# qdrant/qdrant

Measured on AMD Instinct MI355X. Metric: QPS @ recall@10, brute-force, d=768 10M vecs, f32 cosine top-10, higher is better.
Workload: dtype f32 (int8 prefilter + exact f32 re-score)

## Files before the change

include/qdrant_amd.h:

```cpp
#ifndef QDRANT_AMD_H
#define QDRANT_AMD_H

#include <stddef.h>
#include <stdint.h>

#ifdef __cplusplus
extern "C" {
#endif

#define QMX_API __attribute__((visibility("default")))

typedef enum qmx_status {
    QMX_OK = 0,
    QMX_ERR_OUT_OF_MEMORY = 1,
    QMX_ERR_OUT_OF_BOUNDS = 2,
    QMX_ERR_NOT_SUPPORTED = 3,
    QMX_ERR_NOT_READY = 4,
    QMX_ERR_TIMEOUT = 5,
    QMX_ERR_OTHER = 6,
    QMX_ERR_CANCELLED = 7,
    QMX_ERR_BAD_ARG = 8,
    QMX_ERR_NO_DEVICE = 9
} qmx_status;

// ... 135 lines not shown

QMX_API int32_t qmx_segment_create(const qmx_segment_desc *desc, qmx_segment **out);
QMX_API int32_t qmx_segment_create_from_files(const qmx_segment_desc *desc, const char *vectors_path, const char *deleted_path,
                                              qmx_segment **out);

QMX_API int32_t qmx_segment_create_chunked(const qmx_segment_desc *desc, const void *const *chunks, uint64_t rows_per_chunk,
                                           uint32_t n_chunks, qmx_segment **out);
QMX_API int32_t qmx_segment_destroy(qmx_segment *seg);
QMX_API int32_t qmx_segment_set_deleted(qmx_segment *seg, const uint64_t *point_deleted,
                                        uint64_t n_point_bits, const uint64_t *vec_deleted,
                                        uint64_t n_vec_bits);
QMX_API int32_t qmx_segment_read_rows(const qmx_segment *seg, const uint32_t *ids, uint32_t n,
                                      void *out_rows );
QMX_API int32_t qmx_segment_row_bytes(const qmx_segment *seg, uint64_t *out);

typedef struct qmx_sparse_segment_desc {
    uint64_t n;
    const uint64_t *offsets;
    const uint32_t *indices;
    const float *values;
    const uint32_t *map_keys;
    const uint32_t *map_values;
    uint64_t n_map;
    int32_t device_id;
    uint32_t flags;
} qmx_sparse_segment_desc;
QMX_API int32_t qmx_sparse_segment_create(const qmx_sparse_segment_desc *desc, qmx_segment **out);
QMX_API int32_t qmx_sparse_query_create(const qmx_segment *seg, const uint64_t *offsets, const uint32_t *indices, const float *values, uint32_t nq,
                                        qmx_query **out);
typedef struct qmx_segment_info {
    uint32_t derived_copy;
    uint32_t chosen_by_trial;
    uint64_t derived_copy_bytes;
    float i8_scale_balance;
    float trial_i8_ms;
    float trial_half_ms;
    float trial_i8_verified_rows;
    uint32_t trial_i8_fallback_queries;
    uint32_t reserved;
} qmx_segment_info;
QMX_API int32_t qmx_segment_get_info(const qmx_segment *seg, qmx_segment_info *out);


QMX_API int32_t qmx_preprocess_f32(int32_t device_id, uint32_t distance, const float *in,
                                   uint64_t n, uint32_t dim, float *out);
QMX_API int32_t qmx_cast_f32(int32_t device_id, uint32_t dst_dtype, const float *in, uint64_t count,
                             void *out);


QMX_API int32_t qmx_query_create(const qmx_segment *seg, const float *queries, uint32_t nq,
                                 qmx_query **out);
QMX_API int32_t qmx_query_create_internal(const qmx_segment *seg, const uint32_t *point_ids,
                                          uint32_t nq, qmx_query **out);
QMX_API int32_t qmx_query_update(qmx_query *q, const float *queries);
QMX_API int32_t qmx_query_set_filter(qmx_query *q, const uint64_t *allowed, uint64_t n_bits);
QMX_API int32_t qmx_query_destroy(qmx_query *q);
QMX_API int32_t qmx_query_set_stream(qmx_query *q, void *hip_stream);
QMX_API int32_t qmx_query_synchronize(qmx_query *q);
QMX_API int32_t qmx_query_set_timing(qmx_query *q, int32_t enabled);
QMX_API int32_t qmx_query_timing(qmx_query *q, float *total_ms, uint32_t *n_launches);
QMX_API int32_t qmx_query_last_kernel(const qmx_query *q, char *buf, size_t buf_len);
QMX_API int32_t qmx_query_read_encoded(const qmx_query *q, uint32_t query_index, void *out,
                                       uint64_t out_bytes, uint64_t *written);


QMX_API int32_t qmx_score_points(qmx_query *q, const uint32_t *ids, uint32_t n, float *scores,
                                 qmx_counters *counters);
QMX_API int32_t qmx_score_points_ragged(qmx_query *q, const uint32_t *ids, const uint32_t *offsets,
                                        float *scores, qmx_counters *counters);
QMX_API int32_t qmx_score_point(qmx_query *q, uint32_t query_index, uint32_t id, float *out);
QMX_API int32_t qmx_score_internal(const qmx_segment *seg, const uint32_t *a, const uint32_t *b,
                                   uint32_t n, float *out);
QMX_API int32_t qmx_score_bytes(qmx_query *q, const void *rows, uint32_t n, uint64_t stride_bytes,
                                float *scores );


QMX_API int32_t qmx_search_topk(qmx_query *q, uint32_t top, const uint32_t *ids, uint64_t n_ids,
                                qmx_scored_point *out, uint32_t *out_counts,
                                const volatile uint8_t *is_stopped, qmx_counters *counters);
QMX_API int32_t qmx_search_topk_async(qmx_query *q, uint32_t top, const uint32_t *ids,
                                      uint64_t n_ids, qmx_scored_point *out_dev,
                                      uint32_t *out_counts_dev);
QMX_API int32_t qmx_query_last_counters(qmx_query *q, qmx_counters *out);

QMX_API int32_t qmx_rescore(qmx_query *q, const uint32_t *ids, const uint32_t *counts,
                            uint32_t n_per_query, uint32_t top, qmx_scored_point *out,
                            uint32_t *out_counts);

typedef struct qmx_search_params {
    uint32_t top;
    float oversampling;
    uint8_t rescore;
    uint8_t acorn;
    uint8_t pad_[2];
    uint32_t hnsw_ef;
} qmx_search_params;

QMX_API int32_t qmx_search_quantized(const qmx_hnsw *g, qmx_query *searched, qmx_query *original, const qmx_search_params *params,
                                     const uint32_t *ids, uint64_t n_ids, qmx_scored_point *out, uint32_t *out_counts,
                                     const volatile uint8_t *is_stopped, qmx_counters *counters);


typedef enum qmx_custom_kind {
    QMX_CUSTOM_RECO_BEST_SCORE = 0,
    QMX_CUSTOM_RECO_SUM_SCORES = 1,
    QMX_CUSTOM_DISCOVER = 2,
    QMX_CUSTOM_CONTEXT = 3,
    QMX_CUSTOM_FEEDBACK = 4
} qmx_custom_kind;
typedef struct qmx_custom_query {
    uint32_t kind;
    uint32_t first;
    uint32_t n_a;
    uint32_t n_b;
    uint32_t coef_first;
} qmx_custom_query;

QMX_API int32_t qmx_custom_set_coefficients(qmx_query *examples, const float *coefs, uint32_t n);

QMX_API int32_t qmx_multi_score_points(qmx_query *inner, const uint32_t *query_first, uint32_t n_queries, const uint64_t *point_offsets,
                                       uint32_t n_points, const uint32_t *ids, uint32_t n, float *scores);
QMX_API int32_t qmx_multi_search_topk(qmx_query *inner, const uint32_t *query_first, uint32_t n_queries, const uint64_t *point_offsets,
                                      uint32_t n_points, const uint64_t *point_deleted, uint64_t n_deleted_bits, uint32_t top,
                                      const uint32_t *ids, uint64_t n_ids, qmx_scored_point *out, uint32_t *out_counts);

QMX_API int32_t qmx_hnsw_search_with_vectors(const qmx_hnsw *g, qmx_query *links, qmx_query *base, uint32_t top, uint32_t ef,
                                             qmx_scored_point *out, uint32_t *out_counts, const volatile uint8_t *is_stopped,
                                             qmx_counters *counters);

QMX_API int32_t qmx_multi_hnsw_search(const qmx_hnsw *g, qmx_query *inner, const uint32_t *query_first, uint32_t n_queries,
                                      const uint64_t *point_offsets, uint32_t n_points, const uint64_t *point_deleted, uint64_t n_deleted_bits,
                                      uint32_t top, uint32_t ef, qmx_scored_point *out, uint32_t *out_counts, qmx_counters *counters);

QMX_API int32_t qmx_custom_score_points(qmx_query *examples, const qmx_custom_query *queries, uint32_t n_queries,
                                        const uint32_t *ids, uint32_t n, float *scores);
QMX_API int32_t qmx_custom_search_topk(qmx_query *examples, const qmx_custom_query *queries, uint32_t n_queries, uint32_t top,
                                       const uint32_t *ids, uint64_t n_ids, qmx_scored_point *out, uint32_t *out_counts);

QMX_API int32_t qmx_sparse_custom_score_points(qmx_query *examples, const qmx_custom_query *queries, uint32_t n_queries,
                                               const uint32_t *ids, uint32_t n, float *scores);
QMX_API int32_t qmx_sparse_custom_search_topk(qmx_query *examples, const qmx_custom_query *queries, uint32_t n_queries, uint32_t top,
                                              const uint32_t *ids, uint64_t n_ids, qmx_scored_point *out, uint32_t *out_counts,
                                              const volatile uint8_t *is_stopped, qmx_counters *counters);

QMX_API int32_t qmx_custom_hnsw_search(const qmx_hnsw *g, qmx_query *ex, const qmx_custom_query *queries, uint32_t n_queries, uint32_t top,
                                       uint32_t ef, qmx_scored_point *out, uint32_t *out_counts, const volatile uint8_t *is_stopped,
                                       qmx_counters *counters);

QMX_API int32_t qmx_multi_custom_score_points(qmx_query *inner, const uint32_t *example_first, uint32_t n_examples,
                                              const qmx_custom_query *queries, uint32_t n_queries, const uint64_t *point_offsets,
                                              uint32_t n_points, const uint32_t *ids, uint32_t n, float *scores );
QMX_API int32_t qmx_multi_custom_search_topk(qmx_query *inner, const uint32_t *example_first, uint32_t n_examples,
                                             const qmx_custom_query *queries, uint32_t n_queries, const uint64_t *point_offsets,
                                             uint32_t n_points, const uint64_t *point_deleted, uint64_t n_deleted_bits, uint32_t top,
                                             const uint32_t *ids, uint64_t n_ids, qmx_scored_point *out, uint32_t *out_counts);
QMX_API int32_t qmx_multi_custom_hnsw_search(const qmx_hnsw *g, qmx_query *inner, const uint32_t *example_first, uint32_t n_examples,
                                             const qmx_custom_query *queries, uint32_t n_queries, const uint64_t *point_offsets, uint32_t n_points,
                                             const uint64_t *point_deleted, uint64_t n_deleted_bits, uint32_t top, uint32_t ef, qmx_scored_point *out,
                                             uint32_t *out_counts, qmx_counters *counters);

QMX_API int32_t qmx_merge_topk(int32_t device_id, const qmx_scored_point *lists,
                               const uint32_t *list_counts, uint32_t n_lists, uint32_t nq,
                               uint32_t k, qmx_scored_point *out, uint32_t *out_counts);

QMX_API int32_t qmx_merge_topk_async(int32_t device_id, void *hip_stream, const qmx_scored_point *lists_dev,
                                     const uint32_t *list_counts_dev, const uint32_t *list_idx_base_dev,
// ... 155 lines not shown
```

qdrant_amd/_ffi.py:

```python
import ctypes as C
import os

_HERE = os.path.dirname(os.path.abspath(__file__))
LIB_PATH = os.path.join(_HERE, "libqdrant_amd.so")
TESTDATA_LIB_PATH = os.path.join(_HERE, "libqmx_testdata.so")

OK, ERR_OUT_OF_MEMORY, ERR_OUT_OF_BOUNDS, ERR_NOT_SUPPORTED, ERR_NOT_READY, ERR_TIMEOUT, ERR_OTHER, \
    ERR_CANCELLED, ERR_BAD_ARG, ERR_NO_DEVICE = range(10)
STATUS_NAMES = ["OK", "OUT_OF_MEMORY", "OUT_OF_BOUNDS", "NOT_SUPPORTED", "NOT_READY", "TIMEOUT", "OTHER",
                "CANCELLED", "BAD_ARG", "NO_DEVICE"]

DTYPE_F32, DTYPE_F16, DTYPE_U8, DTYPE_SQ_U8, DTYPE_PQ, DTYPE_BQ, DTYPE_TQ, DTYPE_SPARSE = range(8)
COSINE, EUCLID, DOT, MANHATTAN = range(4)

SEG_DATA_ON_DEVICE = 0x1
SEG_U8_SCALAR_ORDER = 0x2
SEG_TIME_KERNELS = 0x4
SEG_BQ_TOGGLE_INVERT = 0x8
SEG_SPLIT_COPY = 0x10
SEG_HALF_COPY = 0x20
SEG_I8_COPY = 0x40
SEG_AUTO_COPY = 0x80
SEG_PQ_PREFILTER_COPY = 0x100


class ScoredPoint(C.Structure):
    _fields_ = [("idx", C.c_uint32), ("score", C.c_float)]


class Counters(C.Structure):
    _fields_ = [("vectors_scored", C.c_uint64), ("bytes_read", C.c_uint64), ("kernel_launches", C.c_uint64),
                ("kernel_ms", C.c_float), ("reserved", C.c_float),
                ("prefilter_candidates", C.c_uint64), ("verified_rows", C.c_uint64), ("fallback_queries", C.c_uint32), ("prefilter_queries", C.c_uint32)]


class SqParams(C.Structure):
    _fields_ = [("actual_dim", C.c_uint32), ("alpha", C.c_float), ("offset", C.c_float), ("multiplier", C.c_float),
                ("invert", C.c_uint8), ("pad_", C.c_uint8 * 3)]


class PqParams(C.Structure):
    _fields_ = [("chunk_size", C.c_uint32), ("n_centroids", C.c_uint32), ("centroids", C.c_void_p),
                ("invert", C.c_uint8), ("lut_mfma", C.c_uint8), ("pad_", C.c_uint8 * 2)]


class BqParams(C.Structure):
    _fields_ = [("encoding", C.c_uint32), ("query_encoding", C.c_uint32), ("mean", C.c_void_p), ("stddev", C.c_void_p)]


BQ_ONE_BIT, BQ_TWO_BITS, BQ_ONE_AND_HALF_BITS = range(3)
BQ_QUERY_SAME_AS_STORAGE, BQ_QUERY_SCALAR_4BITS, BQ_QUERY_SCALAR_8BITS = range(3)


class TqParams(C.Structure):
    _fields_ = [("bits", C.c_uint32), ("rotation_unpadded", C.c_uint32), ("invert", C.c_uint8), ("plus_mode", C.c_uint8), ("pad_", C.c_uint8 * 2),
                ("reserved", C.c_uint32), ("ec_shift", C.c_void_p), ("ec_scale", C.c_void_p)]


TQ_BITS4, TQ_BITS2, TQ_BITS1_5, TQ_BITS1 = range(4)


class SegmentInfo(C.Structure):
    _fields_ = [("derived_copy", C.c_uint32), ("chosen_by_trial", C.c_uint32), ("derived_copy_bytes", C.c_uint64), ("i8_scale_balance", C.c_float),
                ("trial_i8_ms", C.c_float), ("trial_half_ms", C.c_float), ("trial_i8_verified_rows", C.c_float), ("trial_i8_fallback_queries", C.c_uint32),
                ("reserved", C.c_uint32)]


class SegmentDesc(C.Structure):
    _fields_ = [("dtype", C.c_uint32), ("distance", C.c_uint32), ("dim", C.c_uint32), ("flags", C.c_uint32),
                ("n", C.c_uint64), ("row_stride_bytes", C.c_uint64), ("data", C.c_void_p),
                ("device_id", C.c_int32), ("reserved", C.c_int32), ("sq", C.POINTER(SqParams)),
                ("pq", C.POINTER(PqParams)), ("bq", C.POINTER(BqParams)), ("tq", C.POINTER(TqParams))]


class SparseSegmentDesc(C.Structure):
    _fields_ = [("n", C.c_uint64), ("offsets", C.c_void_p), ("indices", C.c_void_p), ("values", C.c_void_p),
                ("map_keys", C.c_void_p), ("map_values", C.c_void_p), ("n_map", C.c_uint64), ("device_id", C.c_int32), ("flags", C.c_uint32)]


class HnswDesc(C.Structure):
    _fields_ = [("m", C.c_uint32), ("m0", C.c_uint32), ("n_points", C.c_uint32), ("n_levels", C.c_uint32),
                ("reindex", C.c_void_p), ("level_offsets", C.c_void_p), ("offsets", C.c_void_p), ("n_offsets", C.c_uint64),
                ("neighbors", C.c_void_p), ("n_neighbors", C.c_uint64),
                ("entry_point_ids", C.c_void_p), ("entry_point_levels", C.c_void_p), ("n_entry_points", C.c_uint32),
                ("n_extra_entry_points", C.c_uint32), ("extra_entry_point_ids", C.c_void_p),
                ("extra_entry_point_levels", C.c_void_p), ("device_id", C.c_int32), ("reserved", C.c_int32)]


class QuantMeta(C.Structure):
    _fields_ = [("dtype", C.c_uint32), ("dim", C.c_uint32), ("distance", C.c_uint32), ("invert", C.c_uint8),
                ("has_deprecated_count", C.c_uint8), ("bq_query_encoding", C.c_uint8), ("pad_", C.c_uint8),
                ("deprecated_count", C.c_uint64), ("sq", SqParams), ("pq", PqParams), ("bq", BqParams), ("tq", TqParams), ("owner", C.c_void_p)]


class GraphLinks(C.Structure):
    _fields_ = [("format", C.c_uint32), ("m", C.c_uint32), ("m0", C.c_uint32), ("n_points", C.c_uint32), ("n_levels", C.c_uint32),
                ("reserved", C.c_uint32), ("n_offsets", C.c_uint64), ("n_neighbors", C.c_uint64),
                ("reindex", C.POINTER(C.c_uint32)), ("level_offsets", C.POINTER(C.c_uint64)), ("offsets", C.POINTER(C.c_uint64)),
                ("neighbors", C.POINTER(C.c_uint32)), ("owner", C.c_void_p)]


class HnswBuildParams(C.Structure):
    _fields_ = [("m", C.c_uint32), ("m0", C.c_uint32), ("ef_construct", C.c_uint32), ("entry_points_num", C.c_uint32),
                ("seed", C.c_uint64), ("max_batch", C.c_uint32), ("reserved", C.c_uint32)]


class HnswInfo(C.Structure):
    _fields_ = [("m", C.c_uint32), ("m0", C.c_uint32), ("n_points", C.c_uint32), ("n_levels", C.c_uint32),
                ("n_offsets", C.c_uint64), ("n_neighbors", C.c_uint64), ("n_entry_points", C.c_uint32),
                ("n_extra_entry_points", C.c_uint32)]


class SearchParams(C.Structure):
    _fields_ = [("top", C.c_uint32), ("oversampling", C.c_float), ("rescore", C.c_uint8), ("acorn", C.c_uint8), ("pad_", C.c_uint8 * 2), ("hnsw_ef", C.c_uint32)]


class CustomQuery(C.Structure):
    _fields_ = [("kind", C.c_uint32), ("first", C.c_uint32), ("n_a", C.c_uint32), ("n_b", C.c_uint32), ("coef_first", C.c_uint32)]


CUSTOM_RECO_BEST_SCORE, CUSTOM_RECO_SUM_SCORES, CUSTOM_DISCOVER, CUSTOM_CONTEXT, CUSTOM_FEEDBACK = range(5)


class FusionParams(C.Structure):
    _fields_ = [("kind", C.c_uint32), ("rrf_k", C.c_uint32), ("weights", C.c_void_p), ("n_weights", C.c_uint32), ("top", C.c_uint32)]


FUSION_RRF, FUSION_DBSF = range(2)
FUSE_MAX_SOURCES, FUSE_MAX_ENTRIES, MMR_MAX_CANDIDATES = 64, 8192, 4096


class QmxError(RuntimeError):
    def __init__(self, status, message):
        self.status = status
        name = STATUS_NAMES[status] if 0 <= status < len(STATUS_NAMES) else str(status)
        super().__init__(f"qmx status {status} ({name}): {message}")


_P = C.c_void_p
TESTDATA_SIGNATURES = {
    "qmx_synth_fill_f32": (C.c_int32, [C.c_int32, C.c_uint64, C.c_uint64, C.c_uint64, C.c_uint32, C.c_void_p]),
    "qmx_synth_fill_latent_f32": (C.c_int32, [C.c_int32, C.c_uint64, C.c_uint64, C.c_uint64, C.c_uint32, C.c_uint32, C.c_float, C.c_void_p]),
}

SIGNATURES = {
    "qmx_abi_version": (C.c_uint32, []),
    "qmx_set_option": (C.c_int32, [C.c_char_p, C.c_int64]),
    "qmx_get_option": (C.c_int32, [C.c_char_p, C.POINTER(C.c_int64)]),
    "qmx_device_count": (C.c_int32, [C.POINTER(C.c_int32)]),
    "qmx_last_error": (C.c_int32, [C.c_char_p, C.c_size_t]),
    "qmx_segment_create": (C.c_int32, [C.POINTER(SegmentDesc), C.POINTER(_P)]),
    "qmx_segment_create_chunked": (C.c_int32, [C.POINTER(SegmentDesc), _P, C.c_uint64, C.c_uint32, C.POINTER(_P)]),
    "qmx_segment_destroy": (C.c_int32, [_P]),
    "qmx_segment_set_deleted": (C.c_int32, [_P, _P, C.c_uint64, _P, C.c_uint64]),
    "qmx_segment_read_rows": (C.c_int32, [_P, _P, C.c_uint32, _P]),
    "qmx_segment_row_bytes": (C.c_int32, [_P, C.POINTER(C.c_uint64)]),
    "qmx_segment_get_info": (C.c_int32, [_P, C.POINTER(SegmentInfo)]),
    "qmx_sparse_segment_create": (C.c_int32, [C.POINTER(SparseSegmentDesc), C.POINTER(_P)]),
    "qmx_sparse_query_create": (C.c_int32, [_P, _P, _P, _P, C.c_uint32, C.POINTER(_P)]),
    "qmx_preprocess_f32": (C.c_int32, [C.c_int32, C.c_uint32, _P, C.c_uint64, C.c_uint32, _P]),
    "qmx_cast_f32": (C.c_int32, [C.c_int32, C.c_uint32, _P, C.c_uint64, _P]),
    "qmx_query_create": (C.c_int32, [_P, _P, C.c_uint32, C.POINTER(_P)]),
    "qmx_query_create_internal": (C.c_int32, [_P, _P, C.c_uint32, C.POINTER(_P)]),
    "qmx_query_update": (C.c_int32, [_P, _P]),
    "qmx_query_set_filter": (C.c_int32, [_P, _P, C.c_uint64]),
    "qmx_query_destroy": (C.c_int32, [_P]),
    "qmx_query_set_stream": (C.c_int32, [_P, _P]),
    "qmx_query_synchronize": (C.c_int32, [_P]),
    "qmx_query_set_timing": (C.c_int32, [_P, C.c_int32]),
    "qmx_query_timing": (C.c_int32, [_P, C.POINTER(C.c_float), C.POINTER(C.c_uint32)]),
    "qmx_query_last_kernel": (C.c_int32, [_P, C.c_char_p, C.c_size_t]),
    "qmx_query_read_encoded": (C.c_int32, [_P, C.c_uint32, _P, C.c_uint64, C.POINTER(C.c_uint64)]),
    "qmx_score_points": (C.c_int32, [_P, _P, C.c_uint32, _P, C.POINTER(Counters)]),
    "qmx_score_points_ragged": (C.c_int32, [_P, _P, _P, _P, C.POINTER(Counters)]),
    "qmx_score_point": (C.c_int32, [_P, C.c_uint32, C.c_uint32, C.POINTER(C.c_float)]),
    "qmx_score_internal": (C.c_int32, [_P, _P, _P, C.c_uint32, _P]),
    "qmx_score_bytes": (C.c_int32, [_P, _P, C.c_uint32, C.c_uint64, _P]),
    "qmx_search_topk": (C.c_int32, [_P, C.c_uint32, _P, C.c_uint64, _P, _P, _P, C.POINTER(Counters)]),
    "qmx_search_topk_async": (C.c_int32, [_P, C.c_uint32, _P, C.c_uint64, _P, _P]),
    "qmx_query_last_counters": (C.c_int32, [_P, C.POINTER(Counters)]),
    "qmx_rescore": (C.c_int32, [_P, _P, _P, C.c_uint32, C.c_uint32, _P, _P]),
    "qmx_search_quantized": (C.c_int32, [_P, _P, _P, C.POINTER(SearchParams), _P, C.c_uint64, _P, _P, _P, C.POINTER(Counters)]),
    "qmx_custom_score_points": (C.c_int32, [_P, _P, C.c_uint32, _P, C.c_uint32, _P]),
    "qmx_custom_search_topk": (C.c_int32, [_P, _P, C.c_uint32, C.c_uint32, _P, C.c_uint64, _P, _P]),
    "qmx_sparse_custom_score_points": (C.c_int32, [_P, _P, C.c_uint32, _P, C.c_uint32, _P]),
    "qmx_sparse_custom_search_topk": (C.c_int32, [_P, _P, C.c_uint32, C.c_uint32, _P, C.c_uint64, _P, _P, _P, C.POINTER(Counters)]),
    "qmx_custom_hnsw_search": (C.c_int32, [_P, _P, _P, C.c_uint32, C.c_uint32, C.c_uint32, _P, _P, _P, C.POINTER(Counters)]),
    "qmx_multi_custom_score_points": (C.c_int32, [_P, _P, C.c_uint32, _P, C.c_uint32, _P, C.c_uint32, _P, C.c_uint32, _P]),
    "qmx_multi_custom_search_topk": (C.c_int32, [_P, _P, C.c_uint32, _P, C.c_uint32, _P, C.c_uint32, _P, C.c_uint64, C.c_uint32, _P, C.c_uint64, _P, _P]),
    "qmx_multi_custom_hnsw_search": (C.c_int32, [_P, _P, _P, C.c_uint32, _P, C.c_uint32, _P, C.c_uint32, _P, C.c_uint64, C.c_uint32, C.c_uint32, _P, _P,
                                                 C.POINTER(Counters)]),
    "qmx_merge_topk": (C.c_int32, [C.c_int32, _P, _P, C.c_uint32, C.c_uint32, C.c_uint32, _P, _P]),
    "qmx_merge_topk_async": (C.c_int32, [C.c_int32, _P, _P, _P, _P, C.c_uint32, C.c_uint32, C.c_uint32, _P, _P]),
    "qmx_topk_record_bytes": (C.c_uint64, [C.c_uint32, C.c_uint32]),
    "qmx_merge_topk_packed_async": (C.c_int32, [C.c_int32, _P, _P, _P, C.c_uint32, C.c_uint32, C.c_uint32, _P, _P]),
    "qmx_fuse_topk": (C.c_int32, [C.c_int32, _P, _P, C.c_uint32, C.c_uint32, C.c_uint32, C.POINTER(FusionParams), _P, _P]),
    "qmx_fuse_topk_async": (C.c_int32, [C.c_int32, _P, _P, _P, C.c_uint32, C.c_uint32, C.c_uint32, C.POINTER(FusionParams), _P, _P]),
    "qmx_mmr_select": (C.c_int32, [_P, _P, _P, C.c_uint32, C.c_float, C.c_uint32, _P, _P]),
    "qmx_mmr_select_async": (C.c_int32, [_P, _P, _P, C.c_uint32, C.c_float, C.c_uint32, _P, _P]),
    "qmx_sharded_search_topk": (C.c_int32, [_P, C.c_uint32, C.c_uint32, _P, _P, _P, _P, C.POINTER(Counters)]),
    "qmx_sharded_search_topk_async": (C.c_int32, [_P, C.c_uint32, C.c_uint32, _P, _P, _P]),
    "qmx_sharded_hnsw_search": (C.c_int32, [_P, _P, C.c_uint32, C.c_uint32, C.c_uint32, _P, _P, _P, _P, C.POINTER(Counters)]),
    "qmx_sharded_query_update": (C.c_int32, [_P, C.c_uint32, _P]),
    "qmx_hnsw_create": (C.c_int32, [C.POINTER(HnswDesc), C.POINTER(_P)]),
    "qmx_hnsw_create_from_plain_file": (C.c_int32, [_P, C.c_uint64, C.POINTER(HnswDesc), C.POINTER(_P)]),
    "qmx_hnsw_create_from_file": (C.c_int32, [_P, C.c_uint64, C.POINTER(HnswDesc), C.POINTER(_P)]),
    "qmx_quant_meta_parse": (C.c_int32, [C.c_uint32, C.c_char_p, C.c_uint64, C.POINTER(QuantMeta)]),
    "qmx_quant_meta_free": (None, [C.POINTER(QuantMeta)]),
    "qmx_graph_links_decode": (C.c_int32, [_P, C.c_uint64, C.POINTER(GraphLinks)]),
    "qmx_graph_links_free": (None, [C.POINTER(GraphLinks)]),
    "qmx_hnsw_destroy": (C.c_int32, [_P]),
    "qmx_hnsw_build": (C.c_int32, [_P, C.POINTER(HnswBuildParams), C.POINTER(_P)]),
    "qmx_hnsw_build_quantized": (C.c_int32, [_P, _P, C.POINTER(HnswBuildParams), C.POINTER(_P)]),
    "qmx_sharded_hnsw_build": (C.c_int32, [C.POINTER(_P), C.POINTER(_P), C.c_uint32, C.POINTER(HnswBuildParams), C.POINTER(_P), C.POINTER(C.c_int32)]),
    "qmx_hnsw_get_info": (C.c_int32, [_P, C.POINTER(HnswInfo)]),
    "qmx_hnsw_export_plain": (C.c_int32, [_P, _P, _P, _P, _P, _P, _P, _P, _P]),
    "qmx_hnsw_search": (C.c_int32, [_P, _P, C.c_uint32, C.c_uint32, _P, _P, _P, C.POINTER(Counters)]),
    "qmx_hnsw_search_acorn": (C.c_int32, [_P, _P, C.c_uint32, C.c_uint32, _P, _P, _P, C.POINTER(Counters)]),
    "qmx_hnsw_search_async": (C.c_int32, [_P, _P, C.c_uint32, C.c_uint32, _P, _P, _P]),
    "qmx_hnsw_search_traced": (C.c_int32, [_P, _P, C.c_uint32, C.c_uint32, _P, _P, _P, C.c_uint32, _P]),
    "qmx_sq_encode": (C.c_int32, [C.c_int32, C.c_uint32, C.POINTER(SqParams), _P, C.c_uint64, C.c_uint32, _P]),
    "qmx_pq_train": (C.c_int32, [C.c_int32, _P, C.c_uint64, C.c_uint32, C.c_uint32, C.c_uint32, C.c_uint32, C.c_float, C.c_uint32, _P, _P]),
    "qmx_sq_fit_min_max": (C.c_int32, [C.c_int32, C.c_uint32, _P, C.c_uint64, C.c_uint32, C.POINTER(SqParams)]),
    "qmx_segment_create_from_files": (C.c_int32, [C.POINTER(SegmentDesc), C.c_char_p, C.c_char_p, C.POINTER(_P)]),
    "qmx_sq_fit_quantile": (C.c_int32, [C.c_int32, C.c_uint32, _P, C.c_uint64, C.c_uint32, C.c_uint64, C.c_float, C.POINTER(SqParams), C.POINTER(C.c_int32)]),
    "qmx_multi_score_points": (C.c_int32, [_P, _P, C.c_uint32, _P, C.c_uint32, _P, C.c_uint32, _P]),
    "qmx_multi_search_topk": (C.c_int32, [_P, _P, C.c_uint32, _P, C.c_uint32, _P, C.c_uint64, C.c_uint32, _P, C.c_uint64, _P, _P]),
    "qmx_tq_encode": (C.c_int32, [C.c_int32, C.c_uint32, C.c_uint32, _P, _P, C.c_uint64, _P]),
    "qmx_vector_stats": (C.c_int32, [C.c_int32, _P, C.c_uint64, C.c_uint32, _P, _P, _P, _P]),
    "qmx_tq_fit_plus": (C.c_int32, [C.c_int32, C.c_uint32, C.c_uint32, _P, _P, C.c_uint64, _P, _P]),
    "qmx_hnsw_search_with_vectors": (C.c_int32, [_P, _P, _P, C.c_uint32, C.c_uint32, _P, _P, _P, _P]),
    "qmx_multi_hnsw_build": (C.c_int32, [_P, _P, C.c_uint32, _P, C.c_uint64, _P, _P]),
    "qmx_multi_hnsw_build_quantized": (C.c_int32, [_P, _P, _P, C.c_uint32, _P, C.c_uint64, _P, _P]),
    "qmx_multi_hnsw_search": (C.c_int32, [_P, _P, _P, C.c_uint32, _P, C.c_uint32, _P, C.c_uint64, C.c_uint32, C.c_uint32, _P, _P, _P]),
    "qmx_custom_set_coefficients": (C.c_int32, [_P, _P, C.c_uint32]),
    "qmx_bq_encode_ex": (C.c_int32, [C.c_int32, C.POINTER(BqParams), _P, C.c_uint64, C.c_uint32, _P]),
    "qmx_bq_row_bytes": (C.c_uint64, [C.c_uint32, C.c_uint32]),
    "qmx_bq_encode": (C.c_int32, [C.c_int32, _P, C.c_uint64, C.c_uint32, _P]),
    "qmx_pq_encode": (C.c_int32, [C.c_int32, C.POINTER(PqParams), _P, C.c_uint64, C.c_uint32, _P]),
}

_lib = None


def lib():
    global _lib
    if _lib is None:
        if not os.path.exists(LIB_PATH):
            raise ImportError(
                f"{LIB_PATH} is missing: build it with `make` (hipcc --offload-arch=gfx950). "
                "qdrant_amd has no CPU fallback.")
        handle = C.CDLL(LIB_PATH)
        for name, (res, args) in SIGNATURES.items():
            fn = getattr(handle, name)
            fn.restype = res
            fn.argtypes = args
        if os.path.exists(TESTDATA_LIB_PATH):
            td = C.CDLL(TESTDATA_LIB_PATH)
            for name, (res, args) in TESTDATA_SIGNATURES.items():
                fn = getattr(td, name)
                fn.restype = res
                fn.argtypes = args
                setattr(handle, name, fn)
# ... 44 lines not shown
```

qdrant_amd/csrc/api_core.hip:

```cpp
#include "api_internal.hpp"

namespace qmx {

static thread_local std::string g_last_error;
const std::string &last_error_text() { return g_last_error; }

void set_error(const char *fmt, ...) {
    char buf[1024];
    va_list ap;
    va_start(ap, fmt);
    vsnprintf(buf, sizeof(buf), fmt, ap);
    va_end(ap);
    g_last_error = buf;
}

int32_t hip_status(hipError_t e, const char *what, const char *file, int line) {
    set_error("HIP error %d (%s) at %s:%d: %s", (int)e, hipGetErrorString(e), file, line, what);
    (void)hipGetLastError();
    switch (e) {
        case hipErrorOutOfMemory: return QMX_ERR_OUT_OF_MEMORY;
        case hipErrorNoDevice:
        case hipErrorInvalidDevice:
        case hipErrorNoBinaryForGpu:
        case hipErrorInsufficientDriver: return QMX_ERR_NO_DEVICE;
        case hipErrorNotReady: return QMX_ERR_NOT_READY;
        case hipErrorInvalidValue: return QMX_ERR_BAD_ARG;
        default: return QMX_ERR_OTHER;
    }
}

static const char *const g_option_names[OPT_COUNT] = {"no_mfma_scan", "no_mfma16", "no_prescan", "prescan_shift", "hnsw_log_cap", "no_split_scan", "split_min_queries", "no_split256", "no_pq_pair", "no_pq_prefilter", "pq_prefilter_min_queries", "hnsw_pq_per_cu", "tq_rotate_block", "no_topk_small", "verify_max_per_query", "hnsw_pq_direct_walk", "hnsw_pq_table_build", "hnsw_no_pq_prefilter", "hnsw_no_lds_visited", "pq_lut_no_lds", "hnsw_per_cu", "hnsw_reference_heap_order", "tq_wide_min_queries", "tq_wide_high_digit", "sq_wide_min_queries", "i8_resident", "debug"};
struct OptionTable {
    std::atomic<int64_t> v[OPT_COUNT];
    int64_t initial[OPT_COUNT];
    OptionTable() {
        for (int i = 0; i < OPT_COUNT; ++i) {
            char env[64] = "QMX_";
            size_t k = 4;
            for (const char *c = g_option_names[i]; *c && k + 1 < sizeof(env); ++c) env[k++] = (char)toupper((unsigned char)*c);
            env[k] = 0;
            const char *e = getenv(env);
            int64_t val = 0;
            if (e) { val = (*e >= '0' && *e <= '9') ? atoll(e) : 1; }
            if (i == OPT_PRESCAN_SHIFT && !e) val = 10;
            if (i == OPT_SPLIT_MIN_QUERIES && !e) val = 1;
            if (i == OPT_PQ_PREFILTER_MIN_QUERIES && !e) val = 4;
            if (i == OPT_TQ_WIDE_MIN_QUERIES && !e) val = 33;
            if (i == OPT_SQ_WIDE_MIN_QUERIES && !e) val = 33;
            if (i == OPT_I8_RESIDENT && !e) val = 1;
            initial[i] = val;
            v[i].store(val, std::memory_order_relaxed);
        }
    }
};
static OptionTable g_options;
int64_t option(Option o) { return g_options.v[o].load(std::memory_order_relaxed); }

static thread_local const void *g_last_kernel = nullptr;
const void *last_noted_kernel() { return g_last_kernel; }
void note_kernel(const void *host_function) { g_last_kernel = host_function; }

void clear_stale_error() {
    hipError_t e = hipGetLastError();
    if (e != hipSuccess) {
        const bool debug = option(OPT_DEBUG) != 0;
        if (debug) fprintf(stderr, "[qmx] dropped stale HIP error %d (%s) before a kernel launch\n", (int)e, hipGetErrorString(e));
    }
}

bool is_device_ptr(const void *p) {
    if (!p) return false;
    hipPointerAttribute_t attr;
    hipError_t e = hipPointerGetAttributes(&attr, p);
    if (e != hipSuccess) {
        (void)hipGetLastError();
        return false;
    }
    return attr.type == hipMemoryTypeDevice || attr.type == hipMemoryTypeManaged;
}

uint32_t elem_bytes(uint32_t dtype) {
    switch (dtype) {
        case QMX_DTYPE_F32: return 4;
        case QMX_DTYPE_F16: return 2;
        default: return 1;
    }
}



int32_t check_device(int32_t device_id, hipDeviceProp_t *prop_out) {
    int count = 0;
    hipError_t e = hipGetDeviceCount(&count);
    if (e != hipSuccess || count == 0) {
        (void)hipGetLastError();
        set_error("no HIP device visible (%s); libqdrant_amd has no CPU fallback", e == hipSuccess ? "count=0" : hipGetErrorString(e));
        return QMX_ERR_NO_DEVICE;
    }
    QMX_REQUIRE(device_id >= 0 && device_id < count, QMX_ERR_NO_DEVICE, "device %d out of range (have %d)", device_id, count);
    hipDeviceProp_t prop;
    QMX_HIP(hipGetDeviceProperties(&prop, device_id));
    QMX_REQUIRE(strncmp(prop.gcnArchName, "gfx950", 6) == 0, QMX_ERR_NO_DEVICE,
                "device %d is %s; this library ships gfx950 (MI355X) code objects only", device_id, prop.gcnArchName);
    QMX_HIP(hipSetDevice(device_id));
    if (prop_out) *prop_out = prop;
    return QMX_OK;
}

}


extern "C" {


// ... 48 lines not shown
```

qdrant_amd/csrc/api_internal.hpp:

```cpp
#pragma once
#include <stdarg.h>
#include <stdio.h>
#include <stdlib.h>
#include <string.h>

#include <ctype.h>
#include <cxxabi.h>

#include <algorithm>
#include <atomic>
#include <mutex>
#include <string>
#include <thread>
#include <new>
#include <vector>

#include "kernels.hpp"
#include "tq_rotate.hpp"

namespace qmx {
const std::string &last_error_text();
const void *last_noted_kernel();
bool is_device_ptr(const void *p);
uint32_t elem_bytes(uint32_t dtype);
// ... 58 lines not shown
    uint32_t tq_bits = 0, tq_value_bits = 0, tq_padded_dim = 0, tq_rot_dim = 0, tq_code_bytes = 0, tq_n_chunks = 0;
    bool tq_invert = false;
    float *d_tq_sf = nullptr, *d_tq_l2 = nullptr, *d_tq_xm = nullptr;
    bool tq_wide = false;
    float tq_sf_min = 0.f, tq_sf_max = 0.f, tq_l2_min = 0.f, tq_l2_max = 0.f;
    uint32_t tq_c1 = 0;
    float *d_tq_shift = nullptr, *d_tq_scale = nullptr;
    int16_t *d_tq_weights = nullptr;
    float tq_weight_scale = 1.0f, tq_mm_const = 0.0f;
    uint32_t *d_tq_tables = nullptr;
    void *d_tq_l1 = nullptr;
    double *d_tq_norms = nullptr;
    bool split_stats = false;
    float row_maxabs = 0.f, row_norm_max = 0.f;
    void *d_rows_split = nullptr;
    bool split_half = false;
    bool split_i8 = false;
    float *d_i8_scale = nullptr;
    uint32_t *d_i8_stats = nullptr;
    float i8_balance = 0.0f;
    uint64_t copy_bytes = 0;
    bool auto_choice = false;
    float auto_i8_ms = 0.0f, auto_half_ms = 0.0f, auto_i8_verified = 0.0f;
    uint32_t auto_i8_fallback = 0;
    SparseSeg *sparse = nullptr;

    bool fast_layout() const {
        if (dtype == QMX_DTYPE_BQ || dtype == QMX_DTYPE_TQ) return row_stride % 16 == 0 && ((uintptr_t)d_rows % 16) == 0;
        if (dtype <= QMX_DTYPE_U8) {
            const uint64_t eb = dtype == QMX_DTYPE_F32 ? 4 : dtype == QMX_DTYPE_F16 ? 2 : 1;
            return dim < 32 ? (row_stride % eb == 0 && ((uintptr_t)d_rows % eb) == 0)
                            : (row_stride % 16 == 0 && ((uintptr_t)d_rows % 16) == 0);
        }
        return true;
    }
    DeletedView deleted_view() const {
        DeletedView v;
        v.point_deleted = d_point_deleted;
        v.n_point_bits = n_point_bits;
        v.vec_deleted = d_vec_deleted;
        v.n_vec_bits = n_vec_bits;
        v.n_rows = n;
        v.allowed = nullptr;
        v.n_allowed_bits = 0;
        return v;
    }
    uint64_t scan_rows() const { return d_point_deleted ? std::min<uint64_t>(n, n_point_bits) : n; }
};

struct qmx_query {
    const qmx_segment *seg = nullptr;
    int device = 0;
    uint32_t nq = 0;
    uint32_t nq_padded = 0;
    uint32_t q_stride = 0;
    uint32_t bq_bits = 1;
    uint32_t tq_qbytes_off = 0;
    uint32_t aux_off = 0;
    void *d_queries = nullptr;
    hipStream_t stream = nullptr;
    hipStream_t own_stream = nullptr;
    struct EvPair { hipEvent_t a = nullptr, b = nullptr; };
    std::vector<EvPair> evs;
    size_t ev_used = 0;
    float timing_ms = 0.f;
    uint32_t timing_launches = 0;
    DevBuf partial, out, counts, ids, scores, misc, enc, bounds, gthr;
    DevBuf mv_qfirst, mv_offsets, mv_deleted;
    DevBuf cq_multi;
    DevBuf cq_sims, cq_scores, cq_desc, cq_coefs;
    uint32_t n_cq_coefs = 0;
    DevBuf cand, cand_cnt, cand_ids;
    DevBuf mmr_ids, mmr_rel;
    DevBuf sp_bq, sp_f32, sp_cand, sp_cnt, sp_ver, sp_vscores, sp_sample, sp_wl, xcnt, tq_rot;
    DevBuf sh_lists, sh_out;
    std::vector<uint32_t> sh_bases_host;
    hipEvent_t sh_done = nullptr;
    hipEvent_t sh_merged = nullptr;
    DevBuf pq_table;
    DevBuf sp_probe, sp_pscores;
    DevBuf sp_plan, sp_fq;
    qmx_counters last_counters{};
    bool last_split = false, last_pq = false;
    uint32_t last_fqt = 64;
    uint64_t last_row_bytes = 0, last_n_cand = 0;
    uint64_t sp_sample_n = 0, sp_sample_of = 0;
    DevBuf filter;
    uint64_t n_filter_bits = 0;
    bool has_filter = false;
    DevBuf hnsw_lutx;
    DevBuf hnsw_pq8;
    DevBuf hnsw_next;
    DevBuf hnsw_refc;
    DevBuf hnsw_vis, hnsw_log, hnsw_scored;
    uint32_t hnsw_slots = 0;
    uint64_t hnsw_vis_words = 0;
    int *d_err = nullptr;
    uint32_t partial_grid_cap = 0;
    bool timing = false;
    const void *last_kernel = nullptr;
    SparseQuery *sparse = nullptr;
};

static inline bool is_sparse(const qmx_segment *s) { return s && s->dtype == QMX_DTYPE_SPARSE; }
static inline bool is_sparse(const qmx_query *q) { return q && is_sparse(q->seg); }
static inline int32_t refuse_sparse(const char *fn) {
    set_error("%s: not supported on a sparse segment (QMX_DTYPE_SPARSE)", fn);
    return QMX_ERR_NOT_SUPPORTED;
}
#define QMX_REFUSE_SPARSE(x)                                 \
    do {                                                     \
        if (is_sparse(x)) return refuse_sparse(__func__);    \
    } while (0)


static bool mfma_scan_ok(const qmx_segment *s) {
    if (s->dtype == QMX_DTYPE_SQ_U8) return sq_mfma_ok(s->distance, s->scan_dim) && !option(OPT_NO_MFMA_SCAN);
    if (s->dtype == QMX_DTYPE_TQ) return !option(OPT_NO_MFMA_SCAN);
    return (s->dtype == QMX_DTYPE_F32 || s->dtype == QMX_DTYPE_F16) && (s->distance == QMX_DISTANCE_DOT || s->distance == QMX_DISTANCE_COSINE) && s->dim >= 32 &&
           s->fast_layout() && !option(OPT_NO_MFMA_SCAN);
}
constexpr uint32_t MAX_QT_MFMA = 32;
constexpr uint32_t MAX_QT_TOPK = 64;
static bool bq_mfma_ok(const qmx_query *q);
static uint32_t tile_qt(const qmx_segment *s, const qmx_query *q) {
    if (s->dtype == QMX_DTYPE_BQ) return bq_mfma_ok(q) && (size_t)MAX_QT_MFMA * q->q_stride <= 150 * 1024 ? MAX_QT_MFMA : MAX_QT;
    if (s->dtype == QMX_DTYPE_SQ_U8) return mfma_scan_ok(s) ? MAX_QT_MFMA : MAX_QT;
    if (s->dtype == QMX_DTYPE_TQ) return mfma_scan_ok(s) && (size_t)MAX_QT_MFMA * q->q_stride <= 150 * 1024 ? MAX_QT_MFMA : 4;
    return mfma_scan_ok(s) && (size_t)MAX_QT_MFMA * (((size_t)s->dim * 4 + 127) / 128 * 128 + QUERY_AUX_BYTES) <= 150 * 1024 ? MAX_QT_MFMA : MAX_QT;
}

static bool bq_mfma_ok(const qmx_query *q) {
    return q->seg->dtype == QMX_DTYPE_BQ && q->tq_qbytes_off != 0 && !option(OPT_NO_MFMA_SCAN) && (size_t)MAX_QT * q->q_stride <= 150 * 1024;
}

static uint32_t lds_tile_stride(uint32_t bytes) { return bytes + (16u + 256u - bytes % 256u) % 256u; }

static void tq_entry_layout(const qmx_segment *seg, uint32_t *pieces, uint32_t *qbytes_off, uint32_t *aux_off) {
    *pieces = seg->tq_value_bits == 4 ? 4 : (seg->tq_value_bits == 1 && seg->d_tq_shift) ? 16 : 8;
    const uint32_t body = (seg->scan_dim + 63) & ~63u;
    *aux_off = body * *pieces;
    *qbytes_off = 0;
    if (seg->tq_value_bits == 1) {
        *qbytes_off = *aux_off;
        *aux_off += body * (*pieces == 16 ? 16 : 8);
    }
}

static int32_t stage_in(qmx_query *q, DevBuf &buf, const void *src, size_t bytes, const void **dev_out) {
    if (bytes == 0 || !src) {
        *dev_out = nullptr;
        return QMX_OK;
    }
    if (is_device_ptr(src)) {
        *dev_out = src;
        return QMX_OK;
    }
    QMX_TRY(buf.reserve(bytes));
    QMX_HIP(hipMemcpyAsync(buf.p, src, bytes, hipMemcpyHostToDevice, q->stream));
    *dev_out = buf.p;
    return QMX_OK;
}

static int32_t copy_out(hipStream_t st, void *dst, const void *src_dev, size_t bytes) {
    if (bytes == 0) return QMX_OK;
    QMX_HIP(hipMemcpyAsync(dst, src_dev, bytes, is_device_ptr(dst) ? hipMemcpyDeviceToDevice : hipMemcpyDeviceToHost, st));
// ... 165 lines not shown
```

qdrant_amd/csrc/api_search.hip:

```cpp
#include "api_internal.hpp"

extern "C" {



static int32_t split_stage(qmx_query *q, const char *what) {
    if (option(OPT_DEBUG) < 2) return QMX_OK;
    hipError_t e = hipStreamSynchronize(q->stream);
    fprintf(stderr, "[qmx] split stage %-28s %s\n", what, e == hipSuccess ? "ok" : hipGetErrorString(e));
    fflush(stderr);
    return e == hipSuccess ? QMX_OK : QMX_ERR_OTHER;
}

static int32_t verify_pool(qmx_query *q, unsigned char *plan, VerifyPool *vp) {
    const uint32_t cap = (uint32_t)std::min<uint64_t>(std::max<uint64_t>((uint64_t)q->nq * SPLIT_VCAP, 262144), 1u << 26);
    QMX_TRY(q->sp_ver.reserve(((size_t)cap * 2 + (size_t)q->nq * 2) * 4));
    QMX_TRY(q->sp_vscores.reserve((size_t)cap * 4));
    uint32_t *b = (uint32_t *)q->sp_ver.p;
    vp->ids = b;
    vp->qsel = b + cap;
    vp->off = b + (size_t)2 * cap;
    vp->cnt = vp->off + q->nq;
    vp->used = (uint32_t *)(plan + 24);
    vp->cap = cap;
    const int64_t mx = option(OPT_VERIFY_MAX_PER_QUERY);
    vp->max_per_query = mx > 0 ? (uint32_t)std::min<int64_t>(mx, cap) : cap;
    return QMX_OK;
}
static inline float split_rel_band(bool half, uint32_t dim) {
    const float acc = (float)dim * 1.1920929e-7f;
    return (half ? 9.765625e-4f + 9.5367432e-7f : 1.9073486e-6f) + acc;
}

__global__ void sample_ids_kernel(uint32_t *ids, uint32_t n, uint64_t step) {
    const uint32_t i = blockIdx.x * blockDim.x + threadIdx.x;
    if (i < n) ids[i] = (uint32_t)((uint64_t)i * step);
}

constexpr uint32_t PQF_TILE = 256;
constexpr uint32_t PQF_WCAP = 512;
static int32_t pq_prefilter_enqueue(qmx_query *q, uint32_t top, uint64_t n_cand, qmx_scored_point *d_out, uint32_t *d_counts,
                                    const volatile uint8_t *is_stopped, qmx_counters *counters, bool timed) {
    const qmx_segment *s = q->seg;
    const SplitPlanLayout pl(q->nq);
    const uint32_t m = s->pq_m, m_pad = (m + 31) / 32 * 32;
    const uint32_t tile_max = std::min<uint32_t>(PQF_TILE, q->nq);
    const uint32_t grid_max = pq_prefilter_grid(s->num_cus, tile_max, nullptr);
    QMX_TRY(q->gthr.reserve((size_t)std::max<uint32_t>(q->nq_padded, PQF_TILE) * sizeof(uint64_t)));
    QMX_TRY(q->pq_table.reserve(pq_prefilter_table_bytes(m, tile_max) + (size_t)(PQF_TILE + 4) * 4));
    QMX_TRY(q->sp_f32.reserve(1024 * sizeof(float)));
    QMX_TRY(q->sp_cand.reserve((size_t)tile_max * SPLIT_CAND_CAP * sizeof(uint64_t)));
    QMX_TRY(q->sp_cnt.reserve((size_t)SPLIT_QT_MAX * 4));
    {
        uint32_t g = grid_max;
        for (uint32_t t = 4; t <= tile_max; t += 4) g = std::max(g, pq_prefilter_grid(s->num_cus, t, nullptr));
        QMX_TRY(q->sp_wl.reserve(pq_prefilter_wlists_bytes(g, PQF_WCAP)));
    }
    QMX_TRY(q->sp_plan.reserve(pl.bytes));
    unsigned char *plan = (unsigned char *)q->sp_plan.p;
    VerifyPool vp;
    QMX_TRY(verify_pool(q, plan, &vp));
    float *band = (float *)q->sp_f32.p;
    q->last_counters = qmx_counters{};
    q->last_split = false;
    const int sshift = (int)std::min<int64_t>(std::max<int64_t>(option(OPT_PRESCAN_SHIFT) - 2, 1), 20);
    const uint64_t S = std::min<uint64_t>(n_cand, std::max<uint64_t>(n_cand >> sshift, 8192));
    if (q->sp_sample_n != S || q->sp_sample_of != n_cand) {
        QMX_TRY(q->sp_sample.reserve((size_t)S * 4));
        ::qmx::clear_stale_error();
        hipLaunchKernelGGL(sample_ids_kernel, dim3((uint32_t)((S + 255) / 256)), dim3(256), 0, q->stream, (uint32_t *)q->sp_sample.p, (uint32_t)S, n_cand / S);
        QMX_HIP(hipGetLastError());
        q->sp_sample_n = S;
        q->sp_sample_of = n_cand;
    }
    const uint32_t *d_sample = (const uint32_t *)q->sp_sample.p;
    QMX_HIP(hipMemsetAsync(plan, 0, pl.zero_bytes, q->stream));
    uint32_t n_tiles = 0, launches = 0;
    for (uint32_t tile0 = 0; tile0 < q->nq; tile0 += PQF_TILE, ++n_tiles) {
        const uint32_t nq_tile = std::min<uint32_t>(PQF_TILE, q->nq - tile0);
        if (is_stopped && *is_stopped) {
            set_error("search cancelled");
            return QMX_ERR_CANCELLED;
        }
        uint64_t *gthr = (uint64_t *)q->gthr.p + tile0;
        ScanArgs a;
        fill_args(q, tile0, nq_tile, a);
        a.n_cand = n_cand;
        a.top = top;
        QMX_TRY(q->scores.reserve((size_t)nq_tile * S * sizeof(float)));
        const uint32_t SQT = tile_qt(s, q);
        for (uint32_t st0 = 0; st0 < nq_tile; st0 += SQT) {
            const uint32_t nq_sub = std::min<uint32_t>(SQT, nq_tile - st0);
            ScanArgs pre;
            fill_args(q, tile0 + st0, nq_sub, pre);
            pre.ids = d_sample;
            pre.n_cand = S;
            pre.top = 1;
            pre.scores = (float *)q->scores.p + (size_t)st0 * S;
            pre.scores_stride = S;
            uint32_t pgrid = 0;
            QMX_TRY(launch_scan(q, (int)pow2_ceil(nq_sub), SCAN_SCORES, pre, &pgrid));
            ++launches;
        }
        QMX_TRY(launch_custom_topk(q->stream, (const float *)q->scores.p, S, d_sample, a.del, nq_tile, top, d_out + (size_t)tile0 * top, d_counts + tile0, gthr));
        int32_t *thr = (int32_t *)((unsigned char *)q->pq_table.p + pq_prefilter_table_bytes(m, tile_max));
        QMX_TRY(launch_pq_lut8(q->stream, a.queries, q->q_stride, nq_tile, m, s->pq.n_centroids, gthr, q->pq_table.p, thr, band));
        QMX_HIP(hipMemsetAsync(q->sp_cnt.p, 0, (size_t)SPLIT_QT_MAX * 4, q->stream));
        uint32_t grid = 0;
        size_t slot = 0;
        if (timed) QMX_TRY(timing_begin(q, &slot));
        QMX_TRY(launch_pq_prefilter(q->stream, a, s->d_pq_rot, q->pq_table.p, thr, nq_tile, s->num_cus, q->sp_wl.p, PQF_WCAP, &grid));
        q->last_kernel = last_noted_kernel();
        if (timed) QMX_TRY(timing_end(q, slot));
        int *tile_ovf = (int *)(plan + pl.tile_ovf) + n_tiles;
        QMX_TRY(launch_regroup_lists(q->stream, a.del, (const unsigned char *)q->sp_wl.p + pq_prefilter_wlists_counts_bytes(grid), (const uint32_t *)q->sp_wl.p, PQF_WCAP,
                                     grid * 16, (uint64_t *)q->sp_cand.p, (uint32_t *)q->sp_cnt.p, SPLIT_CAND_CAP, tile_ovf));
        QMX_TRY(launch_split_select(q->stream, (const uint64_t *)q->sp_cand.p, (const uint32_t *)q->sp_cnt.p, SPLIT_CAND_CAP, band, nq_tile, top, vp, tile0,
                                    tile_ovf, (uint32_t *)(plan + pl.ovf_q) + tile0, (SplitStats *)plan));
        launches += 6;
    }
    const void *pf_kernel = q->last_kernel;
    PairSel sel{vp.qsel, 0, nullptr, vp.used};
    QMX_TRY(score_pairs_device(q, sel, vp.ids, vp.cap, (float *)q->sp_vscores.p, false));
    QMX_TRY(launch_sort_scored(q->stream, (const float *)q->sp_vscores.p, vp.ids, vp.cnt, 0, q->nq, top, d_out, d_counts, vp.off));
    uint32_t *ovf_list = (uint32_t *)(plan + pl.list);
    QMX_TRY(launch_split_plan(q->stream, (const uint32_t *)(plan + pl.ovf_q), q->nq, (const uint64_t *)q->gthr.p, ovf_list, (uint64_t *)(plan + pl.gthr_packed),
                              pl.list_cap, (uint32_t *)(plan + pl.count), (int *)(plan + pl.run16), (int *)(plan + pl.run64), pl.n_run64, (SplitStats *)plan, nullptr, 0,
                              nullptr));
    {
        ScanArgs a;
        fill_args(q, 0, q->nq, a);
        a.n_cand = n_cand;
        a.top = top;
        a.q_map = ovf_list;
        a.run_if = (const int *)(plan + pl.count);
        const uint64_t want = (n_cand + 1023) / 1024, cap = std::max<uint64_t>(1, ((uint64_t)s->num_cus * 2 + q->nq - 1) / q->nq);
        uint32_t slabs = (uint32_t)std::max<uint64_t>(1, std::min(want, cap));
        QMX_TRY(q->partial.reserve((size_t)slabs * q->nq * top * sizeof(uint64_t)));
        a.partial = (uint64_t *)q->partial.p;
        a.partial_qt = q->nq;
        QMX_TRY(launch_scan_pq(q->stream, SCAN_TOPK, a, s->num_cus, &slabs));
        QMX_TRY(launch_merge_keys(q->stream, (const uint64_t *)q->partial.p, slabs, q->nq, q->nq, top, d_out, d_counts, top, 0, nullptr, a.run_if, ovf_list,
                                  slabs * q->nq));
        launches += 5;
    }
    q->last_kernel = pf_kernel;
    q->last_split = true;
    q->last_pq = true;
    {
        qmx_counters &c = q->last_counters;
        c.vectors_scored = (uint64_t)q->nq * n_cand;
        c.bytes_read = (uint64_t)((q->nq + 3) / 4) * n_cand * m_pad + (uint64_t)q->nq * S * s->row_bytes;
        c.kernel_launches = launches;
        c.prefilter_queries = q->nq;
        q->last_row_bytes = s->row_bytes;
        q->last_n_cand = n_cand;
        if (counters) *counters = c;
    }
    return QMX_OK;
}

constexpr uint32_t TQW_FQT = 32;
static int32_t wide_exact_enqueue(qmx_query *q, uint32_t top, uint64_t n_cand, qmx_scored_point *d_out, uint32_t *d_counts, const volatile uint8_t *is_stopped,
                                  qmx_counters *counters, bool timed) {
    const qmx_segment *s = q->seg;
    const bool sq = s->dtype == QMX_DTYPE_SQ_U8;
    const bool tq_high = !sq && option(OPT_TQ_WIDE_HIGH_DIGIT) != 0;
    const SplitPlanLayout pl(q->nq, TQW_FQT);
    const uint32_t grid_cap = (uint32_t)s->num_cus * 8;
    QMX_TRY(q->gthr.reserve((size_t)std::max<uint32_t>(q->nq_padded, SPLIT_QT) * sizeof(uint64_t)));
    QMX_TRY(q->sp_bq.reserve(sq ? sqw_query_bytes(s->scan_dim) : tq4w_query_bytes(s->scan_dim)));
    QMX_TRY(q->sp_f32.reserve(1024 * sizeof(float)));
    QMX_TRY(q->sp_cand.reserve((size_t)SPLIT_QT * SPLIT_CAND_CAP * sizeof(uint64_t)));
    QMX_TRY(q->sp_cnt.reserve((size_t)SPLIT_QT_MAX * 4));
    QMX_TRY(q->sp_wl.reserve(sq ? sqw_wlists_bytes(s->num_cus) : tq4w_wlists_bytes(s->num_cus)));
    QMX_TRY(q->sp_plan.reserve(pl.bytes));
    QMX_TRY(q->sp_fq.reserve((size_t)pl.list_cap * q->q_stride));
    QMX_TRY(q->partial.reserve((size_t)grid_cap * TQW_FQT * std::min<uint32_t>(top, MAX_TOP_FAST) * sizeof(uint64_t)));
    unsigned char *plan = (unsigned char *)q->sp_plan.p;
    VerifyPool vp;
    QMX_TRY(verify_pool(q, plan, &vp));
    float *qinfo = (float *)q->sp_f32.p, *band = qinfo + 512;
    int32_t *thr_i = (int32_t *)(qinfo + 768);
    q->last_counters = qmx_counters{};
    q->last_split = false;
    const int sshift = (int)std::min<int64_t>(std::max<int64_t>(option(OPT_PRESCAN_SHIFT) - (sq ? 2 : 3), 1), 20);
    const uint64_t S = std::min<uint64_t>(n_cand, std::max<uint64_t>(n_cand >> sshift, 8192));
    if (q->sp_sample_n != S || q->sp_sample_of != n_cand) {
        QMX_TRY(q->sp_sample.reserve((size_t)S * 4));
        ::qmx::clear_stale_error();
        hipLaunchKernelGGL(sample_ids_kernel, dim3((uint32_t)((S + 255) / 256)), dim3(256), 0, q->stream, (uint32_t *)q->sp_sample.p, (uint32_t)S, n_cand / S);
        QMX_HIP(hipGetLastError());
        q->sp_sample_n = S;
        q->sp_sample_of = n_cand;
    }
    const uint32_t *d_sample = (const uint32_t *)q->sp_sample.p;
    QMX_HIP(hipMemsetAsync(plan, 0, pl.zero_bytes, q->stream));
    uint32_t n_tiles = 0, launches = 2;
    const void *wide_kernel = nullptr;
    for (uint32_t tile0 = 0; tile0 < q->nq; tile0 += SPLIT_QT, ++n_tiles) {
        const uint32_t nq_tile = std::min<uint32_t>(SPLIT_QT, q->nq - tile0);
        if (is_stopped && *is_stopped) {
            set_error("search cancelled");
            return QMX_ERR_CANCELLED;
        }
        uint64_t *gthr = (uint64_t *)q->gthr.p + tile0;
        ScanArgs a;
        fill_args(q, tile0, nq_tile, a);
        a.n_cand = n_cand;
        a.top = top;
        QMX_TRY(q->scores.reserve((size_t)nq_tile * S * sizeof(float)));
        QMX_TRY(score_matrix_enqueue(q, tile0, nq_tile, d_sample, S, (float *)q->scores.p, S, &launches));
        QMX_TRY(launch_custom_topk(q->stream, (const float *)q->scores.p, S, d_sample, a.del, nq_tile, top, d_out + (size_t)tile0 * top, d_counts + tile0, gthr));
        if (sq) QMX_TRY(launch_sqw_pack(q->stream, a, gthr, s->sq_off_absmax, q->sp_bq.p, thr_i, qinfo, band, (uint32_t *)q->sp_cnt.p, SPLIT_QT_MAX));
        else QMX_TRY(launch_tq4w_pack(q->stream, a, gthr, s->tq_sf_min, s->tq_sf_max, s->tq_l2_min, s->tq_l2_max, s->tq_c1, tq_high ? 1 : 0, q->sp_bq.p, thr_i, qinfo, band,
                                      (uint32_t *)q->sp_cnt.p, SPLIT_QT_MAX));
        uint32_t grid = 0;
        size_t slot = 0;
        if (timed) QMX_TRY(timing_begin(q, &slot));
        if (sq) QMX_TRY(launch_scan_sqw(q->stream, a, q->sp_bq.p, thr_i, s->d_sq_bi, qinfo, s->num_cus, q->sp_wl.p, &grid));
        else QMX_TRY(launch_scan_tq4w(q->stream, a, q->sp_bq.p, thr_i, qinfo, tq_high ? band : nullptr, s->num_cus, q->sp_wl.p, &grid));
        wide_kernel = last_noted_kernel();
        if (timed) QMX_TRY(timing_end(q, slot));
        int *tile_ovf = (int *)(plan + pl.tile_ovf) + n_tiles;
        QMX_TRY(launch_regroup_lists(q->stream, a.del, (const unsigned char *)q->sp_wl.p + (sq ? sqw_wlists_counts_bytes(s->num_cus) : tq4w_wlists_counts_bytes(s->num_cus)), (const uint32_t *)q->sp_wl.p,
                                     sq ? sqw_wcap() : tq4w_wcap(),
                                     grid * 8, (uint64_t *)q->sp_cand.p, (uint32_t *)q->sp_cnt.p, SPLIT_CAND_CAP, tile_ovf));
        QMX_TRY(launch_split_select(q->stream, (const uint64_t *)q->sp_cand.p, (const uint32_t *)q->sp_cnt.p, SPLIT_CAND_CAP, band, nq_tile, top, vp, tile0, tile_ovf,
                                    (uint32_t *)(plan + pl.ovf_q) + tile0, (SplitStats *)plan, tq_high ? qinfo + 3 * SPLIT_QT : nullptr, tq_high));
        launches += 6;
    }
    PairSel sel{vp.qsel, 0, nullptr, vp.used};
    QMX_TRY(score_pairs_device(q, sel, vp.ids, vp.cap, (float *)q->sp_vscores.p, false));
    QMX_TRY(launch_sort_scored(q->stream, (const float *)q->sp_vscores.p, vp.ids, vp.cnt, 0, q->nq, top, d_out, d_counts, vp.off));
    uint32_t *ovf_list = (uint32_t *)(plan + pl.list);
    uint64_t *gthr_packed = (uint64_t *)(plan + pl.gthr_packed);
    QMX_TRY(launch_split_plan(q->stream, (const uint32_t *)(plan + pl.ovf_q), q->nq, (const uint64_t *)q->gthr.p, ovf_list, gthr_packed, pl.list_cap,
                              (uint32_t *)(plan + pl.count), (int *)(plan + pl.run16), (int *)(plan + pl.run64), pl.n_run64, (SplitStats *)plan, q->d_queries,
                              q->q_stride, q->sp_fq.p));
    for (uint32_t pass = 0; pass <= pl.n_run64; ++pass) {
        if (pass && q->nq <= 16) break;
        const uint32_t p0 = pass ? (pass - 1) * TQW_FQT : 0;
        const uint32_t nq_sub = pass ? std::min<uint32_t>(TQW_FQT, q->nq - p0) : std::min<uint32_t>(16, q->nq);
        const int *run_if = pass ? (const int *)(plan + pl.run64) + (pass - 1) : (const int *)(plan + pl.run16);
        ScanArgs a;
        fill_args(q, 0, nq_sub, a);
        a.queries = (const char *)q->sp_fq.p + (size_t)p0 * q->q_stride;
        a.n_cand = n_cand;
        a.top = top;
        a.partial = (uint64_t *)q->partial.p;
        a.gthr = gthr_packed + p0;
        a.run_if = run_if;
        const int fqt = (int)std::max<uint32_t>(16, pow2_ceil(nq_sub));
        a.partial_qt = (uint32_t)fqt;
        uint32_t grid = grid_cap;
        if (sq) QMX_TRY(launch_scan_sq_mfma(q->stream, fqt, SCAN_TOPK, a, s->num_cus, &grid));
        else QMX_TRY(launch_scan_tq_mfma(q->stream, fqt, SCAN_TOPK, a, s->num_cus, &grid));
        QMX_TRY(launch_merge_keys(q->stream, (const uint64_t *)q->partial.p, grid, (uint32_t)fqt, nq_sub, top, d_out, d_counts, top, 0, nullptr, run_if, ovf_list + p0));
        launches += 2;
    }
    q->last_kernel = wide_kernel;
    q->last_split = true;
    q->last_pq = false;
    q->last_fqt = TQW_FQT;
    {
        qmx_counters &c = q->last_counters;
        c.vectors_scored = (uint64_t)q->nq * n_cand;
        c.bytes_read = (uint64_t)n_tiles * n_cand * s->row_bytes + (uint64_t)((q->nq + MAX_QT_MFMA - 1) / MAX_QT_MFMA) * S * s->row_bytes;
        c.kernel_launches = launches;
        c.prefilter_queries = q->nq;
        q->last_row_bytes = s->row_bytes;
        q->last_n_cand = n_cand;
        if (counters) *counters = c;
    }
    return QMX_OK;
}

int32_t search_enqueue(qmx_query *q, uint32_t top, const uint32_t *d_ids, uint64_t n_ids,
                              qmx_scored_point *d_out, uint32_t *d_counts, const volatile uint8_t *is_stopped,
                              qmx_counters *counters, bool timed) {
    const qmx_segment *s = q->seg;
    if (is_sparse(s)) return sparse_search_enqueue(q, top, d_ids, n_ids, d_out, d_counts, is_stopped, counters, timed);
    const uint64_t n_cand = d_ids ? n_ids : s->scan_rows();
    if (tq_l1(s)) {
        q->last_counters = qmx_counters{};
        q->last_split = false;
        ScanArgs a;
        fill_args(q, 0, q->nq, a);
        const uint32_t qtile = (uint32_t)std::max<uint64_t>(1, std::min<uint64_t>(q->nq, (1ull << 26) / std::max<uint64_t>(n_cand, 1)));
        QMX_TRY(q->scores.reserve((size_t)qtile * std::max<uint64_t>(n_cand, 1) * sizeof(float)));
        for (uint32_t q0 = 0; q0 < q->nq; q0 += qtile) {
            if (is_stopped && *is_stopped) {
                set_error("search cancelled");
                return QMX_ERR_CANCELLED;
            }
            const uint32_t nq_tile = std::min<uint32_t>(qtile, q->nq - q0);
            QMX_TRY(tq_l1_scores_device(q, q0, nq_tile, d_ids, n_cand, (float *)q->scores.p, n_cand, nullptr));
            QMX_TRY(launch_custom_topk(q->stream, (const float *)q->scores.p, n_cand, d_ids, a.del, nq_tile, top, d_out + (size_t)q0 * top, d_counts + q0));
            if (counters) counters->kernel_launches += 1 + 3 * (uint32_t)((n_cand + 65535) / 65536);
        }
        if (counters) {
            counters->vectors_scored += (uint64_t)q->nq * n_cand;
            counters->bytes_read += (uint64_t)((q->nq + qtile - 1) / qtile) * n_cand * s->row_bytes;
        }
        return QMX_OK;
    }
    if (s->dtype == QMX_DTYPE_PQ && s->d_pq_rot && !d_ids && top <= MAX_TOP_FAST && n_cand >= (1u << 18) && !option(OPT_NO_PQ_PREFILTER) &&
        q->nq >= (uint32_t)std::max<int64_t>(1, option(OPT_PQ_PREFILTER_MIN_QUERIES)))
        return pq_prefilter_enqueue(q, top, n_cand, d_out, d_counts, is_stopped, counters, timed);
    if (s->dtype == QMX_DTYPE_TQ && s->tq_wide && !d_ids && top <= MAX_TOP_FAST && n_cand >= (1u << 18) && mfma_scan_ok(s) && option(OPT_TQ_WIDE_MIN_QUERIES) > 0 &&
        q->nq >= (uint32_t)option(OPT_TQ_WIDE_MIN_QUERIES) && (size_t)MAX_QT_MFMA * q->q_stride <= 150 * 1024) {
        ScanArgs probe;
        fill_args(q, 0, std::min<uint32_t>(q->nq, SPLIT_QT), probe);
        probe.n_cand = n_cand;
        probe.top = top;
        if (tq4w_shape_ok(probe)) return wide_exact_enqueue(q, top, n_cand, d_out, d_counts, is_stopped, counters, timed);
    }
    if (s->dtype == QMX_DTYPE_SQ_U8 && s->sq_wide && !d_ids && top <= MAX_TOP_FAST && n_cand >= (1u << 18) && mfma_scan_ok(s) && option(OPT_SQ_WIDE_MIN_QUERIES) > 0 &&
        q->nq >= (uint32_t)option(OPT_SQ_WIDE_MIN_QUERIES)) {
        ScanArgs probe;
        fill_args(q, 0, std::min<uint32_t>(q->nq, SPLIT_QT), probe);
        probe.n_cand = n_cand;
        probe.top = top;
        if (sqw_shape_ok(probe)) return wide_exact_enqueue(q, top, n_cand, d_out, d_counts, is_stopped, counters, timed);
    }
    const uint32_t grid_cap = (uint32_t)s->num_cus * 8;
    const bool q64 = s->dtype == QMX_DTYPE_F32 && mfma_scan_ok(s) && q->nq > MAX_QT_MFMA && mfma16_dim_ok(64, s->dim) &&
                     !option(OPT_NO_MFMA16);
    const bool q32 = s->dtype == QMX_DTYPE_F32 && mfma_scan_ok(s) && q->nq > MAX_QT && s->dim > 768 && mfma16_dim_ok(32, s->dim) &&
                     !option(OPT_NO_MFMA16);
    const uint32_t split_fqt = split_fallback_qt(s->dim);
    const bool split_dims = s->dtype == QMX_DTYPE_F32 && mfma_scan_ok(s) && (mfma16_dim_ok(64, s->dim) || (s->d_rows_split && split_fqt != 0)) && !option(OPT_NO_MFMA16);
    const bool split = split_dims && (q64 || (s->d_rows_split && q->nq >= (uint32_t)std::max<int64_t>(1, option(OPT_SPLIT_MIN_QUERIES)))) && s->split_stats &&
                       !d_ids && top <= MAX_TOP_FAST && n_cand >= (1u << 18) && s->dim % 128 == 0 && s->row_stride % 16 == 0 && !option(OPT_NO_SPLIT_SCAN);
    const uint32_t split_qt = (split && s->d_rows_split && s->split_half && q->nq > SPLIT_QT && !option(OPT_NO_SPLIT256)) ? SPLIT_QT_MAX : SPLIT_QT;
    const uint32_t TQ = split ? split_qt : q64 ? MAX_QT_TOPK : q32 ? MAX_QT_MFMA : tile_qt(s, q);
    const uint32_t ptop_max = std::min<uint32_t>(top, MAX_TOP_FAST);
    const uint32_t n_pass = (top + MAX_TOP_FAST - 1) / MAX_TOP_FAST;
    QMX_TRY(q->partial.reserve((size_t)grid_cap * std::min<uint32_t>(TQ, MAX_QT_TOPK) * ptop_max * sizeof(uint64_t)));
    if (n_pass > 1) QMX_TRY(q->bounds.reserve((size_t)TQ * sizeof(uint64_t)));
    QMX_TRY(q->gthr.reserve((size_t)std::max<uint32_t>(q->nq_padded, SPLIT_QT_MAX) * sizeof(uint64_t)));
    std::vector<std::pair<uint32_t, uint32_t>> split_tiles;
    float *sp_qnorm = nullptr, *sp_thr = nullptr, *sp_band = nullptr, *sp_scales = nullptr, *sp_qmax = nullptr;
    const SplitPlanLayout pl(q->nq, split_fqt ? split_fqt : SPLIT_FQT);
    unsigned char *plan = nullptr;
    VerifyPool vp{};
    q->last_counters = qmx_counters{};
    q->last_split = false;
    if (split) {
        QMX_TRY(q->sp_bq.reserve(split_query_bytes(s->dim)));
        QMX_TRY(q->sp_f32.reserve(1280 * sizeof(float)));
        QMX_TRY(q->sp_cand.reserve((size_t)split_qt * SPLIT_CAND_CAP * sizeof(uint64_t)));
        QMX_TRY(q->sp_cnt.reserve((size_t)SPLIT_QT_MAX * 4));
        if (s->d_rows_split) QMX_TRY(q->sp_wl.reserve(split_wlists_bytes(s->num_cus)));
        QMX_TRY(q->sp_plan.reserve(pl.bytes));
        QMX_TRY(verify_pool(q, (unsigned char *)q->sp_plan.p, &vp));
        QMX_TRY(q->sp_fq.reserve((size_t)pl.list_cap * q->q_stride));
        if (s->split_i8) {
            QMX_TRY(q->sp_probe.reserve((size_t)q->nq * (split_i8_probe() + 1) * 4));
            QMX_TRY(q->sp_pscores.reserve((size_t)q->nq * split_i8_probe() * 4));
        }
        plan = (unsigned char *)q->sp_plan.p;
        float *f = (float *)q->sp_f32.p;
        sp_qnorm = f; sp_thr = f + 256; sp_band = f + 512; sp_scales = f + 768; sp_qmax = f + 1024;
        const int sshift = (int)std::min<int64_t>(std::max<int64_t>(option(OPT_PRESCAN_SHIFT) + (s->d_rows_split ? 1 : -2), 1), 20);
        const uint64_t S = std::min<uint64_t>(n_cand, std::max<uint64_t>(n_cand >> sshift, 8192));
        if (q->sp_sample_n != S || q->sp_sample_of != n_cand) {
            QMX_TRY(q->sp_sample.reserve((size_t)S * 4));
            ::qmx::clear_stale_error();
            hipLaunchKernelGGL(sample_ids_kernel, dim3((uint32_t)((S + 255) / 256)), dim3(256), 0, q->stream, (uint32_t *)q->sp_sample.p, (uint32_t)S, n_cand / S);
            QMX_HIP(hipGetLastError());
            q->sp_sample_n = S;
            q->sp_sample_of = n_cand;
        }
        QMX_HIP(hipMemsetAsync(plan, 0, pl.zero_bytes, q->stream));
    }
    for (uint32_t tile0 = 0; tile0 < q->nq; tile0 += TQ) {
        const uint32_t nq_tile = std::min<uint32_t>(TQ, q->nq - tile0);
        if (split && (nq_tile > MAX_QT_TOPK || s->d_rows_split)) {
            if (is_stopped && *is_stopped) {
                set_error("search cancelled");
                return QMX_ERR_CANCELLED;
            }
            const uint32_t S = (uint32_t)q->sp_sample_n;
            const uint32_t *d_sample = (const uint32_t *)q->sp_sample.p;
            uint64_t *gthr = (uint64_t *)q->gthr.p + tile0;
            ScanArgs a;
            fill_args(q, tile0, nq_tile, a);
            a.n_cand = n_cand;
            a.top = top;
            QMX_TRY(q->scores.reserve((size_t)nq_tile * S * sizeof(float)));
            QMX_TRY(score_matrix_enqueue(q, tile0, nq_tile, d_sample, S, (float *)q->scores.p, S, nullptr));
            QMX_TRY(launch_custom_topk(q->stream, (const float *)q->scores.p, S, d_sample, a.del, nq_tile, top, d_out + (size_t)tile0 * top, d_counts + tile0, gthr));
            QMX_TRY(split_stage(q, "prescan"));
            if (s->split_i8) {
                float *sp_texact = sp_qnorm, *sp_qscale = sp_qmax;
                QMX_TRY(launch_split_i8_pack(q->stream, (const float *)q->enc.p + (size_t)tile0 * s->dim, nq_tile, s->dim, s->d_i8_scale, gthr, s->d_i8_stats,
                                             s->row_norm_max, q->sp_bq.p, sp_qscale, sp_band, sp_thr, sp_texact, (uint32_t *)q->sp_cnt.p, SPLIT_QT_MAX));
                QMX_TRY(split_stage(q, "int8 pack"));
                const uint32_t np = split_i8_probe();
                uint32_t *probe_ids = (uint32_t *)q->sp_probe.p, *probe_cnt = probe_ids + (size_t)q->nq * np;
                int *tile_ovf = (int *)(plan + pl.tile_ovf) + split_tiles.size();
                const uint32_t sstride = 16;
                for (uint32_t ph = 1; ph <= 2; ++ph) {
                    const uint32_t phase = ph | (sstride << 8);
                    size_t slot = 0;
                    if (timed) QMX_TRY(timing_begin(q, &slot));
                    QMX_TRY(launch_scan_i8copy(q->stream, a, q->sp_bq.p, sp_qscale, sp_thr, s->num_cus, s->d_rows_split, q->sp_wl.p, phase));
                    q->last_kernel = last_noted_kernel();
                    if (timed) QMX_TRY(timing_end(q, slot));
                    QMX_TRY(launch_split_regroup(q->stream, a, q->sp_wl.p, s->num_cus, (uint64_t *)q->sp_cand.p, (uint32_t *)q->sp_cnt.p, SPLIT_CAND_CAP, tile_ovf,
                                                 phase, SPLIT_QT));
                    QMX_TRY(launch_split_i8_probe(q->stream, (const uint64_t *)q->sp_cand.p, (const uint32_t *)q->sp_cnt.p, SPLIT_CAND_CAP, sp_band, nq_tile, top, tile_ovf,
                                                  probe_ids + (size_t)tile0 * np, probe_cnt + tile0));
                    const void *scan_kernel = q->last_kernel;
                    PairSel psel{nullptr, np, probe_cnt};
                    QMX_TRY(score_pairs_device(q, psel, probe_ids, (uint64_t)(tile0 + nq_tile) * np, (float *)q->sp_pscores.p, false));
                    q->last_kernel = scan_kernel;
                    QMX_TRY(launch_split_i8_bound(q->stream, (const float *)q->sp_pscores.p + (size_t)tile0 * np, probe_cnt + tile0, nq_tile, top, sp_band, sp_qscale,
                                                  sp_thr, sp_texact));
                }
                QMX_TRY(split_stage(q, "int8 scan"));
                QMX_TRY(launch_split_select(q->stream, (const uint64_t *)q->sp_cand.p, (const uint32_t *)q->sp_cnt.p, SPLIT_CAND_CAP, sp_band, nq_tile, top, vp, tile0,
                                            tile_ovf, (uint32_t *)(plan + pl.ovf_q) + tile0, (SplitStats *)plan, sp_texact));
                QMX_TRY(split_stage(q, "select"));
                split_tiles.push_back({tile0, nq_tile});
                if (counters) counters->kernel_launches += 13;
                continue;
            }
            const float row_scale = split_row_scale(s->row_maxabs);
            const int half = s->split_half ? 1 : 0;
            const uint32_t tqt = nq_tile > SPLIT_QT ? SPLIT_QT_MAX : SPLIT_QT;
            QMX_TRY(launch_split_pack_queries(q->stream, (const float *)q->enc.p + (size_t)tile0 * s->dim, nq_tile, s->dim, sp_qmax, sp_qnorm, q->sp_bq.p, half, tqt));
            QMX_TRY(launch_split_thresholds(q->stream, gthr, sp_qnorm, sp_qmax, nq_tile, split_rel_band(half, s->dim), s->row_norm_max, row_scale, sp_scales, sp_thr,
                                            sp_band, tqt, (uint32_t *)q->sp_cnt.p, SPLIT_QT_MAX));
            QMX_TRY(split_stage(q, "pack + thresholds"));
            for (uint32_t phase = s->d_rows_split ? 1 : 0; phase <= (s->d_rows_split ? 2u : 0u); ++phase) {
                size_t slot = 0;
                if (timed) QMX_TRY(timing_begin(q, &slot));
                QMX_TRY(launch_scan_f32_split(q->stream, a, q->sp_bq.p, row_scale, sp_scales, sp_thr, (uint64_t *)q->sp_cand.p, (uint32_t *)q->sp_cnt.p,
                                              SPLIT_CAND_CAP, s->num_cus, s->d_rows_split, half, q->sp_wl.p, phase, tqt));
                q->last_kernel = last_noted_kernel();
                if (timed) QMX_TRY(timing_end(q, slot));
                if (s->d_rows_split)
                    QMX_TRY(launch_split_regroup(q->stream, a, q->sp_wl.p, s->num_cus, (uint64_t *)q->sp_cand.p, (uint32_t *)q->sp_cnt.p, SPLIT_CAND_CAP,
                                                 (int *)(plan + pl.tile_ovf) + split_tiles.size(), phase, tqt));
                if (phase == 1)
                    QMX_TRY(launch_split_refine(q->stream, (const uint64_t *)q->sp_cand.p, (const uint32_t *)q->sp_cnt.p, SPLIT_CAND_CAP, sp_band, nq_tile, top,
                                                sp_scales, sp_thr));
            }
            QMX_TRY(split_stage(q, "split kernel"));
            QMX_TRY(launch_split_select(q->stream, (const uint64_t *)q->sp_cand.p, (const uint32_t *)q->sp_cnt.p, SPLIT_CAND_CAP, sp_band, nq_tile, top, vp, tile0,
                                        (const int *)(plan + pl.tile_ovf) + split_tiles.size(), (uint32_t *)(plan + pl.ovf_q) + tile0, (SplitStats *)plan));
            QMX_TRY(split_stage(q, "select"));
            split_tiles.push_back({tile0, nq_tile});
            if (counters) counters->kernel_launches += 8;
            continue;
        }
        const int qt = (int)pow2_ceil(nq_tile);
        for (uint32_t pass = 0; pass < n_pass; ++pass) {
            if (is_stopped && *is_stopped) {
                set_error("search cancelled");
                return QMX_ERR_CANCELLED;
            }
            const uint32_t off = pass * MAX_TOP_FAST;
            const uint32_t ptop = std::min<uint32_t>(MAX_TOP_FAST, top - off);
            ScanArgs a;
            fill_args(q, tile0, nq_tile, a);
            a.ids = d_ids;
            a.n_cand = n_cand;
            a.top = ptop;
            a.partial = (uint64_t *)q->partial.p;
            a.partial_qt = (uint32_t)qt;
            a.key_bound = pass ? (const uint64_t *)q->bounds.p : nullptr;
            const bool m16 = s->dtype == QMX_DTYPE_F32 && mfma_scan_ok(s) && mfma16_scan_ok(qt, SCAN_TOPK, a);
            const bool sqm = (s->dtype == QMX_DTYPE_SQ_U8 || s->dtype == QMX_DTYPE_TQ ? qt >= 4 : s->dtype == QMX_DTYPE_F16 && qt >= 8) && mfma_scan_ok(s);
            const bool m4 = s->dtype == QMX_DTYPE_F32 && qt >= 8 && mfma_scan_ok(s);
            const bool bqk = s->dtype == QMX_DTYPE_BQ && qt >= 4;
            if (pass == 0 && n_cand >= (1u << 18) && (m16 || sqm || m4 || bqk) && !option(OPT_NO_PRESCAN)) {
                const int pre_shift = (int)std::min<int64_t>(std::max<int64_t>(option(OPT_PRESCAN_SHIFT), 1), 20);
                const uint64_t pre_n = std::max<uint64_t>(n_cand >> pre_shift, 1u << 13) & ~(uint64_t)15;
                {
                    QMX_TRY(q->scores.reserve((size_t)nq_tile * pre_n * sizeof(float)));
                    QMX_TRY(score_matrix_enqueue(q, tile0, nq_tile, d_ids, pre_n, (float *)q->scores.p, pre_n, nullptr));
                    QMX_TRY(launch_custom_topk(q->stream, (const float *)q->scores.p, pre_n, d_ids, a.del, nq_tile, ptop, d_out + (size_t)tile0 * top,
                                               d_counts + tile0, (uint64_t *)q->gthr.p + tile0));
                }
                a.gthr = (const uint64_t *)q->gthr.p + tile0;
                if (counters) counters->kernel_launches += 2;
            }
            uint32_t grid = grid_cap;
            size_t slot = 0;
            if (timed) QMX_TRY(timing_begin(q, &slot));
            QMX_TRY(launch_scan(q, qt, SCAN_TOPK, a, &grid));
            q->last_kernel = last_noted_kernel();
            if (timed) QMX_TRY(timing_end(q, slot));
            QMX_TRY(launch_merge_keys(q->stream, (const uint64_t *)q->partial.p, grid, (uint32_t)qt, nq_tile, ptop,
                                      d_out + (size_t)tile0 * top, d_counts + tile0, top, off,
                                      n_pass > 1 ? (uint64_t *)q->bounds.p : nullptr));
            if (counters) counters->kernel_launches += 2;
        }
    }
    if (!split_tiles.empty()) {
        const void *split_kernel = q->last_kernel;
        const uint32_t first = split_tiles.front().first, last = split_tiles.back().first + split_tiles.back().second;
        QMX_REQUIRE(first == 0, QMX_ERR_OTHER, "split tiles must start at query 0");
        PairSel sel{vp.qsel, 0, nullptr, vp.used};
        QMX_TRY(score_pairs_device(q, sel, vp.ids, vp.cap, (float *)q->sp_vscores.p, false));
        QMX_TRY(split_stage(q, "verify gather"));
        QMX_TRY(launch_sort_scored(q->stream, (const float *)q->sp_vscores.p, vp.ids, vp.cnt, 0, last, top, d_out, d_counts, vp.off));
// ... 60 lines not shown

int32_t fold_split_counters(qmx_query *q, qmx_counters *c) {
    if (!q->last_split || !q->sp_plan.p) return QMX_OK;
    SplitStats st;
    QMX_HIP(hipMemcpy(&st, q->sp_plan.p, sizeof(st), hipMemcpyDeviceToHost));
    c->prefilter_candidates = st.candidates;
    c->verified_rows = st.verified;
    c->fallback_queries = st.fallback_queries;
    c->bytes_read += st.verified * q->last_row_bytes;
    if (st.fallback_queries) {
        const uint32_t f = st.fallback_queries;
        const uint64_t passes = q->last_pq ? f : f <= 16 ? 1 : (f + q->last_fqt - 1) / q->last_fqt;
        c->bytes_read += passes * q->last_n_cand * q->last_row_bytes;
    }
    return QMX_OK;
}

int32_t qmx_search_topk(qmx_query *q, uint32_t top, const uint32_t *ids, uint64_t n_ids, qmx_scored_point *out,
                        uint32_t *out_counts, const volatile uint8_t *is_stopped, qmx_counters *counters) {
    QMX_REQUIRE(q && out && out_counts, QMX_ERR_BAD_ARG, "NULL argument");
    if (top == 0 && is_sparse(q)) {
        if (counters) memset(counters, 0, sizeof(*counters));
        QMX_HIP(hipSetDevice(q->device));
        if (is_device_ptr(out_counts)) {
            QMX_HIP(hipMemsetAsync(out_counts, 0, (size_t)q->nq * 4, q->stream));
            QMX_HIP(hipStreamSynchronize(q->stream));
        } else {
            for (uint32_t i = 0; i < q->nq; ++i) out_counts[i] = 0;
        }
        return QMX_OK;
    }
    QMX_REQUIRE(top >= 1, QMX_ERR_BAD_ARG, "top must be > 0 (FixedLengthPriorityQueue::new panics on 0)");
    QMX_REQUIRE(top <= MAX_TOP, QMX_ERR_NOT_SUPPORTED, "top %u > %u not supported yet", top, MAX_TOP);
    QMX_HIP(hipSetDevice(q->seg->device));
    if (counters) memset(counters, 0, sizeof(*counters));
    if (q->nq == 0) return QMX_OK;
    const void *d_ids = nullptr;
    if (ids) {
        if (n_ids == 0) {
            if (is_device_ptr(out_counts)) {
                QMX_HIP(hipMemsetAsync(out_counts, 0, (size_t)q->nq * 4, q->stream));
                QMX_HIP(hipStreamSynchronize(q->stream));
            } else {
                for (uint32_t i = 0; i < q->nq; ++i) out_counts[i] = 0;
            }
            return QMX_OK;
        }
        QMX_TRY(stage_in(q, q->ids, ids, (size_t)n_ids * 4, &d_ids));
    }
    const bool out_dev = is_device_ptr(out);
    const bool cnt_dev = is_device_ptr(out_counts);
    qmx_scored_point *d_out = out;
    uint32_t *d_counts = out_counts;
    if (!out_dev) {
        QMX_TRY(q->out.reserve((size_t)q->nq * top * sizeof(qmx_scored_point)));
        d_out = (qmx_scored_point *)q->out.p;
    }
    if (!cnt_dev) {
        QMX_TRY(q->counts.reserve((size_t)q->nq * sizeof(uint32_t)));
        d_counts = (uint32_t *)q->counts.p;
    }
    const bool timed = q->timing || (q->seg->flags & QMX_SEG_TIME_KERNELS) != 0;
    QMX_TRY(search_enqueue(q, top, (const uint32_t *)d_ids, n_ids, d_out, d_counts, is_stopped, counters, timed));
    if (!out_dev) QMX_TRY(copy_out(q->stream, out, d_out, (size_t)q->nq * top * sizeof(qmx_scored_point)));
    if (!cnt_dev) QMX_TRY(copy_out(q->stream, out_counts, d_counts, (size_t)q->nq * sizeof(uint32_t)));
    QMX_TRY(check_err_flag(q));
    if (counters) QMX_TRY(fold_split_counters(q, counters));
    if (timed) {
        const float before = q->timing_ms;
        QMX_TRY(timing_fold(q));
        if (counters) counters->kernel_ms = q->timing_ms - before;
    }
    return QMX_OK;
}

int32_t qmx_query_last_counters(qmx_query *q, qmx_counters *out) {
    QMX_REQUIRE(q && out, QMX_ERR_BAD_ARG, "NULL argument");
    QMX_HIP(hipSetDevice(q->device));
    QMX_HIP(hipStreamSynchronize(q->stream));
    *out = q->last_counters;
    return fold_split_counters(q, out);
}

int32_t qmx_search_topk_async(qmx_query *q, uint32_t top, const uint32_t *ids, uint64_t n_ids,
                              qmx_scored_point *out_dev, uint32_t *out_counts_dev) {
    QMX_REQUIRE(q && out_dev && out_counts_dev, QMX_ERR_BAD_ARG, "NULL argument");
    QMX_REQUIRE(top >= 1 && top <= MAX_TOP, QMX_ERR_NOT_SUPPORTED, "top %u not in 1..%u", top, MAX_TOP);
    QMX_REQUIRE(!ids || is_device_ptr(ids), QMX_ERR_BAD_ARG, "async search needs device ids");
    QMX_HIP(hipSetDevice(q->seg->device));
    if (q->nq == 0) return QMX_OK;
    const bool timed = q->timing || (q->seg->flags & QMX_SEG_TIME_KERNELS) != 0;
    return search_enqueue(q, top, ids, n_ids, out_dev, out_counts_dev, nullptr, nullptr, timed);
}

int32_t qmx_merge_topk(int32_t device_id, const qmx_scored_point *lists, const uint32_t *list_counts, uint32_t n_lists,
                       uint32_t nq, uint32_t k, qmx_scored_point *out, uint32_t *out_counts) {
    QMX_REQUIRE(lists && out && out_counts, QMX_ERR_BAD_ARG, "NULL argument");
    QMX_REQUIRE(k >= 1 && k <= MAX_TOP, QMX_ERR_NOT_SUPPORTED, "k %u not in 1..%u", k, MAX_TOP);
    QMX_TRY(check_device(device_id, nullptr));
    if (nq == 0) return QMX_OK;
    const size_t lbytes = (size_t)n_lists * nq * k * sizeof(qmx_scored_point);
    const size_t cbytes = (size_t)n_lists * nq * sizeof(uint32_t);
    const size_t obytes = (size_t)nq * k * sizeof(qmx_scored_point);
    DevBuf bl, bc, bo, boc;
    const qmx_scored_point *d_lists = lists;
    const uint32_t *d_lc = list_counts;
    qmx_scored_point *d_out = out;
    uint32_t *d_oc = out_counts;
    int32_t rc = QMX_OK;
    do {
        if (!is_device_ptr(lists)) {
            if ((rc = bl.reserve(lbytes)) != QMX_OK) break;
            if (hipMemcpy(bl.p, lists, lbytes, hipMemcpyHostToDevice) != hipSuccess) { rc = QMX_ERR_OTHER; break; }
            d_lists = (const qmx_scored_point *)bl.p;
        }
        if (list_counts && !is_device_ptr(list_counts)) {
            if ((rc = bc.reserve(cbytes)) != QMX_OK) break;
            if (hipMemcpy(bc.p, list_counts, cbytes, hipMemcpyHostToDevice) != hipSuccess) { rc = QMX_ERR_OTHER; break; }
            d_lc = (const uint32_t *)bc.p;
        }
        const bool od = is_device_ptr(out), ocd = is_device_ptr(out_counts);
        if (!od) { if ((rc = bo.reserve(obytes)) != QMX_OK) break; d_out = (qmx_scored_point *)bo.p; }
        if (!ocd) { if ((rc = boc.reserve((size_t)nq * 4)) != QMX_OK) break; d_oc = (uint32_t *)boc.p; }
        if ((rc = launch_merge_points(nullptr, d_lists, d_lc, nullptr, n_lists, nq, k, d_out, d_oc)) != QMX_OK) break;
        if (!od && hipMemcpy(out, d_out, obytes, hipMemcpyDeviceToHost) != hipSuccess) { rc = QMX_ERR_OTHER; break; }
        if (!ocd && hipMemcpy(out_counts, d_oc, (size_t)nq * 4, hipMemcpyDeviceToHost) != hipSuccess) { rc = QMX_ERR_OTHER; break; }
        if (hipDeviceSynchronize() != hipSuccess) rc = QMX_ERR_OTHER;
    } while (0);
    bl.release(); bc.release(); bo.release(); boc.release();
    return rc;
}

int32_t qmx_merge_topk_async(int32_t device_id, void *hip_stream, const qmx_scored_point *lists_dev,
                             const uint32_t *list_counts_dev, const uint32_t *list_idx_base_dev, uint32_t n_lists,
                             uint32_t nq, uint32_t k, qmx_scored_point *out_dev, uint32_t *out_counts_dev) {
    QMX_REQUIRE(lists_dev && out_dev && out_counts_dev, QMX_ERR_BAD_ARG, "NULL argument");
    QMX_REQUIRE(k >= 1 && k <= MAX_TOP, QMX_ERR_NOT_SUPPORTED, "k %u not in 1..%u", k, MAX_TOP);
    QMX_HIP(hipSetDevice(device_id));
    if (nq == 0) return QMX_OK;
    return launch_merge_points((hipStream_t)hip_stream, lists_dev, list_counts_dev, list_idx_base_dev, n_lists, nq, k,
                               out_dev, out_counts_dev);
}


uint64_t qmx_topk_record_bytes(uint32_t nq, uint32_t k) {
    return ((uint64_t)nq * k * sizeof(qmx_scored_point) + (uint64_t)nq * sizeof(uint32_t) + 7) & ~7ull;
}

int32_t qmx_merge_topk_packed_async(int32_t device_id, void *hip_stream, const void *records_dev, const uint32_t *list_idx_base_dev, uint32_t n_lists,
                                    uint32_t nq, uint32_t k, qmx_scored_point *out_dev, uint32_t *out_counts_dev) {
    QMX_REQUIRE(records_dev && out_dev && out_counts_dev, QMX_ERR_BAD_ARG, "NULL argument");
    QMX_REQUIRE(k >= 1 && k <= MAX_TOP, QMX_ERR_NOT_SUPPORTED, "k %u not in 1..%u", k, MAX_TOP);
    QMX_REQUIRE(((uintptr_t)records_dev & 7) == 0, QMX_ERR_BAD_ARG, "records must be 8-byte aligned");
    QMX_HIP(hipSetDevice(device_id));
    if (nq == 0) return QMX_OK;
    const uint64_t rec = qmx_topk_record_bytes(nq, k);
    const qmx_scored_point *lists = (const qmx_scored_point *)records_dev;
    const uint32_t *counts = (const uint32_t *)((const char *)records_dev + (uint64_t)nq * k * sizeof(qmx_scored_point));
    return launch_merge_points((hipStream_t)hip_stream, lists, counts, list_idx_base_dev, n_lists, nq, k, out_dev, out_counts_dev,
                               rec / sizeof(qmx_scored_point), rec / sizeof(uint32_t));
}

int32_t qmx_search_quantized(const qmx_hnsw *g, qmx_query *quantized, qmx_query *raw, const qmx_search_params *p, const uint32_t *ids,
                             uint64_t n_ids, qmx_scored_point *out, uint32_t *out_counts, const volatile uint8_t *is_stopped,
                             qmx_counters *counters) {
    QMX_REFUSE_SPARSE(quantized);
// ... 53 lines not shown
```

qdrant_amd/csrc/common.hpp:

```cpp
#pragma once
#include <hip/hip_runtime.h>
#include <hip/hip_fp16.h>
#include <stdint.h>
#include <atomic>
#include <string>

#include "../../include/qdrant_amd.h"

namespace qmx {

void set_error(const char *fmt, ...);
int32_t hip_status(hipError_t e, const char *what, const char *file, int line);
void clear_stale_error();

enum Option {
    OPT_NO_MFMA_SCAN = 0,
    OPT_NO_MFMA16,
    OPT_NO_PRESCAN,
    OPT_PRESCAN_SHIFT,
    OPT_HNSW_LOG_CAP,
    OPT_NO_SPLIT_SCAN,
    OPT_SPLIT_MIN_QUERIES,
    OPT_NO_SPLIT256,
    OPT_NO_PQ_PAIR,
    OPT_NO_PQ_PREFILTER,
    OPT_PQ_PREFILTER_MIN_QUERIES,
    OPT_HNSW_PQ_PER_CU,
    OPT_TQ_ROTATE_BLOCK,
    OPT_NO_TOPK_SMALL,
    OPT_VERIFY_MAX_PER_QUERY,
    OPT_HNSW_PQ_DIRECT_WALK,
    OPT_HNSW_PQ_TABLE_BUILD,
    OPT_HNSW_NO_PQ_PREFILTER,
    OPT_HNSW_NO_LDS_VISITED,
    OPT_PQ_LUT_NO_LDS,
    OPT_HNSW_PER_CU,
    OPT_HNSW_REFERENCE_HEAP_ORDER,
    OPT_TQ_WIDE_MIN_QUERIES,
    OPT_TQ_WIDE_HIGH_DIGIT,
    OPT_SQ_WIDE_MIN_QUERIES,
    OPT_I8_RESIDENT,
    OPT_DEBUG,
    OPT_COUNT
};
int64_t option(Option o);
struct DeviceOnce {
    std::atomic<uint64_t> done{0};
    int dev = 0;
    bool need() {
        if (hipGetDevice(&dev) != hipSuccess) { dev = 0; return true; }
        return dev >= 64 || !(done.load(std::memory_order_acquire) & (1ull << dev));
    }
    void mark() { if (dev < 64) done.fetch_or(1ull << dev, std::memory_order_release); }
};
void note_kernel(const void *host_function);
#define QMX_NOTE_KERNEL(fn) ::qmx::note_kernel(reinterpret_cast<const void *>(fn))

#define QMX_HIP(expr)                                                        \
    do {                                                                     \
        hipError_t e__ = (expr);                                             \
        if (e__ != hipSuccess) return ::qmx::hip_status(e__, #expr, __FILE__, __LINE__); \
    } while (0)

#define QMX_TRY(expr)                           \
    do {                                        \
        int32_t s__ = (expr);                   \
        if (s__ != QMX_OK) return s__;          \
    } while (0)

#define QMX_REQUIRE(cond, code, ...)            \
    do {                                        \
        if (!(cond)) {                          \
            ::qmx::set_error(__VA_ARGS__);      \
            return (code);                      \
        }                                       \
    } while (0)

#if defined(__HIPCC__)

constexpr int WAVE = 64;

constexpr int DPP_QUAD_XOR1 = 0xB1;
constexpr int DPP_QUAD_XOR2 = 0x4E;
constexpr int DPP_ROW_HALF_MIRROR = 0x141;
constexpr int DPP_QUAD_BCAST0 = 0x00;
constexpr int DPP_QUAD_BCAST1 = 0x55;
constexpr int DPP_QUAD_BCAST2 = 0xAA;
constexpr int DPP_QUAD_BCAST3 = 0xFF;

template <int CTRL>
__device__ __forceinline__ float dpp_f32(float v) {
    return __int_as_float(__builtin_amdgcn_update_dpp(0, __float_as_int(v), CTRL, 0xF, 0xF, true));
}
template <int CTRL>
__device__ __forceinline__ int dpp_i32(int v) {
    return __builtin_amdgcn_update_dpp(0, v, CTRL, 0xF, 0xF, true);
}

__device__ __forceinline__ uint64_t readlane_u64(uint64_t v, int lane_uniform) {
    uint32_t lo = __builtin_amdgcn_readlane((int)(uint32_t)v, lane_uniform);
    uint32_t hi = __builtin_amdgcn_readlane((int)(uint32_t)(v >> 32), lane_uniform);
    return ((uint64_t)hi << 32) | lo;
}
__device__ __forceinline__ uint64_t shfl_up1_u64(uint64_t v) {
    uint32_t lo = __shfl_up((int)(uint32_t)v, 1, 64);
    uint32_t hi = __shfl_up((int)(uint32_t)(v >> 32), 1, 64);
    return ((uint64_t)hi << 32) | lo;
}

__device__ __forceinline__ uint32_t score_to_ord(float s) {
    uint32_t b = __float_as_uint(s);
    if (s != s) return 0xFFFFFFFFu;
    return (b & 0x80000000u) ? ~b : (b | 0x80000000u);
}
__device__ __forceinline__ float ord_to_score(uint32_t o) {
    uint32_t b = (o & 0x80000000u) ? (o & 0x7FFFFFFFu) : ~o;
    return __uint_as_float(b);
}
__device__ __forceinline__ uint64_t make_key(float s, uint32_t idx) {
    return ((uint64_t)score_to_ord(s) << 32) | (uint32_t)(~idx);
}
__device__ __forceinline__ uint32_t key_idx(uint64_t k) { return ~(uint32_t)k; }
__device__ __forceinline__ float key_score(uint64_t k) { return ord_to_score((uint32_t)(k >> 32)); }

// ... 39 lines not shown
```

qdrant_amd/csrc/kernels.hpp:

```cpp
#pragma once
#include "common.hpp"

namespace qmx {

constexpr int MAX_QT = 16;
constexpr int SCAN_BLOCK = 512;
constexpr int MAX_TOP_FAST = 64;

struct TqEc {
    const int16_t *weights;
    const float *xm;
    float weight_scale, mm_const;
};
struct ScanArgs {
    const void *rows;
    uint64_t n_rows;
    uint64_t row_stride;
    uint32_t dim;
    uint32_t nseg;
    uint32_t rem_pieces;
    uint32_t tail_start;
    uint32_t aux_off;
    uint32_t nq;
    const void *queries;
// ... 208 lines not shown
                                uint32_t padded_dim);
int32_t launch_hnsw_build_pq(hipStream_t st, const ScanArgs &a, const HnswBuildArgs &h, int phase, uint32_t grid, int *per_cu);
int32_t launch_hnsw_build_maxsim_pq(hipStream_t st, const ScanArgs &a, const HnswBuildArgs &h, int phase, uint32_t grid, int *per_cu);
int32_t launch_hnsw_build_maxsim_tq(hipStream_t st, const ScanArgs &a, const HnswBuildArgs &h, int phase, uint32_t grid, int *per_cu);
int32_t launch_pq_pair_table(hipStream_t st, uint32_t distance, uint32_t dim, const qmx_pq_params &pq, const float *d_centroids, float *d_pair);
int32_t launch_u8_row_norms(hipStream_t st, const void *rows, uint64_t row_stride, uint64_t n, uint32_t dim, uint32_t flags, float *norms_f, int32_t *norms_i);
constexpr uint32_t HNSW_LDS_QUERY_MAX = 150 * 1024;

int32_t launch_scan_dense(hipStream_t st, int dtype, int distance, int qt, ScanMode mode,
                          const ScanArgs &a, int num_cus, uint32_t *grid_out);
int32_t launch_scan_f32_mfma(hipStream_t st, int qt, ScanMode mode, const ScanArgs &a, int num_cus, uint32_t *grid_out);
bool sq_mfma_ok(uint32_t distance, uint32_t actual_dim);
int32_t launch_scan_sq_mfma(hipStream_t st, int qt, ScanMode mode, const ScanArgs &a, int num_cus, uint32_t *grid_out);
int32_t launch_scan_f16_mfma(hipStream_t st, int qt, ScanMode mode, const ScanArgs &a, int num_cus, uint32_t *grid_out);
struct PairSel {
    const uint32_t *qsel;
    uint32_t per_query;
    const uint32_t *counts;
    const uint32_t *limit;
    __device__ __forceinline__ uint32_t query_of(uint64_t item) const {
        if (qsel) return qsel[item];
        if (per_query) return (uint32_t)(item / per_query);
        return (uint32_t)item;
    }
    __device__ __forceinline__ bool live(uint64_t item, uint32_t qi) const {
        if (limit && item >= (uint64_t)*limit) return false;
        if (per_query && counts) return (uint32_t)(item % per_query) < counts[qi];
        return true;
    }
};

int32_t launch_pairs_dense(hipStream_t st, int dtype, int distance, const ScanArgs &a, const PairSel &sel,
                           uint64_t n_items, int num_cus);
int32_t launch_pairs_sq(hipStream_t st, int distance, const ScanArgs &a, const PairSel &sel, uint64_t n_items, int num_cus);
int32_t launch_scan_sq(hipStream_t st, int distance, int qt, ScanMode mode, const ScanArgs &a, int num_cus,
                       uint32_t *grid_out);
int32_t launch_sq_encode(hipStream_t st, int distance, const qmx_sq_params &sp, uint32_t dim, const float *in, uint64_t n,
                         uint8_t *codes_out, uint64_t codes_stride, float *offsets_out, uint8_t *rows_out, int is_query,
                         uint32_t aux_off);
int32_t launch_sq_split(hipStream_t st, const void *rows, uint64_t row_stride, uint64_t n, uint32_t actual_dim, void *codes,
                        float *offsets);
int32_t launch_sq_gather_rows(hipStream_t st, const void *codes, const float *offsets, uint32_t actual_dim, const uint32_t *ids,
                              uint32_t n, uint64_t n_rows, void *rows_out, int *err_flag);
int32_t launch_sq_internal_query(hipStream_t st, const void *codes, const float *offsets, uint32_t actual_dim, const uint32_t *ids,
                                 uint32_t nq, uint64_t n_rows, float shift, void *tile, uint32_t q_stride, uint32_t aux_off,
                                 int *err_flag);
bool mfma16_dim_ok(int qt, uint32_t dim);
bool mfma16_scan_ok(int qt, ScanMode mode, const ScanArgs &a);
int32_t launch_scan_f32_mfma16(hipStream_t st, int qt, const ScanArgs &a, int num_cus, uint32_t *grid_out);
bool split_scan_ok(const ScanArgs &a);
size_t split_query_bytes(uint32_t dim);
float split_row_scale(float row_maxabs);
int32_t launch_split_row_stats(hipStream_t st, const void *rows, uint64_t row_stride, uint64_t n, uint32_t dim, uint32_t *d_stats);
int32_t launch_split_pack_queries(hipStream_t st, const float *d_q, uint32_t nq, uint32_t dim, float *d_qmax, float *d_qnorm, void *d_bq, int half, uint32_t qt);
int32_t launch_split_thresholds(hipStream_t st, const uint64_t *d_gthr, const float *d_qnorm, const float *d_qmax, uint32_t nq, float rel_band, float row_norm_max,
                                float row_scale, float *d_scales, float *d_thr, float *d_band, uint32_t qt, uint32_t *d_cand_cnt, uint32_t n_cnt);
int32_t launch_scan_f32_split(hipStream_t st, const ScanArgs &a, const void *d_bq, float row_scale, const float *d_scales, const float *d_thr,
                              uint64_t *d_cand, uint32_t *d_cand_cnt, uint32_t cap, int num_cus, const void *d_rows_split, int half, void *d_wlists, uint32_t phase, uint32_t qt);
int32_t launch_regroup_lists(hipStream_t st, const DeletedView &del, const void *d_wlist, const uint32_t *d_wcnt, uint32_t wcap, uint32_t n_lists, uint64_t *d_cand,
                             uint32_t *d_cand_cnt, uint32_t cap, int *d_overflow);
size_t pq_rot_bytes(uint64_t n, uint32_t m);
bool pq_prefilter_shape_ok(uint32_t m, uint32_t ncent);
int32_t launch_pq_rotate(hipStream_t st, const void *codes, uint64_t row_stride, uint64_t n, uint32_t m, void *d_out);
size_t pq_prefilter_table_bytes(uint32_t m, uint32_t nq);
uint32_t pq_prefilter_grid(int num_cus, uint32_t nq, uint32_t *n_slabs_out);
size_t pq_prefilter_wlists_counts_bytes(uint32_t grid);
size_t pq_prefilter_wlists_bytes(uint32_t grid, uint32_t wcap);
int32_t launch_pq_lut8(hipStream_t st, const void *d_luts, uint32_t q_stride, uint32_t nq, uint32_t m, uint32_t ncent, const uint64_t *d_gthr, void *d_table8,
                       int32_t *d_thr, float *d_band);
int32_t launch_pq_prefilter(hipStream_t st, const ScanArgs &a, const void *d_rot, const void *d_table8, const int32_t *d_thr, uint32_t nq, int num_cus,
                            void *d_wlists, uint32_t wcap, uint32_t *grid_out);
int32_t launch_split_refine(hipStream_t st, const uint64_t *d_cand, const uint32_t *d_cand_cnt, uint32_t cap, const float *d_band, uint32_t nq, uint32_t top,
                            const float *d_scales, float *d_thr);
size_t split_wlists_bytes(int num_cus);
int32_t launch_split_regroup(hipStream_t st, const ScanArgs &a, const void *d_wlists, int num_cus, uint64_t *d_cand, uint32_t *d_cand_cnt, uint32_t cap,
                             int *d_overflow, uint32_t phase, uint32_t qt);
size_t split_copy_bytes(uint64_t n, uint32_t dim, int half);
int32_t launch_split_copy(hipStream_t st, const void *rows, uint64_t row_stride, uint64_t n, uint32_t dim, float row_scale, void *d_out, int half);
struct SplitStats {
    unsigned long long candidates;
    unsigned long long verified;
    uint32_t fallback_queries;
    uint32_t pad;
};
struct VerifyPool {
    uint32_t *ids, *qsel, *off, *cnt, *used;
    uint32_t cap;
    uint32_t max_per_query;
};
int32_t launch_split_select(hipStream_t st, const uint64_t *d_cand, const uint32_t *d_cand_cnt, uint32_t cap, const float *d_band, uint32_t nq, uint32_t top,
                            const VerifyPool &pool, uint32_t q_base, const int *d_tile_overflow, uint32_t *d_ovf_q, SplitStats *d_stats,
                            const float *d_t_exact = nullptr, bool tighten = false);
bool split_i8_dim_ok(uint32_t dim);
size_t split_i8_copy_bytes(uint64_t n, uint32_t dim);
size_t split_i8_query_bytes(uint32_t dim);
uint32_t split_i8_probe();
int32_t launch_split_i8_colstats(hipStream_t st, const void *rows, uint64_t row_stride, uint64_t n, uint32_t dim, uint32_t *d_colmax, float *d_colsq);
float split_i8_choose_scales(const float *colmax, const float *colsq, uint64_t n, uint32_t dim, float *scale);
int32_t launch_split_i8_rowstats(hipStream_t st, const void *rows, uint64_t row_stride, uint64_t n, uint32_t dim, const float *d_scale, uint32_t *d_stats);
int32_t launch_split_i8_copy(hipStream_t st, const void *rows, uint64_t row_stride, uint64_t n, uint32_t dim, const float *d_scale, void *d_out);
int32_t launch_split_i8_pack(hipStream_t st, const float *d_q, uint32_t nq, uint32_t dim, const float *d_scale, const uint64_t *d_gthr, const uint32_t *d_row_stats,
                             float row_norm_max, void *d_bq, float *d_qscale, float *d_band, float *d_thr, float *d_t_exact, uint32_t *d_cand_cnt, uint32_t n_cnt);
int32_t launch_scan_i8copy(hipStream_t st, const ScanArgs &a, const void *d_bq, const float *d_qscale, const float *d_thr, int num_cus, const void *d_rows_i8,
                           void *d_wlists, uint32_t phase);
int32_t launch_split_i8_probe(hipStream_t st, const uint64_t *d_cand, const uint32_t *d_cand_cnt, uint32_t cap, const float *d_band, uint32_t nq, uint32_t top,
                              const int *d_tile_overflow, uint32_t *d_probe_ids, uint32_t *d_probe_cnt);
int32_t launch_split_i8_bound(hipStream_t st, const float *d_scores, uint32_t *d_probe_cnt, uint32_t nq, uint32_t top, const float *d_band, const float *d_qscale,
                              float *d_thr, float *d_t_exact);
bool tq4w_shape_ok(const ScanArgs &a);
size_t tq4w_query_bytes(uint32_t code_bytes);
size_t tq4w_wlists_counts_bytes(int num_cus);
size_t tq4w_wlists_bytes(int num_cus);
uint32_t tq4w_wcap();
int32_t launch_tq4w_stats(hipStream_t st, const float *d_sf, const float *d_l2, const void *d_rows, uint64_t row_stride, uint32_t code_bytes, uint64_t n, uint32_t *d_stats);
int32_t launch_tq4w_pack(hipStream_t st, const ScanArgs &a, const uint64_t *d_gthr, float sf_min, float sf_max, float l2_min, float l2_max, uint32_t c1, int high_only,
                         void *d_bq, int32_t *d_thr_i,
                         float *d_qinfo, float *d_band, uint32_t *d_cand_cnt, uint32_t n_cnt);
int32_t launch_scan_tq4w(hipStream_t st, const ScanArgs &a, const void *d_bq, const int32_t *d_thr_i, const float *d_qinfo, const float *d_band_high_only, int num_cus,
                         void *d_wlists, uint32_t *grid_out);
bool sqw_shape_ok(const ScanArgs &a);
size_t sqw_query_bytes(uint32_t dim);
size_t sqw_wlists_counts_bytes(int num_cus);
size_t sqw_wlists_bytes(int num_cus);
uint32_t sqw_wcap();
int32_t launch_sqw_stats(hipStream_t st, const float *d_off, uint64_t n, float multiplier, int32_t *d_bi, uint32_t *d_stats);
int32_t launch_sqw_pack(hipStream_t st, const ScanArgs &a, const uint64_t *d_gthr, float off_absmax, void *d_bq, int32_t *d_thr_i, float *d_qinfo, float *d_band,
                        uint32_t *d_cand_cnt, uint32_t n_cnt);
int32_t launch_scan_sqw(hipStream_t st, const ScanArgs &a, const void *d_bq, const int32_t *d_thr_i, const int32_t *d_bi, const float *d_qinfo, int num_cus,
                        void *d_wlists, uint32_t *grid_out);
int32_t launch_split_plan(hipStream_t st, const uint32_t *d_ovf_q, uint32_t nq, const uint64_t *d_gthr, uint32_t *d_list, uint64_t *d_gthr_packed, uint32_t list_cap,
                          uint32_t *d_count, int *d_run16, int *d_run64, uint32_t n_run64, SplitStats *d_stats, const void *d_queries, uint32_t q_stride,
                          void *d_packed_queries);
int32_t launch_order_statistics_f32(hipStream_t st, const float *d_in, float *d_tmp, uint64_t n, uint64_t lo_pos, uint64_t hi_pos, float *h_out);
int32_t launch_scan_bq(hipStream_t st, int qt, ScanMode mode, const ScanArgs &a, int num_cus, uint32_t *grid_out);
int32_t launch_pairs_bq(hipStream_t st, const ScanArgs &a, const PairSel &sel, uint64_t n_items, int num_cus);
int32_t launch_pairs_tq(hipStream_t st, const ScanArgs &a, const PairSel &sel, uint64_t n_items, int num_cus);
uint64_t bq_row_bytes(uint32_t dim, uint32_t encoding);
int32_t launch_bq_encode_scalar_query(hipStream_t st, const float *d_in, uint32_t nq, uint32_t dim, uint32_t encoding, uint32_t bits, uint8_t *d_out,
                                      uint32_t out_stride, uint32_t qbytes_off, uint32_t aux_off, uint32_t body);
int32_t launch_vector_stats(hipStream_t st, const float *d_rows, uint64_t row_stride_bytes, uint64_t n, uint32_t dim, float *d_min, float *d_max, float *d_mean,
                            float *d_stddev);
int32_t launch_bq_encode(hipStream_t st, const float *d_in, uint64_t n, uint32_t dim, uint32_t encoding, const float *d_mean, const float *d_stddev,
                         uint8_t *d_out, uint64_t out_stride);
int32_t launch_scan_pq(hipStream_t st, ScanMode mode, const ScanArgs &a, int num_cus, uint32_t *grid_out);
int32_t launch_pairs_pq(hipStream_t st, const ScanArgs &a, const PairSel &sel, uint64_t n_items, int num_cus);
int32_t launch_pq_lut(hipStream_t st, uint32_t distance, uint32_t dim, const qmx_pq_params &pq, const float *d_centroids,
                      const float *d_queries, uint32_t nq, float *d_lut);
int32_t launch_pq_internal(hipStream_t st, uint32_t distance, uint32_t dim, const qmx_pq_params &pq, const float *d_centroids,
                           const float *d_pair, const void *rows, uint64_t row_stride, uint64_t n_rows, const uint32_t *a_ids, const uint32_t *b_ids,
                           uint32_t n, float *out, int *err_flag);
int32_t launch_pq_train(hipStream_t st, uint32_t dim, uint32_t chunk_size, uint32_t n_centroids, const float *d_data, uint64_t n,
                        uint32_t max_iters, float accuracy, uint32_t threads, float *d_centroids, uint32_t *iters_host);
int32_t launch_pq_encode(hipStream_t st, uint32_t dim, const qmx_pq_params &pq, const float *d_centroids, const float *d_in,
                         uint64_t n, uint8_t *d_codes);
int32_t launch_pack_queries(hipStream_t st, int dtype, int distance, const void *src, int src_is_encoded,
                            uint32_t src_stride, uint32_t nq, uint32_t dim, void *tile, uint32_t q_stride, uint32_t aux_off);
int32_t launch_merge_keys(hipStream_t st, const uint64_t *partial, uint32_t n_lists,
                          uint32_t qt_stride, uint32_t nq, uint32_t top, qmx_scored_point *out,
                          uint32_t *out_counts, uint32_t out_stride = 0, uint32_t out_offset = 0,
                          uint64_t *next_bound = nullptr, const int *run_if = nullptr, const uint32_t *out_map = nullptr, uint32_t shared_grid = 0);
int32_t launch_merge_points(hipStream_t st, const qmx_scored_point *lists, const uint32_t *list_counts,
                            const uint32_t *list_idx_base, uint32_t n_lists, uint32_t nq, uint32_t k, qmx_scored_point *out,
                            uint32_t *out_counts, uint64_t list_stride = 0, uint64_t count_stride = 0);
int32_t launch_split_candidates(hipStream_t st, const qmx_scored_point *cand, const uint32_t *cand_cnt, uint32_t n_per, uint32_t nq,
                                uint32_t *ids, uint32_t top, qmx_scored_point *out, uint32_t *out_counts);
int32_t launch_sort_scored(hipStream_t st, const float *scores, const uint32_t *ids, const uint32_t *counts, uint32_t n_per_query, uint32_t nq, uint32_t top,
                           qmx_scored_point *out, uint32_t *out_counts, const uint32_t *offsets = nullptr);

int32_t launch_custom_combine(hipStream_t st, const qmx_custom_query *d_queries, uint32_t n_queries, const float *d_sims, uint64_t n,
                              const float *d_coefs, float *d_out);
int32_t launch_maxsim(hipStream_t st, const float *d_sims, uint64_t n_rows, const uint32_t *d_qfirst, uint32_t n_queries, const uint64_t *d_offsets,
                      uint32_t n_points, const uint32_t *d_ids, uint64_t n, float *d_out, int *err_flag);
int32_t launch_custom_topk(hipStream_t st, const float *d_scores, uint64_t n, const uint32_t *d_ids, const DeletedView &del, uint32_t n_queries,
                           uint32_t top, qmx_scored_point *d_out, uint32_t *d_counts, uint64_t *d_bound = nullptr);

int32_t launch_cosine_preprocess_f32(hipStream_t st, const float *in, float *out, uint64_t n, uint32_t dim);
int32_t launch_cast_f32(hipStream_t st, int dst_dtype, const float *in, void *out, uint64_t count);
int32_t launch_minmax_f32(hipStream_t st, const float *in, uint64_t count, float *min_out, float *max_out);
int32_t launch_gather_rows(hipStream_t st, const void *rows, uint64_t row_stride, uint64_t row_bytes,
                           const uint32_t *ids, uint32_t n, uint64_t n_rows, void *out, int *err_flag);

struct SparseRows {
    const uint64_t *off;
    const uint32_t *idx;
    const float *val;
    uint64_t n;
};
// ... 69 lines not shown
```

qdrant_amd/csrc/scan_split.hip:

```cpp
#include <type_traits>

#include "scan_common.hpp"

namespace qmx {

typedef _Float16 half8 __attribute__((ext_vector_type(8)));
typedef _Float16 half4 __attribute__((ext_vector_type(4)));
typedef float f32x4s __attribute__((ext_vector_type(4)));

constexpr int SP_BM = 256;
constexpr int SP_QT = 128;
constexpr int SP_QT_MAX = 256;
constexpr int SP_THREADS = 768;
constexpr int SP_CONSUMERS = 8;
constexpr int SP_A_UNITS = SP_BM * 2 * 4;
constexpr int SP_B_UNITS = SP_QT * 2 * 4;
constexpr int SP_BRING = 4;
constexpr int SP_LDS = (2 * SP_A_UNITS + SP_BRING * SP_B_UNITS) * 16;

__device__ __forceinline__ uint32_t sp_unit(uint32_t t, uint32_t hl, uint32_t kq, uint32_t m) { return ((t * 2 + hl) * 4 + kq) * 16 + (m ^ (2 * kq)); }

__device__ __forceinline__ void sp_split4(const f32x4s v, float scale, half4 &h, half4 &l) {
#pragma unroll
    for (int i = 0; i < 4; ++i) {
// ... 43 lines not shown
    mx = sh[0];
    for (uint32_t w = 1; w < blockDim.x / 64; ++w) mx = __builtin_fmaxf(mx, sh[w]);
    return sp_pow2_scale(mx);
}
__global__ __launch_bounds__(256) void sp_pack_queries_kernel(const float *q, uint32_t nq, uint32_t dim, const float *qmax, uint4 *bq, int half, uint32_t qt) {
    __shared__ float sh_mx[4];
    const float scale = sp_batch_scale(qmax, nq, sh_mx);
    const uint32_t gid = blockIdx.x * blockDim.x + threadIdx.x;
    if (gid >= (dim / 32) * qt * 4) return;
    const uint32_t b_units = qt * 8;
    const uint32_t k32 = gid / (qt * 4), r = gid % (qt * 4);
    const uint32_t nt = r / 64, kq = (r / 16) % 4, n = r % 16;
    const uint32_t qi = nt * 16 + n;
    half8 h, l;
#pragma unroll
    for (int e = 0; e < 8; ++e) {
        const float x = qi < nq ? q[(uint64_t)qi * dim + k32 * 32 + kq * 8 + e] * scale : 0.0f;
        h[e] = (_Float16)x;
        l[e] = (_Float16)(x - (float)h[e]);
    }
    if (half) {
        bq[(uint64_t)(k32 / 2) * b_units + sp_unit(nt, k32 & 1u, kq, n)] = *reinterpret_cast<const uint4 *>(&h);
        return;
    }
    uint4 *chunk = bq + (uint64_t)k32 * b_units;
    chunk[sp_unit(nt, 0, kq, n)] = *reinterpret_cast<const uint4 *>(&h);
    chunk[sp_unit(nt, 1, kq, n)] = *reinterpret_cast<const uint4 *>(&l);
}
__global__ __launch_bounds__(256) void sp_thresholds_kernel(const uint64_t *gthr, const float *qnorm, const float *qmax, uint32_t nq, float rel_band,
                                                            float row_norm_max, float row_scale, float *scales, float *thr, float *band, uint32_t *cand_cnt,
                                                            uint32_t n_cnt) {
    __shared__ float sh_mx[4];
    const float qs = sp_batch_scale(qmax, nq, sh_mx);
    const uint32_t q = threadIdx.x;
    if (q == 0) {
        scales[0] = qs;
        scales[1] = row_scale * qs;
        scales[2] = 1.0f / (row_scale * qs);
    }
    for (uint32_t i = q; i < n_cnt; i += blockDim.x) cand_cnt[i] = 0;
    if (q >= nq) { thr[q] = __builtin_inff(); band[q] = 0.0f; return; }
    const float b = rel_band * row_norm_max * qnorm[q];
    const uint64_t k = gthr[q];
    band[q] = k ? b : __builtin_inff();
    thr[q] = k ? (key_score(k) - b) * (row_scale * qs) : __builtin_inff();
}

typedef __attribute__((address_space(3))) unsigned char sp_lds_byte;
__device__ __forceinline__ void sp_glds16(const unsigned char *src, uint32_t lane_off, uint32_t lds_dst) {
    unsigned keep;
    asm volatile("s_mov_b32 %0, m0\n\ts_mov_b32 m0, %3\n\ts_nop 0\n\tglobal_load_lds_dwordx4 %1, %2\n\ts_mov_b32 m0, %0"
                 : "=&s"(keep) : "v"(lane_off), "s"(src), "s"(lds_dst) : "memory");
}

__device__ __forceinline__ void sp_glds16_nt(const unsigned char *src, uint32_t lane_off, uint32_t lds_dst) {
    unsigned keep;
    asm volatile("s_mov_b32 %0, m0\n\ts_mov_b32 m0, %3\n\ts_nop 0\n\tglobal_load_lds_dwordx4 %1, %2 nt\n\ts_mov_b32 m0, %0"
                 : "=&s"(keep) : "v"(lane_off), "s"(src), "s"(lds_dst) : "memory");
}

__device__ __forceinline__ void sp_glds16_m0(const unsigned char *src, uint32_t lane_off, uint32_t lds_dst) {
    asm volatile("s_mov_b32 m0, %2\n\ts_nop 0\n\tglobal_load_lds_dwordx4 %0, %1" : : "v"(lane_off), "s"(src), "s"(lds_dst) : "memory");
}

__device__ __forceinline__ void sp_glds16_m0_nt(const unsigned char *src, uint32_t lane_off, uint32_t lds_dst) {
    asm volatile("s_mov_b32 m0, %2\n\ts_nop 0\n\tglobal_load_lds_dwordx4 %0, %1 nt" : : "v"(lane_off), "s"(src), "s"(lds_dst) : "memory");
}

struct SplitArgs {
    const uint4 *bq;
    uint32_t nchunks;
    uint32_t nq;
    float row_scale;
    const float *scales;
    const float *thr;
    const uint4 *rows_split;
    uint32_t phase;
    uint4 *wlist;
    uint32_t *wcnt;
    uint32_t wcap;
    uint64_t *cand;
    uint32_t *cand_cnt;
    uint32_t cap;
};

__device__ __forceinline__ void sp_stage_barrier() {
    asm volatile("s_waitcnt lgkmcnt(0)" ::: "memory");
    __builtin_amdgcn_s_barrier();
    asm volatile("" ::: "memory");
}

__global__ __launch_bounds__(SP_THREADS, 1) void scan_f32_split_kernel(const ScanArgs a, const SplitArgs s) {
    extern __shared__ __attribute__((aligned(16))) unsigned char smem_raw[];
    uint4 *lds = reinterpret_cast<uint4 *>(smem_raw);
    const int tid = threadIdx.x, lane = tid & 63;
    const int w = __builtin_amdgcn_readfirstlane(tid >> 6);
    const unsigned char *rows = reinterpret_cast<const unsigned char *>(a.rows);
    const uint64_t n_tiles = (a.n_cand + SP_BM - 1) / SP_BM;
    const uint32_t nch = s.nchunks;
    const uint64_t my_tiles = blockIdx.x < n_tiles ? (n_tiles - blockIdx.x + gridDim.x - 1) / gridDim.x : 0;
    const uint64_t G = my_tiles * nch;
    if (G == 0) return;

    if (w >= SP_CONSUMERS) {
        const uint32_t pw = (uint32_t)w - SP_CONSUMERS;
        const uint32_t p = (uint32_t)lane & 7u, lrow0 = pw * 64u + ((uint32_t)lane >> 3);
        const float rscale = s.row_scale;
        const uint32_t kq_w = p >> 1;
        uint32_t a_wr[2];
#pragma unroll
        for (int e = 0; e < 2; ++e) a_wr[e] = sp_unit(pw * 4u, 0, kq_w, ((uint32_t)lane >> 3) + 8u * (uint32_t)e) * 16u + (p & 1u) * 8u;
        f32x4s areg[3][8];
        typedef const __attribute__((address_space(1))) unsigned char *sp_gptr;
        sp_gptr tile_base = (sp_gptr)(uintptr_t)rows;
        uint32_t voff[8];
        uint64_t ld_g = 0, ld_it = 0;
        uint32_t ld_kc = 0;
        auto set_tile = [&](uint64_t it) {
            const uint64_t tile = blockIdx.x + it * gridDim.x;
            const uint64_t first = tile * SP_BM;
            const uint64_t left = a.n_cand - first;
            const uint64_t tb = (uint64_t)(uintptr_t)(rows + first * a.row_stride);
            tile_base = (sp_gptr)(uintptr_t)(((uint64_t)(uint32_t)__builtin_amdgcn_readfirstlane((int)(uint32_t)(tb >> 32)) << 32) |
                                             (uint32_t)__builtin_amdgcn_readfirstlane((int)(uint32_t)tb));
#pragma unroll
            for (int rr = 0; rr < 8; ++rr) {
                const uint64_t rl = lrow0 + 8u * (uint32_t)rr;
                voff[rr] = (uint32_t)((rl < left ? rl : left - 1) * a.row_stride) + p * 16u;
            }
        };
        auto issue = [&](int slot) {
            if (ld_g >= G) return;
            sp_gptr cb = tile_base + ld_kc * 128u;
#pragma unroll
            for (int rr = 0; rr < 8; ++rr)
                areg[slot][rr] = __builtin_nontemporal_load(reinterpret_cast<const __attribute__((address_space(1))) f32x4s *>(cb + voff[rr]));
            ++ld_g;
            if (++ld_kc == nch) {
                ld_kc = 0;
                ++ld_it;
                if (ld_g < G) set_tile(ld_it);
            }
        };
        auto convert = [&](int slot, uint32_t buf) {
            unsigned char *ab = reinterpret_cast<unsigned char *>(lds + buf * SP_A_UNITS);
#pragma unroll
            for (int rr = 0; rr < 8; ++rr) {
                half4 h, l;
                sp_split4(areg[slot][rr], rscale, h, l);
                const uint32_t off = a_wr[rr & 1] + (uint32_t)(rr >> 1) * (128u * 16u);
                *reinterpret_cast<half4 *>(ab + off) = h;
                *reinterpret_cast<half4 *>(ab + off + 64 * 16) = l;
            }
        };
        set_tile(0);
#pragma unroll
        for (int sl = 0; sl < 3; ++sl) issue(sl);
        convert(0, 0);
        issue(0);
        sp_stage_barrier();
        for (uint64_t g = 0; g < G; g += 6) {
#pragma unroll
            for (int u = 0; u < 6; ++u) {
                if (g + u >= G) break;
                if (g + u + 1 < G) {
                    convert((u + 1) % 3, (uint32_t)(u + 1) & 1u);
// ... 778 lines not shown
constexpr uint32_t SP_I8_PROBE = 64;
constexpr uint32_t SP_I8_MAX_DIM = 4096;

__global__ __launch_bounds__(256) void sp_i8_colmax_kernel(const unsigned char *rows, uint64_t row_stride, uint64_t n, uint32_t dim, uint32_t *colmax, float *colsq) {
    float mx[SP_I8_MAX_DIM / 256], sq[SP_I8_MAX_DIM / 256];
#pragma unroll
    for (int j = 0; j < (int)(SP_I8_MAX_DIM / 256); ++j) { mx[j] = 0.0f; sq[j] = 0.0f; }
    for (uint64_t r = blockIdx.x; r < n; r += gridDim.x) {
        const float *v = reinterpret_cast<const float *>(rows + r * row_stride);
#pragma unroll
        for (int j = 0; j < (int)(SP_I8_MAX_DIM / 256); ++j) {
            const uint32_t c = threadIdx.x + 256u * (uint32_t)j;
            if (c < dim) {
                const float x = v[c];
                mx[j] = __builtin_fmaxf(mx[j], __builtin_fabsf(x));
                sq[j] = __builtin_fmaf(x, x, sq[j]);
            }
        }
    }
#pragma unroll
    for (int j = 0; j < (int)(SP_I8_MAX_DIM / 256); ++j) {
        const uint32_t c = threadIdx.x + 256u * (uint32_t)j;
        if (c < dim) {
            atomicMax(&colmax[c], __float_as_uint(mx[j]));
            atomicAdd(&colsq[c], sq[j]);
        }
    }
}
__device__ __forceinline__ int sp_i8_code(float x, float s) {
    int c = (int)__builtin_rintf(x / s);
    return c > 127 ? 127 : (c < -127 ? -127 : c);
}
__global__ __launch_bounds__(256) void sp_i8_row_stats_kernel(const unsigned char *rows, uint64_t row_stride, uint64_t n, uint32_t dim, const float *scale,
                                                              uint32_t *stats) {
    const int lane = threadIdx.x & 63;
    const uint64_t wave = (uint64_t)blockIdx.x * 4 + (threadIdx.x >> 6), nwaves = (uint64_t)gridDim.x * 4;
    uint32_t m1 = 0, m2 = 0;
    bool bad = false;
    for (uint64_t r = wave; r < n; r += nwaves) {
        const float *v = reinterpret_cast<const float *>(rows + r * row_stride);
        uint32_t c1 = 0, c2 = 0;
        for (uint32_t i = lane; i < dim; i += 64) {
            const float x = v[i];
            bad = bad || !(__builtin_fabsf(x) < __builtin_inff());
            const int c = sp_i8_code(x, scale[i]);
            c1 += (uint32_t)(c < 0 ? -c : c);
            c2 += (uint32_t)(c * c);
        }
        for (int o = 32; o >= 1; o >>= 1) {
            c1 += __shfl_xor(c1, o, 64);
            c2 += __shfl_xor(c2, o, 64);
        }
        m1 = c1 > m1 ? c1 : m1;
        m2 = c2 > m2 ? c2 : m2;
    }
    if (lane == 0) {
        atomicMax(&stats[0], m1);
        atomicMax(&stats[1], m2);
    }
    if (bad) atomicOr(&stats[2], 1u);
}
__global__ __launch_bounds__(256) void sp_i8_copy_kernel(const unsigned char *rows, uint64_t row_stride, uint64_t n, uint32_t dim, const float *scale, uint4 *out) {
    const uint32_t nch = dim / 128;
    const uint64_t n_tiles = (n + SP3_BM - 1) / SP3_BM;
    const uint64_t total = n_tiles * nch * SP3_A_UNITS;
    for (uint64_t gid = (uint64_t)blockIdx.x * 256 + threadIdx.x; gid < total; gid += (uint64_t)gridDim.x * 256) {
        const uint32_t u = (uint32_t)(gid % SP3_A_UNITS);
        const uint64_t blk = gid / SP3_A_UNITS, tile = blk / nch;
        const uint32_t k128 = (uint32_t)(blk % nch);
        const uint32_t kq = (u >> 4) & 3u, hl = (u >> 6) & 1u, t = u >> 7, m = (u & 15u) ^ (2u * kq);
        const uint64_t r = tile * SP3_BM + t * 16u + m;
        const uint32_t g = k128 * 8u + hl * 4u + kq;
        uint32_t w[4] = {0u, 0u, 0u, 0u};
        if (r < n) {
            const float *v = reinterpret_cast<const float *>(rows + r * row_stride) + g * 16;
            const float *sc = scale + g * 16;
#pragma unroll
            for (int e = 0; e < 16; ++e) w[e / 4] |= ((uint32_t)sp_i8_code(v[e], sc[e]) & 0xFFu) << (8 * (e % 4));
        }
        out[gid] = make_uint4(w[0], w[1], w[2], w[3]);
    }
}

__device__ __forceinline__ float sp_block_max(float v, float *sh) {
    for (int o = 32; o >= 1; o >>= 1) v = __builtin_fmaxf(v, __shfl_xor(v, o, 64));
    __syncthreads();
    if ((threadIdx.x & 63) == 0) sh[threadIdx.x >> 6] = v;
    __syncthreads();
    return __builtin_fmaxf(__builtin_fmaxf(sh[0], sh[1]), __builtin_fmaxf(sh[2], sh[3]));
}
__device__ __forceinline__ float sp_block_sum(float v, float *sh) {
    for (int o = 32; o >= 1; o >>= 1) v += __shfl_xor(v, o, 64);
    __syncthreads();
    if ((threadIdx.x & 63) == 0) sh[threadIdx.x >> 6] = v;
    __syncthreads();
    return (sh[0] + sh[1]) + (sh[2] + sh[3]);
}
__global__ __launch_bounds__(256) void sp_i8_pack_kernel(const float *q, uint32_t nq, uint32_t dim, const float *scale, const uint64_t *gthr,
                                                         const uint32_t *row_stats, float row_norm_max, uint4 *bq, float *qscale, float *band, float *thr,
                                                         float *t_exact, uint32_t *cand_cnt, uint32_t n_cnt) {
    extern __shared__ __attribute__((aligned(16))) float sh_q[];
    __shared__ float sh_red[4];
    const uint32_t qi = blockIdx.x;
    const bool live = qi < nq;
    if (qi == 0)
        for (uint32_t i = threadIdx.x; i < n_cnt; i += 256) cand_cnt[i] = 0;
    float mx = 0.0f, ss = 0.0f, bad = 0.0f;
    for (uint32_t i = threadIdx.x; i < dim; i += 256) {
        const float raw = live ? q[(uint64_t)qi * dim + i] : 0.0f;
        const float v = raw * scale[i];
        sh_q[i] = v;
        mx = __builtin_fmaxf(mx, __builtin_fabsf(v));
        ss = __builtin_fmaf(raw, raw, ss);
        if (!(__builtin_fabsf(v) < __builtin_inff())) bad = 1.0f;
    }
    mx = sp_block_max(mx, sh_red);
    ss = sp_block_sum(ss, sh_red);
    bad = sp_block_max(bad, sh_red);
    const float t = mx > 1.0e-30f ? mx / 127.0f : 1.0f;
    float sabs = 0.0f, sf2 = 0.0f;
    for (uint32_t u = threadIdx.x; u < dim / 16; u += 256) {
        const uint32_t k128 = u / 8, hl = (u / 4) & 1u, kq = u % 4;
        uint32_t w[4] = {0u, 0u, 0u, 0u};
#pragma unroll
        for (int e = 0; e < 16; ++e) {
            const float x = sh_q[u * 16 + e] / t;
            float c = __builtin_rintf(x);
            c = c > 127.0f ? 127.0f : (c < -127.0f ? -127.0f : c);
            if (!(c == c)) c = 0.0f;
            const float f = x - c;
            sabs += __builtin_fabsf(c);
            sf2 = __builtin_fmaf(f, f, sf2);
            w[e / 4] |= ((uint32_t)(int)c & 0xFFu) << (8 * (e % 4));
        }
        bq[(uint64_t)k128 * SP_B_UNITS + sp_unit(qi >> 4, hl, kq, qi & 15u)] = make_uint4(w[0], w[1], w[2], w[3]);
    }
    sabs = sp_block_sum(sabs, sh_red);
    sf2 = sp_block_sum(sf2, sh_red);
    if (threadIdx.x != 0) return;
    if (!live) {
        qscale[qi] = 0.0f;
        band[qi] = 0.0f;
        thr[qi] = __builtin_inff();
        t_exact[qi] = -__builtin_inff();
        return;
    }
    const float c1 = (float)row_stats[0], c2 = __builtin_sqrtf((float)row_stats[1]);
    const float cf = __builtin_fminf(0.5f * c1, c2 * __builtin_sqrtf(sf2));
    const float b = t * (cf + 0.5f * sabs + 0.25f * (float)dim) * 1.001f + 2.0f * (float)dim * 1.1920929e-7f * row_norm_max * __builtin_sqrtf(ss);
    const uint64_t k = gthr[qi];
    const bool ok = bad == 0.0f && k != 0 && b < 3.0e38f;
    qscale[qi] = t;
    band[qi] = ok ? b : __builtin_inff();
    t_exact[qi] = ok ? key_score(k) : -__builtin_inff();
    thr[qi] = ok ? (key_score(k) - b) / t : __builtin_inff();
}

constexpr int SP8_BRING = 3;
constexpr int SP8_LDS = (SP3_ARING * SP3_A_UNITS + SP8_BRING * SP_B_UNITS) * 16;
__global__ __launch_bounds__(SP3_THREADS, 1) void scan_i8copy_kernel(const ScanArgs a, const SplitArgs s) {
    extern __shared__ __attribute__((aligned(16))) unsigned char smem_raw[];
    uint4 *lds = reinterpret_cast<uint4 *>(smem_raw);
    const int tid = threadIdx.x, lane = tid & 63;
    const int w = __builtin_amdgcn_readfirstlane(tid >> 6);
    const uint64_t all_tiles = (a.n_cand + SP3_BM - 1) / SP3_BM;
    const uint64_t n_tiles = split_phase_tiles(all_tiles, s.phase);
    const uint32_t nch = s.nchunks;
    const uint64_t my_tiles = blockIdx.x < n_tiles ? (n_tiles - blockIdx.x + gridDim.x - 1) / gridDim.x : 0;
    const uint32_t phase = s.phase & 0xFFu, pstride = split_phase_stride(s.phase);
    auto tile_of = [&](uint64_t j) -> uint64_t { return phase == 0 ? j : phase == 1 ? j * pstride : j + j / (pstride - 1) + 1; };
    if (my_tiles == 0) {
        if (lane == 0) s.wcnt[blockIdx.x * (SP3_THREADS / 64) + (uint32_t)w] = 0;
        return;
    }
    const uint32_t wm = (uint32_t)w & 3u, wn = (uint32_t)w >> 2;
    const uint32_t kq_r = (uint32_t)lane >> 4, m_r = (uint32_t)lane & 15u;
    const uint32_t a_rd = sp_unit(wm * 4, 0, kq_r, m_r), b_rd = sp_unit(wn * 4, 0, kq_r, m_r);
    float thr[4], qs[4];
#pragma unroll
    for (int nt = 0; nt < 4; ++nt) {
        thr[nt] = s.thr[wn * 64 + nt * 16 + m_r];
        qs[nt] = s.scales[wn * 64 + nt * 16 + m_r];
    }
    asm volatile("s_waitcnt vmcnt(0)" ::: "memory");
    const uint32_t lds0 = (uint32_t)(uintptr_t)(sp_lds_byte *)smem_raw;
    const uint32_t lane_off = (uint32_t)lane * 16u;
    uint4 *b_lds = lds + SP3_ARING * SP3_A_UNITS;
    uint64_t ra_it = 0;
    uint32_t ra_kc = 0, ra_slot = 0, rb_kc = 0, rb_slot = 0;
    auto uniform_ptr = [&](uint64_t v) {
        return reinterpret_cast<const unsigned char *>(((uint64_t)(uint32_t)__builtin_amdgcn_readfirstlane((int)(uint32_t)(v >> 32)) << 32) |
                                                       (uint32_t)__builtin_amdgcn_readfirstlane((int)(uint32_t)v));
    };
    const unsigned char *ra_src = nullptr, *rb_src = nullptr;
    uint32_t ra_dst = 0, rb_dst = 0;
    auto rows_begin = [&]() {
        const uint64_t tile = tile_of(blockIdx.x + ra_it * gridDim.x);
        ra_src = uniform_ptr((uint64_t)(uintptr_t)(s.rows_split + (tile * nch + ra_kc) * SP3_A_UNITS) + (uint32_t)w * 4096u);
        ra_dst = lds0 + (ra_slot * SP3_A_UNITS) * 16u + (uint32_t)w * 4096u;
        ra_slot = ra_slot + 1 == SP3_ARING ? 0 : ra_slot + 1;
        if (ra_kc + 1 < nch) ++ra_kc;
        else if (ra_it + 1 < my_tiles) { ra_kc = 0; ++ra_it; }
    };
    auto rows_piece = [&](int i) { sp_glds16_nt(ra_src + i * 1024, lane_off, ra_dst + i * 1024); };
    auto queries_begin = [&]() {
        rb_src = uniform_ptr((uint64_t)(uintptr_t)(s.bq + (uint64_t)rb_kc * SP_B_UNITS) + (uint32_t)w * 2048u);
        rb_dst = lds0 + (SP3_ARING * SP3_A_UNITS + rb_slot * SP_B_UNITS) * 16u + (uint32_t)w * 2048u;
        rb_slot = rb_slot + 1 == SP8_BRING ? 0 : rb_slot + 1;
        rb_kc = rb_kc + 1 == nch ? 0 : rb_kc + 1;
    };
    auto queries_piece = [&](int i) { sp_glds16(rb_src + i * 1024, lane_off, rb_dst + i * 1024); };
    auto request_rows = [&]() {
        rows_begin();
#pragma unroll
        for (int i = 0; i < 4; ++i) rows_piece(i);
    };
    auto request_queries = [&]() {
        queries_begin();
        queries_piece(0);
        queries_piece(1);
    };
    request_queries();
    request_rows();
    request_queries();
    request_rows();
    asm volatile("s_waitcnt vmcnt(6)" ::: "memory");
    sp_stage_barrier();
    uint32_t slot = 0, bslot = 0;
    i32x4s acc[4][4];
    uint4 *const wl = s.wlist + (uint64_t)(blockIdx.x * (SP3_THREADS / 64) + (uint32_t)w) * s.wcap;
    uint32_t wcount = 0;
    auto epilogue = [&](uint64_t tile) {
        const uint32_t row0 = (uint32_t)(tile * SP3_BM) + wm * 64 + 4 * kq_r;
        const uint32_t n_rows32 = (uint32_t)a.n_cand;
        bool hit[4];
        bool maybe = false;
#pragma unroll
        for (int nt = 0; nt < 4; ++nt) {
            int mx = acc[0][nt][0];
#pragma unroll
            for (int mt = 0; mt < 4; ++mt)
#pragma unroll
                for (int j = 0; j < 4; ++j) mx = acc[mt][nt][j] > mx ? acc[mt][nt][j] : mx;
            hit[nt] = !((float)mx < thr[nt]);
            maybe = maybe || hit[nt];
        }
        if (!__ballot(maybe)) return;
#pragma unroll
        for (int nt = 0; nt < 4; ++nt) {
            if (!__ballot(hit[nt])) continue;
            const uint32_t q = wn * 64 + (uint32_t)nt * 16 + m_r;
#pragma unroll
            for (int mt = 0; mt < 4; ++mt) {
                int m4 = acc[mt][nt][0];
#pragma unroll
                for (int j = 1; j < 4; ++j) m4 = acc[mt][nt][j] > m4 ? acc[mt][nt][j] : m4;
                if (!__ballot(!((float)m4 < thr[nt]))) continue;
#pragma unroll
                for (int j = 0; j < 4; ++j) {
                    const float v = (float)acc[mt][nt][j];
                    const uint32_t row = row0 + (uint32_t)mt * 16 + (uint32_t)j;
                    const bool c = !(v < thr[nt]) && row < n_rows32 && q < s.nq;
                    const uint64_t hits = __ballot(c);
                    if (hits) {
                        const uint32_t at = wcount + __builtin_amdgcn_mbcnt_hi((uint32_t)(hits >> 32), __builtin_amdgcn_mbcnt_lo((uint32_t)hits, 0u));
                        if (c && at < s.wcap) {
                            const uint64_t key = make_key(v * qs[nt], row);
                            wl[at] = make_uint4((uint32_t)key, (uint32_t)(key >> 32), q, 0u);
                        }
                        wcount += (uint32_t)__builtin_popcountll(hits);
                    }
                }
            }
        }
    };
    for (uint64_t it = 0; it < my_tiles; ++it) {
        if (it) epilogue(tile_of(blockIdx.x + (it - 1) * gridDim.x));
#pragma unroll
        for (int mt = 0; mt < 4; ++mt)
#pragma unroll
            for (int nt = 0; nt < 4; ++nt) acc[mt][nt] = (i32x4s){0, 0, 0, 0};
        for (uint32_t kc = 0; kc < nch; ++kc) {
            queries_begin();
            rows_begin();
            const uint4 *ab = lds + slot * SP3_A_UNITS + a_rd;
            const uint4 *bb = b_lds + bslot * SP_B_UNITS + b_rd;
            i32x4s b0[4], b1[4];
#pragma unroll
            for (int nt = 0; nt < 4; ++nt) {
                b0[nt] = *reinterpret_cast<const i32x4s *>(bb + nt * 128);
                b1[nt] = *reinterpret_cast<const i32x4s *>(bb + nt * 128 + 64);
            }
#pragma unroll
            for (int mt = 0; mt < 4; ++mt) {
                const i32x4s a0 = *reinterpret_cast<const i32x4s *>(ab + mt * 128);
                const i32x4s a1 = *reinterpret_cast<const i32x4s *>(ab + mt * 128 + 64);
#pragma unroll
                for (int nt = 0; nt < 4; ++nt) acc[mt][nt] = __builtin_amdgcn_mfma_i32_16x16x64_i8(a1, b1[nt], acc[mt][nt], 0, 0, 0);
                if (mt == 0) queries_piece(0);
                if (mt == 1) queries_piece(1);
                if (mt == 2) { rows_piece(0); rows_piece(1); }
                if (mt == 3) { rows_piece(2); rows_piece(3); }
                __builtin_amdgcn_sched_barrier(0);
#pragma unroll
                for (int nt = 0; nt < 4; ++nt) acc[mt][nt] = __builtin_amdgcn_mfma_i32_16x16x64_i8(a0, b0[nt], acc[mt][nt], 0, 0, 0);
            }
            slot = slot + 1 == SP3_ARING ? 0 : slot + 1;
            bslot = bslot + 1 == SP8_BRING ? 0 : bslot + 1;
            asm volatile("s_waitcnt vmcnt(6)" ::: "memory");
            sp_stage_barrier();
        }
    }
    epilogue(tile_of(blockIdx.x + (my_tiles - 1) * gridDim.x));
    if (lane == 0) s.wcnt[blockIdx.x * (SP3_THREADS / 64) + (uint32_t)w] = wcount;
    asm volatile("s_waitcnt vmcnt(0)" ::: "memory");
}


constexpr uint32_t SP8R_MAX_NCH = 8;
__host__ __device__ constexpr size_t sp8r_lds_bytes(uint32_t nch) { return (size_t)nch * SP_B_UNITS * 16 + 2 * SP_QT * 4; }
template <int OFF>
__device__ __forceinline__ void sp_gload16(i32x4s &dst, const unsigned char *sbase, uint32_t voff) {
    asm volatile("global_load_dwordx4 %0, %1, %2 offset:%3 nt" : "=v"(dst) : "v"(voff), "s"(sbase), "n"(OFF) : "memory");
}
template <int I, int N, class F>
__device__ __forceinline__ void sp_static_for(F &&f) {
    if constexpr (I < N) {
        f(std::integral_constant<int, I>{});
        sp_static_for<I + 1, N>(f);
    }
}
template <int AHEAD>
__global__ __launch_bounds__(SP3_THREADS, 1) void scan_i8copy_kernel_res(const ScanArgs a, const SplitArgs s) {
    constexpr int SLOTS = AHEAD + 1, WAVES = SP3_THREADS / 64, THREADS = SP3_THREADS, MT = 2, NL = 2 * MT;
    static_assert(SP3_BM == WAVES * MT * 16, "a wave owns two row tiles of a 256-row tile");
    static_assert(NL * AHEAD <= 62, "vmcnt is six bits");
    extern __shared__ __attribute__((aligned(16))) unsigned char smem_raw[];
    uint4 *lds = reinterpret_cast<uint4 *>(smem_raw);
    const int tid = threadIdx.x, lane = tid & 63;
    const int w = __builtin_amdgcn_readfirstlane(tid >> 6);
    const uint64_t all_tiles = (a.n_cand + SP3_BM - 1) / SP3_BM;
    const uint64_t n_tiles = split_phase_tiles(all_tiles, s.phase);
    const uint32_t nch = s.nchunks;
    const uint64_t my_tiles = blockIdx.x < n_tiles ? (n_tiles - blockIdx.x + gridDim.x - 1) / gridDim.x : 0;
    const uint32_t phase = s.phase & 0xFFu, pstride = split_phase_stride(s.phase);
    auto tile_of = [&](uint64_t j) -> uint64_t { return phase == 0 ? j : phase == 1 ? j * pstride : j + j / (pstride - 1) + 1; };
    if (my_tiles == 0) {
        if (lane == 0) s.wcnt[blockIdx.x * WAVES + (uint32_t)w] = 0;
        return;
    }
    const uint32_t ws = (uint32_t)w;
    auto my_tile = [&](uint64_t i) -> uint64_t { return tile_of(blockIdx.x + i * gridDim.x); };
    float *thr_lds = reinterpret_cast<float *>(smem_raw + (size_t)nch * SP_B_UNITS * 16), *qs_lds = thr_lds + SP_QT;
#pragma unroll 4
    for (uint32_t u = (uint32_t)tid; u < nch * SP_B_UNITS; u += THREADS) lds[u] = s.bq[u];
    for (int u = tid; u < SP_QT; u += THREADS) {
        thr_lds[u] = s.thr[u];
        qs_lds[u] = s.scales[u];
    }
    __syncthreads();
    asm volatile("s_waitcnt vmcnt(0) lgkmcnt(0)" ::: "memory");
    const uint32_t kq_r = (uint32_t)lane >> 4, m_r = (uint32_t)lane & 15u;
    const uint32_t lane_unit = kq_r * 16u + (m_r ^ (2u * kq_r));
    const uint4 *const b_rd = lds + lane_unit;
    const uint32_t lane_off = lane_unit * 16u;
    auto uniform_ptr = [&](uint64_t v) {
        return reinterpret_cast<const unsigned char *>(((uint64_t)(uint32_t)__builtin_amdgcn_readfirstlane((int)(uint32_t)(v >> 32)) << 32) |
                                                       (uint32_t)__builtin_amdgcn_readfirstlane((int)(uint32_t)v));
    };
    auto load_stage = [&](uint64_t tile, uint32_t kc, i32x4s (&rc)[NL]) __attribute__((always_inline)) {
        const unsigned char *src = uniform_ptr((uint64_t)(uintptr_t)(s.rows_split + (tile * nch + kc) * SP3_A_UNITS) + ws * (NL * 1024u));
        sp_gload16<0>(rc[0], src, lane_off);
        sp_gload16<1024>(rc[1], src, lane_off);
        sp_gload16<2048>(rc[2], src, lane_off);
        sp_gload16<3072>(rc[3], src, lane_off);
    };
    i32x4s acc[MT][8];
    uint4 *const wl = s.wlist + (uint64_t)(blockIdx.x * WAVES + (uint32_t)w) * s.wcap;
    uint32_t wcount = 0;
    const uint32_t n_rows32 = (uint32_t)a.n_cand;
    auto epilogue = [&](uint64_t tile) __attribute__((always_inline)) {
        const uint32_t row0 = (uint32_t)(tile * SP3_BM) + ws * (MT * 16u) + 4 * kq_r;
        uint32_t hits8 = 0;
#pragma unroll
        for (int nt = 0; nt < 8; ++nt) {
            int mx = acc[0][nt][0];
#pragma unroll
            for (int mt = 0; mt < MT; ++mt)
#pragma unroll
                for (int j = 0; j < 4; ++j) mx = acc[mt][nt][j] > mx ? acc[mt][nt][j] : mx;
            if (!((float)mx < thr_lds[nt * 16 + (int)m_r])) hits8 |= 1u << nt;
        }
        if (!__ballot(hits8 != 0)) return;
#pragma unroll
        for (int nt = 0; nt < 8; ++nt) {
            if (!__ballot((hits8 >> nt) & 1u)) continue;
            const uint32_t q = (uint32_t)nt * 16 + m_r;
            const float th = thr_lds[q], qs = qs_lds[q];
#pragma unroll
            for (int mt = 0; mt < MT; ++mt) {
#pragma unroll
                for (int j = 0; j < 4; ++j) {
                    const float v = (float)acc[mt][nt][j];
                    const uint32_t row = row0 + (uint32_t)mt * 16 + (uint32_t)j;
                    const bool c = !(v < th) && row < n_rows32 && q < s.nq;
                    const uint64_t hits = __ballot(c);
                    if (hits) {
                        const uint32_t at = wcount + __builtin_amdgcn_mbcnt_hi((uint32_t)(hits >> 32), __builtin_amdgcn_mbcnt_lo((uint32_t)hits, 0u));
                        if (c && at < s.wcap) {
                            const uint64_t key = make_key(v * qs, row);
                            wl[at] = make_uint4((uint32_t)key, (uint32_t)(key >> 32), q, 0u);
                        }
                        wcount += (uint32_t)__builtin_popcountll(hits);
                    }
                }
            }
        }
    };
    const uint64_t n_stages = my_tiles * nch;
    uint64_t itr = 0, tile_r = my_tile(0);
    uint32_t kr = 0;
    auto advance_r = [&]() {
        if (kr + 1 < nch) ++kr;
        else if (itr + 1 < my_tiles) { kr = 0; ++itr; tile_r = my_tile(itr); }
    };
    i32x4s rc[SLOTS][NL];
    sp_static_for<0, AHEAD>([&](auto DC) __attribute__((always_inline)) {
        load_stage(tile_r, kr, rc[decltype(DC)::value]);
        advance_r();
    });
    uint64_t it = 0, tile_c = my_tile(0), tile_done = 0;
    uint32_t kc = 0;
    auto one_stage = [&](auto IC) __attribute__((always_inline)) {
        constexpr int I = decltype(IC)::value, IL = (I + AHEAD) % SLOTS;
        if (kc == 0) {
            if (it) epilogue(tile_done);
#pragma unroll
            for (int mt = 0; mt < MT; ++mt)
#pragma unroll
                for (int nt = 0; nt < 8; ++nt) acc[mt][nt] = (i32x4s){0, 0, 0, 0};
        }
        load_stage(tile_r, kr, rc[IL]);
        advance_r();
        asm volatile("s_waitcnt vmcnt(%0)" : : "n"(NL * AHEAD) : "memory");
        asm volatile("" : "+v"(rc[I][0]), "+v"(rc[I][1]), "+v"(rc[I][2]), "+v"(rc[I][3]) : : "memory");
#pragma unroll
        for (int hl = 0; hl < 2; ++hl) {
            const uint4 *bb = b_rd + kc * SP_B_UNITS + hl * 64;
            constexpr int RA = 3;
            i32x4s bv[RA + 1];
#pragma unroll
            for (int k = 0; k < RA; ++k) bv[k] = *reinterpret_cast<const i32x4s *>(bb + k * 128);
#pragma unroll
            for (int nt = 0; nt < 8; ++nt) {
                if (nt + RA < 8) bv[(nt + RA) % (RA + 1)] = *reinterpret_cast<const i32x4s *>(bb + (nt + RA) * 128);
#pragma unroll
                for (int mt = 0; mt < MT; ++mt) acc[mt][nt] = __builtin_amdgcn_mfma_i32_16x16x64_i8(rc[I][mt * 2 + hl], bv[nt % (RA + 1)], acc[mt][nt], 0, 0, 0);
                __builtin_amdgcn_sched_barrier(0);
            }
        }
        if (++kc == nch) {
            kc = 0;
            tile_done = tile_c;
            if (++it < my_tiles) tile_c = my_tile(it);
        }
    };
    for (uint64_t g = 0; g < n_stages; g += SLOTS) {
        sp_static_for<0, SLOTS>([&](auto IC) __attribute__((always_inline)) {
            if (g + decltype(IC)::value < n_stages) one_stage(IC);
        });
    }
    asm volatile("s_waitcnt vmcnt(0)" ::: "memory");
    epilogue(tile_done);
    if (lane == 0) s.wcnt[blockIdx.x * WAVES + (uint32_t)w] = wcount;
    asm volatile("s_waitcnt vmcnt(0)" ::: "memory");
}

__global__ __launch_bounds__(SEL_BLOCK) void sp_i8_probe_kernel(const uint64_t *cand, const uint32_t *cand_cnt, uint32_t cap, const float *band,
                                                                const int *tile_overflow, uint32_t top, uint32_t *probe_ids, uint32_t *probe_cnt) {
    __shared__ SelShared sel_sh;
    uint64_t (*const sh)[WAVE] = sel_sh.sh;
    SelScratch &scratch = sel_sh.scratch;
    __shared__ uint64_t sh_kth;
    __shared__ uint32_t sh_n;
    const uint32_t q = blockIdx.x;
    const uint32_t raw = cand_cnt[q];
    if (*tile_overflow || raw > cap || raw == 0 || !(band[q] < 3.0e38f)) {
        if (threadIdx.x == 0) probe_cnt[q] = 0;
        return;
    }
    const uint64_t *c = cand + (uint64_t)q * cap;
    const uint32_t k = top < SP_I8_PROBE ? top : SP_I8_PROBE;
    const uint32_t want = raw < k ? raw : k;
    if (threadIdx.x == 0) sh_n = 0;
    if (raw <= (uint32_t)SEL_SURV) block_kth_key_ranked(c, raw, want, &scratch, &sh_kth);
    else block_kth_key(c, raw, (int)want, sh, &sh_kth);
    const uint64_t kth = sh_kth;
    for (uint32_t base = 0; base < raw; base += SEL_BLOCK) {
        const uint32_t i = base + threadIdx.x;
        if (i < raw) {
            const uint64_t key = c[i];
            if (kth != 0 && key >= kth) {
                const uint32_t slot = atomicAdd(&sh_n, 1u);
                if (slot < SP_I8_PROBE) probe_ids[(uint64_t)q * SP_I8_PROBE + slot] = key_idx(key);
            }
        }
    }
    __syncthreads();
    if (threadIdx.x == 0) probe_cnt[q] = sh_n < SP_I8_PROBE ? sh_n : SP_I8_PROBE;
}
__global__ __launch_bounds__(64) void sp_i8_bound_kernel(const float *scores, uint32_t *probe_cnt, uint32_t top, const float *band, const float *qscale,
                                                         float *thr, float *t_exact) {
    const uint32_t q = blockIdx.x;
    const int lane = threadIdx.x;
    const uint32_t n = probe_cnt[q];
    const float sc = (uint32_t)lane < n ? scores[(uint64_t)q * SP_I8_PROBE + lane] : -__builtin_inff();
    uint32_t rank = 0;
    for (int j = 0; j < 64; ++j) {
        const float o = __shfl(sc, j, 64);
        rank += (o > sc || (o == sc && j < lane)) ? 1u : 0u;
    }
    if (lane == 0) probe_cnt[q] = 0;
    if (n < top || !(band[q] < 3.0e38f)) return;
    if ((uint32_t)lane < n && rank == top - 1 && sc == sc) {
        if (sc > t_exact[q]) t_exact[q] = sc;
        const float t = (sc - band[q]) / qscale[q];
        if (t > thr[q]) thr[q] = t;
    }
// ... 152 lines not shown
    hipLaunchKernelGGL(sp_plan_kernel, dim3(1), dim3(256), 0, st, d_ovf_q, nq, d_gthr, d_list, d_gthr_packed, list_cap, d_count, d_run16, d_run64, n_run64, d_stats,
                       (const uint4 *)d_queries, q_stride / 16, (uint4 *)d_packed_queries);
    QMX_HIP(hipGetLastError());
    return QMX_OK;
}

bool split_i8_dim_ok(uint32_t dim) { return dim % 128 == 0 && dim >= 128 && dim <= SP_I8_MAX_DIM; }
size_t split_i8_copy_bytes(uint64_t n, uint32_t dim) { return (size_t)((n + SP3_BM - 1) / SP3_BM) * (dim / 128) * SP3_A_UNITS * 16; }
size_t split_i8_query_bytes(uint32_t dim) { return (size_t)(dim / 128) * SP_B_UNITS * 16; }
uint32_t split_i8_probe() { return SP_I8_PROBE; }
int32_t launch_split_i8_colstats(hipStream_t st, const void *rows, uint64_t row_stride, uint64_t n, uint32_t dim, uint32_t *d_colmax, float *d_colsq) {
    QMX_REQUIRE(split_i8_dim_ok(dim), QMX_ERR_BAD_ARG, "int8 copy of dim %u", dim);
    ::qmx::clear_stale_error();
    QMX_HIP(hipMemsetAsync(d_colmax, 0, (size_t)dim * 4, st));
    QMX_HIP(hipMemsetAsync(d_colsq, 0, (size_t)dim * 4, st));
    if (n) hipLaunchKernelGGL(sp_i8_colmax_kernel, dim3(2048), dim3(256), 0, st, (const unsigned char *)rows, row_stride, n, dim, d_colmax, d_colsq);
    QMX_HIP(hipGetLastError());
    return QMX_OK;
}
float split_i8_choose_scales(const float *colmax, const float *colsq, uint64_t n, uint32_t dim, float *scale) {
    std::vector<double> s0(dim), sig(dim);
    double wmax = 0.0;
    for (uint32_t i = 0; i < dim; ++i) {
        s0[i] = colmax[i] > 1.0e-30f ? (double)colmax[i] / 127.0 : 1.0;
        sig[i] = n ? sqrt((double)colsq[i] / (double)n) : 0.0;
        if (!(sig[i] < 1.0e30)) sig[i] = 0.0;
        wmax = std::max(wmax, sig[i] * s0[i]);
    }
    auto scales_of = [&](double G, std::vector<double> &s) {
        for (uint32_t i = 0; i < dim; ++i) {
            const double w = sig[i] * s0[i];
            s[i] = (w > 0.0 && wmax / G > w && colmax[i] > 1.0e-30f) ? s0[i] * (wmax / G / w) : s0[i];
        }
    };
    auto predicted = [&](const std::vector<double> &s) {
        double vmax = 0.0, vsum = 0.0, c2 = 0.0;
        for (uint32_t i = 0; i < dim; ++i) {
            const double v = sig[i] * s[i];
            vmax = std::max(vmax, v);
            vsum += v;
            c2 += (sig[i] / s[i]) * (sig[i] / s[i]);
        }
        const double t = 3.0 * vmax / 127.0;
        if (!(t > 0.0)) return 0.0;
        double f2 = 0.0;
        for (uint32_t i = 0; i < dim; ++i) f2 += std::min(1.0 / 12.0, (sig[i] * s[i] / t) * (sig[i] * s[i] / t));
        return 0.4 * vsum + t * sqrt(c2) * sqrt(f2);
    };
    static const double grid[] = {1.0e30, 64.0, 45.0, 32.0, 23.0, 16.0, 11.0, 8.0, 5.6, 4.0, 2.8, 2.0};
    std::vector<double> s(dim), best(dim);
    double best_b = 0.0, best_g = grid[0];
    for (size_t k = 0; k < sizeof(grid) / sizeof(grid[0]); ++k) {
        scales_of(grid[k], s);
        const double b = predicted(s);
        if (k == 0 || b < best_b * 0.98) {
            best_b = b;
            best_g = grid[k];
            best = s;
        }
    }
    for (uint32_t i = 0; i < dim; ++i) {
        float f = (float)best[i];
        const float floor_s = colmax[i] > 1.0e-30f ? colmax[i] / 127.0f : 1.0f;
        scale[i] = f >= floor_s ? f : floor_s;
    }
    return best_g >= 1.0e29 ? 0.0f : (float)best_g;
}
int32_t launch_split_i8_rowstats(hipStream_t st, const void *rows, uint64_t row_stride, uint64_t n, uint32_t dim, const float *d_scale, uint32_t *d_stats) {
    QMX_REQUIRE(split_i8_dim_ok(dim), QMX_ERR_BAD_ARG, "int8 copy of dim %u", dim);
    ::qmx::clear_stale_error();
    QMX_HIP(hipMemsetAsync(d_stats, 0, 16, st));
    if (n) hipLaunchKernelGGL(sp_i8_row_stats_kernel, dim3(2048), dim3(256), 0, st, (const unsigned char *)rows, row_stride, n, dim, d_scale, d_stats);
    QMX_HIP(hipGetLastError());
    return QMX_OK;
}
int32_t launch_split_i8_copy(hipStream_t st, const void *rows, uint64_t row_stride, uint64_t n, uint32_t dim, const float *d_scale, void *d_out) {
    if (n == 0) return QMX_OK;
    ::qmx::clear_stale_error();
    hipLaunchKernelGGL(sp_i8_copy_kernel, dim3(8192), dim3(256), 0, st, (const unsigned char *)rows, row_stride, n, dim, d_scale, (uint4 *)d_out);
    QMX_HIP(hipGetLastError());
    return QMX_OK;
}
int32_t launch_split_i8_pack(hipStream_t st, const float *d_q, uint32_t nq, uint32_t dim, const float *d_scale, const uint64_t *d_gthr, const uint32_t *d_row_stats,
                             float row_norm_max, void *d_bq, float *d_qscale, float *d_band, float *d_thr, float *d_t_exact, uint32_t *d_cand_cnt, uint32_t n_cnt) {
    QMX_REQUIRE(nq <= (uint32_t)SP_QT, QMX_ERR_BAD_ARG, "int8 tile of %u queries", nq);
    ::qmx::clear_stale_error();
    hipLaunchKernelGGL(sp_i8_pack_kernel, dim3(SP_QT), dim3(256), (size_t)dim * 4, st, d_q, nq, dim, d_scale, d_gthr, d_row_stats, row_norm_max, (uint4 *)d_bq,
                       d_qscale, d_band, d_thr, d_t_exact, d_cand_cnt, n_cnt);
    QMX_HIP(hipGetLastError());
    return QMX_OK;
}
int32_t launch_scan_i8copy(hipStream_t st, const ScanArgs &a, const void *d_bq, const float *d_qscale, const float *d_thr, int num_cus, const void *d_rows_i8,
                           void *d_wlists, uint32_t phase) {
    const uint32_t nch_r = a.dim / 128;
    const bool resident = option(OPT_I8_RESIDENT) > 0 && nch_r <= SP8R_MAX_NCH;
    void (*kfn)(const ScanArgs, const SplitArgs) = resident ? scan_i8copy_kernel_res<1> : scan_i8copy_kernel;
    const size_t lds_bytes = resident ? sp8r_lds_bytes(nch_r) : (size_t)SP8_LDS;
    static thread_local DeviceOnce attr_once;
    if (attr_once.need()) {
        QMX_HIP(hipFuncSetAttribute(reinterpret_cast<const void *>(scan_i8copy_kernel), hipFuncAttributeMaxDynamicSharedMemorySize, SP8_LDS));
        QMX_HIP(hipFuncSetAttribute(reinterpret_cast<const void *>(scan_i8copy_kernel_res<1>), hipFuncAttributeMaxDynamicSharedMemorySize, (int)sp8r_lds_bytes(SP8R_MAX_NCH)));
        attr_once.mark();
    }
    QMX_REQUIRE(d_rows_i8 && d_wlists && split_i8_dim_ok(a.dim), QMX_ERR_BAD_ARG, "the int8 scan reads the int8 copy and writes per-wave candidate lists");
    SplitArgs s;
    s.rows_split = (const uint4 *)d_rows_i8;
    s.bq = (const uint4 *)d_bq;
    s.nchunks = a.dim / 128;
    s.nq = a.nq;
    s.row_scale = 1.0f;
    s.scales = d_qscale;
    s.thr = d_thr;
    s.cand = nullptr;
    s.cand_cnt = nullptr;
    s.cap = 0;
    s.wcap = SP_WCAP;
    s.wcnt = (uint32_t *)d_wlists;
    s.wlist = (uint4 *)((unsigned char *)d_wlists + split_wlists_counts_bytes(num_cus));
    s.phase = phase;
    const uint64_t n_tiles = split_phase_tiles((a.n_cand + SP3_BM - 1) / SP3_BM, phase);
    if (n_tiles == 0) return QMX_OK;
    const uint32_t grid = (uint32_t)std::max<uint64_t>(1, std::min<uint64_t>(n_tiles, (uint64_t)num_cus));
    ::qmx::clear_stale_error();
    QMX_NOTE_KERNEL(kfn);
    hipLaunchKernelGGL(kfn, dim3(grid), dim3(SP3_THREADS), lds_bytes, st, a, s);
    QMX_HIP(hipGetLastError());
    return QMX_OK;
}
int32_t launch_split_i8_probe(hipStream_t st, const uint64_t *d_cand, const uint32_t *d_cand_cnt, uint32_t cap, const float *d_band, uint32_t nq, uint32_t top,
                              const int *d_tile_overflow, uint32_t *d_probe_ids, uint32_t *d_probe_cnt) {
    ::qmx::clear_stale_error();
    hipLaunchKernelGGL(sp_i8_probe_kernel, dim3(nq), dim3(SEL_BLOCK), 0, st, d_cand, d_cand_cnt, cap, d_band, d_tile_overflow, top, d_probe_ids, d_probe_cnt);
    QMX_HIP(hipGetLastError());
    return QMX_OK;
}
int32_t launch_split_i8_bound(hipStream_t st, const float *d_scores, uint32_t *d_probe_cnt, uint32_t nq, uint32_t top, const float *d_band, const float *d_qscale,
                              float *d_thr, float *d_t_exact) {
    ::qmx::clear_stale_error();
    hipLaunchKernelGGL(sp_i8_bound_kernel, dim3(nq), dim3(64), 0, st, d_scores, d_probe_cnt, top, d_band, d_qscale, d_thr, d_t_exact);
    QMX_HIP(hipGetLastError());
    return QMX_OK;
}

}
```

qdrant_amd/scorer.py:

```python
import ctypes as C
import enum
import os
from typing import Iterable, List, Optional, Sequence

import numpy as np

from . import _ffi as F


class Distance(enum.IntEnum):
    Cosine = F.COSINE
    Euclid = F.EUCLID
    Dot = F.DOT
    Manhattan = F.MANHATTAN


class VectorStorageDatatype(enum.IntEnum):
    Float32 = F.DTYPE_F32
    Float16 = F.DTYPE_F16
    Uint8 = F.DTYPE_U8


ScoredPointOffset = np.dtype([("idx", np.uint32), ("score", np.float32)])

# ... 575 lines not shown
        self.nq = nq

    def set_filter(self, allowed=None):
        if allowed is None:
            F.check(F.lib().qmx_query_set_filter(self._h, None, 0))
            return
        words = _bits_to_words(np.asarray(allowed, dtype=bool))
        F.check(F.lib().qmx_query_set_filter(self._h, F.ptr(words), len(allowed)))

    def score_points(self, points: Sequence[int]) -> np.ndarray:
        ids = np.ascontiguousarray(points, dtype=np.uint32)
        scores = np.empty((self.nq, len(ids)), dtype=np.float32)
        F.check(F.lib().qmx_score_points(self._h, F.ptr(ids), len(ids), F.ptr(scores), None))
        return scores

    def score_point(self, point: int, query_index: int = 0) -> float:
        out = C.c_float()
        F.check(F.lib().qmx_score_point(self._h, query_index, int(point), C.byref(out)))
        return out.value

    def score_internal(self, point_a, point_b) -> np.ndarray:
        a = np.ascontiguousarray(np.atleast_1d(point_a), dtype=np.uint32)
        b = np.ascontiguousarray(np.atleast_1d(point_b), dtype=np.uint32)
        out = np.empty(len(a), dtype=np.float32)
        F.check(F.lib().qmx_score_internal(self.storage._h, F.ptr(a), F.ptr(b), len(a), F.ptr(out)))
        return out

    def score_points_ragged(self, ids_per_query: Sequence[Sequence[int]]) -> List[np.ndarray]:
        assert len(ids_per_query) == self.nq
        lens = [len(x) for x in ids_per_query]
        offsets = np.zeros(self.nq + 1, dtype=np.uint32)
        offsets[1:] = np.cumsum(lens)
        ids = (np.concatenate([np.asarray(x, dtype=np.uint32) for x in ids_per_query])
               if offsets[-1] else np.zeros(0, dtype=np.uint32))
        scores = np.empty(int(offsets[-1]), dtype=np.float32)
        F.check(F.lib().qmx_score_points_ragged(self._h, F.ptr(ids), F.ptr(offsets), F.ptr(scores), None))
        return [scores[offsets[i]:offsets[i + 1]] for i in range(self.nq)]

    def score_bytes(self, rows) -> np.ndarray:
        rows = np.ascontiguousarray(rows)
        n = rows.shape[0]
        stride = rows.strides[0]
        scores = np.empty((self.nq, n), dtype=np.float32)
        F.check(F.lib().qmx_score_bytes(self._h, F.ptr(rows), n, stride, F.ptr(scores)))
        return scores

    def rescore(self, ids, top: int, counts=None) -> List[np.ndarray]:
        ids = np.ascontiguousarray(ids, dtype=np.uint32)
        assert ids.ndim == 2 and ids.shape[0] == self.nq
        cnt = None if counts is None else np.ascontiguousarray(counts, dtype=np.uint32)
        out = np.zeros((self.nq, top), dtype=ScoredPointOffset)
        oc = np.zeros(self.nq, dtype=np.uint32)
        F.check(F.lib().qmx_rescore(self._h, F.ptr(ids), F.ptr(cnt), ids.shape[1], top, F.ptr(out), F.ptr(oc)))
        return [out[i, :oc[i]].copy() for i in range(self.nq)]

    def encoded_query(self, query_index: int = 0) -> np.ndarray:
        if isinstance(self.storage, EncodedVectorsPQ):
            qz = self.storage.quantizer
            out = np.empty((qz.m, qz.n_centroids), dtype=np.float32)
            F.check(F.lib().qmx_query_read_encoded(self._h, query_index, F.ptr(out), out.nbytes, None))
            return out
        if isinstance(self.storage, EncodedVectorsBin):
            qz = self.storage.quantizer
            planes = {0: 1, 1: 4, 2: 8}[qz.query_encoding] if not getattr(self, "_internal", False) else 1
            out = np.empty(qz.quantized_vector_size() * planes, dtype=np.uint8)
            F.check(F.lib().qmx_query_read_encoded(self._h, query_index, F.ptr(out), out.nbytes, None))
            return out
        if isinstance(self.storage, EncodedVectorsU8):
            nbytes = 4 + self.storage.quantizer.actual_dim
            out = np.empty(nbytes, dtype=np.uint8)
            F.check(F.lib().qmx_query_read_encoded(self._h, query_index, F.ptr(out), nbytes, None))
            return out
        nbytes = self.storage.dim * np.dtype(_NP_ELEM[int(self.storage.datatype)]).itemsize
        out = np.empty(nbytes, dtype=np.uint8)
        written = C.c_uint64()
        F.check(F.lib().qmx_query_read_encoded(self._h, query_index, F.ptr(out), nbytes, C.byref(written)))
        return out[:written.value].view(_NP_ELEM[int(self.storage.datatype)])

    def last_counters(self) -> "F.Counters":
        c = F.Counters()
        F.check(F.lib().qmx_query_last_counters(self._h, C.byref(c)))
        return c

    def close(self):
        if self._h:
            F.lib().qmx_query_destroy(self._h)
            self._h = C.c_void_p()

    def __del__(self):
        try:
            self.close()
        except Exception:
            pass


def new_raw_scorer(query, storage: VectorStorage) -> RawScorer:
    if isinstance(storage, SparseVectorStorage):
        return storage._raw_scorer(query)
    if hasattr(query, "data_ptr") and getattr(query, "is_cuda", False):
        q = query
        assert q.dim() == 2 and q.is_contiguous() and str(q.dtype) == "torch.float32"
    else:
        q = np.ascontiguousarray(np.atleast_2d(query), dtype=np.float32)
    if q.shape[1] != storage.dim:
        raise ValueError(f"query dim {q.shape[1]} != storage dim {storage.dim}")
    h = C.c_void_p()
    F.check(F.lib().qmx_query_create(storage._h, F.ptr(q), q.shape[0], C.byref(h)))
    return RawScorer(h, storage, q.shape[0])


def new_raw_scorer_internal(point_ids, storage: VectorStorage) -> RawScorer:
    ids = np.ascontiguousarray(np.atleast_1d(point_ids), dtype=np.uint32)
    h = C.c_void_p()
    F.check(F.lib().qmx_query_create_internal(storage._h, F.ptr(ids), len(ids), C.byref(h)))
    scorer = RawScorer(h, storage, len(ids))
    scorer._internal = True
    return scorer


def _is_sparse_example(v) -> bool:
    return isinstance(v, (tuple, list)) and len(v) == 2 and np.ndim(v[0]) == 1 and np.ndim(v[1]) == 1


class CustomQuery:

    def __init__(self, kind: int, examples, n_a: int, n_b: int, coefs=None):
        examples = list(examples)
        kinds = {_is_sparse_example(v) for v in examples}
        if len(kinds) > 1:
            raise ValueError("a custom query mixes dense and sparse examples")
        self.sparse = kinds.pop() if kinds else None
        if self.sparse:
            examples = [(np.asarray(ix, dtype=np.uint32), np.asarray(vx, dtype=np.float32)) for ix, vx in examples]
        else:
            examples = [np.asarray(v, dtype=np.float32) for v in examples]
        self.kind, self.examples, self.n_a, self.n_b = kind, examples, n_a, n_b
        self.coefs = None if coefs is None else np.asarray(coefs, dtype=np.float32)

    @classmethod
    def recommend_best_score(cls, positives, negatives):
        return cls(F.CUSTOM_RECO_BEST_SCORE, list(positives) + list(negatives), len(positives), len(negatives))

    @classmethod
    def recommend_sum_scores(cls, positives, negatives):
        return cls(F.CUSTOM_RECO_SUM_SCORES, list(positives) + list(negatives), len(positives), len(negatives))

    @classmethod
    def discover(cls, target, pairs):
        return cls(F.CUSTOM_DISCOVER, [target] + [v for p in pairs for v in p], 1, len(pairs))

    @classmethod
    def context(cls, pairs):
        return cls(F.CUSTOM_CONTEXT, [v for p in pairs for v in p], 0, len(pairs))

    @classmethod
    def feedback_naive(cls, target, feedback, a: float, b: float, c: float, margin: float = 0.0):
        pairs, coefs = [], [np.float32(a)]
        for i, (pv, ps) in enumerate(feedback):
            for j, (nv, ns) in enumerate(feedback):
                if i == j:
                    continue
                confidence = np.float32(ps) - np.float32(ns)
                if confidence <= np.float32(margin):
                    continue
                pairs.append((pv, nv))
                coefs.append(np.float32(np.power(confidence, np.float32(b), dtype=np.float32) * np.float32(c)))
# ... 205 lines not shown
```

Baseline: 97590.

## Add in-kernel int8 threshold ladder to merge two-phase scan into one launch

Adds a per-query histogram ladder of witness scores that the resident int8 scan kernel updates atomically. Whenever a level holds at least top-k witnesses, the kernel raises the pruning threshold on the fly, and other waves periodically refresh the threshold in LDS. This replaces the two-phase scan with probe/bound passes by a single launch, removing kernel launches and the second pass. The cost is atomics, extra epilogue work, and more LDS. The feature is gated behind a new i8_ladder option, and a stats API is added.

```diff
diff --git a/include/qdrant_amd.h b/include/qdrant_amd.h
--- a/include/qdrant_amd.h
+++ b/include/qdrant_amd.h
@@ -241,6 +241,13 @@
                                       uint64_t n_ids, qmx_scored_point *out_dev,
                                       uint32_t *out_counts_dev);
 QMX_API int32_t qmx_query_last_counters(qmx_query *q, qmx_counters *out);
+typedef struct qmx_prefilter_stats {
+    uint32_t passes;
+    uint32_t scan_launches;
+    uint32_t threshold_raises;
+    uint32_t reserved;
+} qmx_prefilter_stats;
+QMX_API int32_t qmx_query_last_prefilter_stats(qmx_query *q, qmx_prefilter_stats *out);
 
 QMX_API int32_t qmx_rescore(qmx_query *q, const uint32_t *ids, const uint32_t *counts,
                             uint32_t n_per_query, uint32_t top, qmx_scored_point *out,
diff --git a/qdrant_amd/_ffi.py b/qdrant_amd/_ffi.py
--- a/qdrant_amd/_ffi.py
+++ b/qdrant_amd/_ffi.py
@@ -32,6 +32,10 @@
     _fields_ = [("vectors_scored", C.c_uint64), ("bytes_read", C.c_uint64), ("kernel_launches", C.c_uint64),
                 ("kernel_ms", C.c_float), ("reserved", C.c_float),
                 ("prefilter_candidates", C.c_uint64), ("verified_rows", C.c_uint64), ("fallback_queries", C.c_uint32), ("prefilter_queries", C.c_uint32)]
+
+
+class PrefilterStats(C.Structure):
+    _fields_ = [("passes", C.c_uint32), ("scan_launches", C.c_uint32), ("threshold_raises", C.c_uint32), ("reserved", C.c_uint32)]
 
 
 class SqParams(C.Structure):
@@ -179,6 +183,7 @@
     "qmx_search_topk": (C.c_int32, [_P, C.c_uint32, _P, C.c_uint64, _P, _P, _P, C.POINTER(Counters)]),
     "qmx_search_topk_async": (C.c_int32, [_P, C.c_uint32, _P, C.c_uint64, _P, _P]),
     "qmx_query_last_counters": (C.c_int32, [_P, C.POINTER(Counters)]),
+    "qmx_query_last_prefilter_stats": (C.c_int32, [_P, C.POINTER(PrefilterStats)]),
     "qmx_rescore": (C.c_int32, [_P, _P, _P, C.c_uint32, C.c_uint32, _P, _P]),
     "qmx_search_quantized": (C.c_int32, [_P, _P, _P, C.POINTER(SearchParams), _P, C.c_uint64, _P, _P, _P, C.POINTER(Counters)]),
     "qmx_custom_score_points": (C.c_int32, [_P, _P, C.c_uint32, _P, C.c_uint32, _P]),
diff --git a/qdrant_amd/csrc/api_core.hip b/qdrant_amd/csrc/api_core.hip
--- a/qdrant_amd/csrc/api_core.hip
+++ b/qdrant_amd/csrc/api_core.hip
@@ -29,7 +29,7 @@
     }
 }
 
-static const char *const g_option_names[OPT_COUNT] = {"no_mfma_scan", "no_mfma16", "no_prescan", "prescan_shift", "hnsw_log_cap", "no_split_scan", "split_min_queries", "no_split256", "no_pq_pair", "no_pq_prefilter", "pq_prefilter_min_queries", "hnsw_pq_per_cu", "tq_rotate_block", "no_topk_small", "verify_max_per_query", "hnsw_pq_direct_walk", "hnsw_pq_table_build", "hnsw_no_pq_prefilter", "hnsw_no_lds_visited", "pq_lut_no_lds", "hnsw_per_cu", "hnsw_reference_heap_order", "tq_wide_min_queries", "tq_wide_high_digit", "sq_wide_min_queries", "i8_resident", "debug"};
+static const char *const g_option_names[OPT_COUNT] = {"no_mfma_scan", "no_mfma16", "no_prescan", "prescan_shift", "hnsw_log_cap", "no_split_scan", "split_min_queries", "no_split256", "no_pq_pair", "no_pq_prefilter", "pq_prefilter_min_queries", "hnsw_pq_per_cu", "tq_rotate_block", "no_topk_small", "verify_max_per_query", "hnsw_pq_direct_walk", "hnsw_pq_table_build", "hnsw_no_pq_prefilter", "hnsw_no_lds_visited", "pq_lut_no_lds", "hnsw_per_cu", "hnsw_reference_heap_order", "tq_wide_min_queries", "tq_wide_high_digit", "sq_wide_min_queries", "i8_resident", "i8_ladder", "debug"};
 struct OptionTable {
     std::atomic<int64_t> v[OPT_COUNT];
     int64_t initial[OPT_COUNT];
diff --git a/qdrant_amd/csrc/api_internal.hpp b/qdrant_amd/csrc/api_internal.hpp
--- a/qdrant_amd/csrc/api_internal.hpp
+++ b/qdrant_amd/csrc/api_internal.hpp
@@ -164,6 +164,7 @@
     DevBuf sp_plan, sp_fq;
     qmx_counters last_counters{};
     bool last_split = false, last_pq = false;
+    uint32_t last_scan_launches = 0, last_scan_passes = 0;
     uint32_t last_fqt = 64;
     uint64_t last_row_bytes = 0, last_n_cand = 0;
     uint64_t sp_sample_n = 0, sp_sample_of = 0;
diff --git a/qdrant_amd/csrc/api_search.hip b/qdrant_amd/csrc/api_search.hip
--- a/qdrant_amd/csrc/api_search.hip
+++ b/qdrant_amd/csrc/api_search.hip
@@ -63,6 +63,7 @@
     float *band = (float *)q->sp_f32.p;
     q->last_counters = qmx_counters{};
     q->last_split = false;
+    q->last_scan_launches = q->last_scan_passes = 0;
     const int sshift = (int)std::min<int64_t>(std::max<int64_t>(option(OPT_PRESCAN_SHIFT) - 2, 1), 20);
     const uint64_t S = std::min<uint64_t>(n_cand, std::max<uint64_t>(n_cand >> sshift, 8192));
     if (q->sp_sample_n != S || q->sp_sample_of != n_cand) {
@@ -184,6 +185,7 @@
     int32_t *thr_i = (int32_t *)(qinfo + 768);
     q->last_counters = qmx_counters{};
     q->last_split = false;
+    q->last_scan_launches = q->last_scan_passes = 0;
     const int sshift = (int)std::min<int64_t>(std::max<int64_t>(option(OPT_PRESCAN_SHIFT) - (sq ? 2 : 3), 1), 20);
     const uint64_t S = std::min<uint64_t>(n_cand, std::max<uint64_t>(n_cand >> sshift, 8192));
     if (q->sp_sample_n != S || q->sp_sample_of != n_cand) {
@@ -347,11 +349,12 @@
     VerifyPool vp{};
     q->last_counters = qmx_counters{};
     q->last_split = false;
+    q->last_scan_launches = q->last_scan_passes = 0;
     if (split) {
         QMX_TRY(q->sp_bq.reserve(split_query_bytes(s->dim)));
         QMX_TRY(q->sp_f32.reserve(1280 * sizeof(float)));
         QMX_TRY(q->sp_cand.reserve((size_t)split_qt * SPLIT_CAND_CAP * sizeof(uint64_t)));
-        QMX_TRY(q->sp_cnt.reserve((size_t)SPLIT_QT_MAX * 4));
+        QMX_TRY(q->sp_cnt.reserve(((size_t)SPLIT_QT_MAX + (s->split_i8 ? split_i8_ladder_words() : 0)) * 4));
         if (s->d_rows_split) QMX_TRY(q->sp_wl.reserve(split_wlists_bytes(s->num_cus)));
         QMX_TRY(q->sp_plan.reserve(pl.bytes));
         QMX_TRY(verify_pool(q, (unsigned char *)q->sp_plan.p, &vp));
@@ -395,18 +398,22 @@
             QMX_TRY(split_stage(q, "prescan"));
             if (s->split_i8) {
                 float *sp_texact = sp_qnorm, *sp_qscale = sp_qmax;
+                const bool ladder_on = split_i8_ladder_ok(s->dim);
+                I8Ladder ladder{(uint32_t *)q->sp_cnt.p + SPLIT_QT_MAX, sp_texact, sp_band, &((SplitStats *)plan)->ladder_raises};
                 QMX_TRY(launch_split_i8_pack(q->stream, (const float *)q->enc.p + (size_t)tile0 * s->dim, nq_tile, s->dim, s->d_i8_scale, gthr, s->d_i8_stats,
-                                             s->row_norm_max, q->sp_bq.p, sp_qscale, sp_band, sp_thr, sp_texact, (uint32_t *)q->sp_cnt.p, SPLIT_QT_MAX));
+                                             s->row_norm_max, q->sp_bq.p, sp_qscale, sp_band, sp_thr, sp_texact, (uint32_t *)q->sp_cnt.p, SPLIT_QT_MAX,
+                                             ladder_on ? ladder.words : nullptr));
                 QMX_TRY(split_stage(q, "int8 pack"));
                 const uint32_t np = split_i8_probe();
                 uint32_t *probe_ids = (uint32_t *)q->sp_probe.p, *probe_cnt = probe_ids + (size_t)q->nq * np;
                 int *tile_ovf = (int *)(plan + pl.tile_ovf) + split_tiles.size();
                 const uint32_t sstride = 16;
-                for (uint32_t ph = 1; ph <= 2; ++ph) {
+                for (uint32_t ph = ladder_on ? 0 : 1; ph <= (ladder_on ? 0u : 2u); ++ph) {
                     const uint32_t phase = ph | (sstride << 8);
                     size_t slot = 0;
                     if (timed) QMX_TRY(timing_begin(q, &slot));
-                    QMX_TRY(launch_scan_i8copy(q->stream, a, q->sp_bq.p, sp_qscale, sp_thr, s->num_cus, s->d_rows_split, q->sp_wl.p, phase));
+                    QMX_TRY(launch_scan_i8copy(q->stream, a, q->sp_bq.p, sp_qscale, sp_thr, s->num_cus, s->d_rows_split, q->sp_wl.p, phase,
+                                               ladder_on ? &ladder : nullptr));
                     q->last_kernel = last_noted_kernel();
                     if (timed) QMX_TRY(timing_end(q, slot));
                     QMX_TRY(launch_split_regroup(q->stream, a, q->sp_wl.p, s->num_cus, (uint64_t *)q->sp_cand.p, (uint32_t *)q->sp_cnt.p, SPLIT_CAND_CAP, tile_ovf,
@@ -420,12 +427,14 @@
                     QMX_TRY(launch_split_i8_bound(q->stream, (const float *)q->sp_pscores.p + (size_t)tile0 * np, probe_cnt + tile0, nq_tile, top, sp_band, sp_qscale,
                                                   sp_thr, sp_texact));
                 }
-                QMX_TRY(split_stage(q, "int8 scan"));
+                q->last_scan_launches += ladder_on ? 1 : 2;
+                q->last_scan_passes += 1;
+                QMX_TRY(split_stage(q, ladder_on ? "int8 scan (ladder: one launch)" : "int8 scan (two launches)"));
                 QMX_TRY(launch_split_select(q->stream, (const uint64_t *)q->sp_cand.p, (const uint32_t *)q->sp_cnt.p, SPLIT_CAND_CAP, sp_band, nq_tile, top, vp, tile0,
                                             tile_ovf, (uint32_t *)(plan + pl.ovf_q) + tile0, (SplitStats *)plan, sp_texact));
                 QMX_TRY(split_stage(q, "select"));
                 split_tiles.push_back({tile0, nq_tile});
-                if (counters) counters->kernel_launches += 13;
+                if (counters) counters->kernel_launches += ladder_on ? 8 : 13;
                 continue;
             }
             const float row_scale = split_row_scale(s->row_maxabs);
@@ -652,6 +661,20 @@
     return fold_split_counters(q, out);
 }
 
+int32_t qmx_query_last_prefilter_stats(qmx_query *q, qmx_prefilter_stats *out) {
+    QMX_REQUIRE(q && out, QMX_ERR_BAD_ARG, "NULL argument");
+    QMX_HIP(hipSetDevice(q->device));
+    QMX_HIP(hipStreamSynchronize(q->stream));
+    *out = qmx_prefilter_stats{};
+    if (!q->last_split || !q->sp_plan.p || !q->last_scan_passes) return QMX_OK;
+    SplitStats st;
+    QMX_HIP(hipMemcpy(&st, q->sp_plan.p, sizeof(st), hipMemcpyDeviceToHost));
+    out->passes = q->last_scan_passes;
+    out->scan_launches = q->last_scan_launches;
+    out->threshold_raises = st.ladder_raises;
+    return QMX_OK;
+}
+
 int32_t qmx_search_topk_async(qmx_query *q, uint32_t top, const uint32_t *ids, uint64_t n_ids,
                               qmx_scored_point *out_dev, uint32_t *out_counts_dev) {
     QMX_REQUIRE(q && out_dev && out_counts_dev, QMX_ERR_BAD_ARG, "NULL argument");
diff --git a/qdrant_amd/csrc/common.hpp b/qdrant_amd/csrc/common.hpp
--- a/qdrant_amd/csrc/common.hpp
+++ b/qdrant_amd/csrc/common.hpp
@@ -40,6 +40,7 @@
     OPT_TQ_WIDE_HIGH_DIGIT,
     OPT_SQ_WIDE_MIN_QUERIES,
     OPT_I8_RESIDENT,
+    OPT_I8_LADDER,
     OPT_DEBUG,
     OPT_COUNT
 };
diff --git a/qdrant_amd/csrc/kernels.hpp b/qdrant_amd/csrc/kernels.hpp
--- a/qdrant_amd/csrc/kernels.hpp
+++ b/qdrant_amd/csrc/kernels.hpp
@@ -314,7 +314,10 @@
     unsigned long long verified;
     uint32_t fallback_queries;
     uint32_t pad;
-};
+    uint32_t ladder_raises;
+    uint32_t pad2;
+};
+static_assert(sizeof(SplitStats) == 32, "SplitPlanLayout::count sits behind SplitStats");
 struct VerifyPool {
     uint32_t *ids, *qsel, *off, *cnt, *used;
     uint32_t cap;
@@ -332,9 +335,17 @@
 int32_t launch_split_i8_rowstats(hipStream_t st, const void *rows, uint64_t row_stride, uint64_t n, uint32_t dim, const float *d_scale, uint32_t *d_stats);
 int32_t launch_split_i8_copy(hipStream_t st, const void *rows, uint64_t row_stride, uint64_t n, uint32_t dim, const float *d_scale, void *d_out);
 int32_t launch_split_i8_pack(hipStream_t st, const float *d_q, uint32_t nq, uint32_t dim, const float *d_scale, const uint64_t *d_gthr, const uint32_t *d_row_stats,
-                             float row_norm_max, void *d_bq, float *d_qscale, float *d_band, float *d_thr, float *d_t_exact, uint32_t *d_cand_cnt, uint32_t n_cnt);
+                             float row_norm_max, void *d_bq, float *d_qscale, float *d_band, float *d_thr, float *d_t_exact, uint32_t *d_cand_cnt, uint32_t n_cnt,
+                             uint32_t *d_ladder = nullptr);
+struct I8Ladder {
+    uint32_t *words;
+    const float *t0, *band;
+    uint32_t *raises;
+};
+size_t split_i8_ladder_words();
+bool split_i8_ladder_ok(uint32_t dim);
 int32_t launch_scan_i8copy(hipStream_t st, const ScanArgs &a, const void *d_bq, const float *d_qscale, const float *d_thr, int num_cus, const void *d_rows_i8,
-                           void *d_wlists, uint32_t phase);
+                           void *d_wlists, uint32_t phase, const I8Ladder *ladder = nullptr);
 int32_t launch_split_i8_probe(hipStream_t st, const uint64_t *d_cand, const uint32_t *d_cand_cnt, uint32_t cap, const float *d_band, uint32_t nq, uint32_t top,
                               const int *d_tile_overflow, uint32_t *d_probe_ids, uint32_t *d_probe_cnt);
 int32_t launch_split_i8_bound(hipStream_t st, const float *d_scores, uint32_t *d_probe_cnt, uint32_t nq, uint32_t top, const float *d_band, const float *d_qscale,
diff --git a/qdrant_amd/csrc/scan_split.hip b/qdrant_amd/csrc/scan_split.hip
--- a/qdrant_amd/csrc/scan_split.hip
+++ b/qdrant_amd/csrc/scan_split.hip
@@ -149,6 +149,11 @@
     uint64_t *cand;
     uint32_t *cand_cnt;
     uint32_t cap;
+    uint32_t *lad_thr = nullptr;
+    uint32_t *lad_cnt = nullptr;
+    const float *lad_t0 = nullptr;
+    const float *lad_band = nullptr;
+    uint32_t *lad_raises = nullptr;
 };
 
 __device__ __forceinline__ void sp_stage_barrier() {
@@ -1093,6 +1098,8 @@
     }
 }
 
+constexpr uint32_t SP_LAD_LEVELS = 64;
+constexpr float SP_LAD_STEP = 0.5f;
 __device__ __forceinline__ float sp_block_max(float v, float *sh) {
     for (int o = 32; o >= 1; o >>= 1) v = __builtin_fmaxf(v, __shfl_xor(v, o, 64));
     __syncthreads();
@@ -1109,13 +1116,15 @@
 }
 __global__ __launch_bounds__(256) void sp_i8_pack_kernel(const float *q, uint32_t nq, uint32_t dim, const float *scale, const uint64_t *gthr,
                                                          const uint32_t *row_stats, float row_norm_max, uint4 *bq, float *qscale, float *band, float *thr,
-                                                         float *t_exact, uint32_t *cand_cnt, uint32_t n_cnt) {
+                                                         float *t_exact, uint32_t *cand_cnt, uint32_t n_cnt,
+                                                         uint32_t *ladder ) {
     extern __shared__ __attribute__((aligned(16))) float sh_q[];
     __shared__ float sh_red[4];
     const uint32_t qi = blockIdx.x;
     const bool live = qi < nq;
     if (qi == 0)
         for (uint32_t i = threadIdx.x; i < n_cnt; i += 256) cand_cnt[i] = 0;
+    if (ladder && threadIdx.x < SP_LAD_LEVELS) ladder[SP_QT + qi * SP_LAD_LEVELS + threadIdx.x] = 0;
     float mx = 0.0f, ss = 0.0f, bad = 0.0f;
     for (uint32_t i = threadIdx.x; i < dim; i += 256) {
         const float raw = live ? q[(uint64_t)qi * dim + i] : 0.0f;
@@ -1154,6 +1163,7 @@
         band[qi] = 0.0f;
         thr[qi] = __builtin_inff();
         t_exact[qi] = -__builtin_inff();
+        if (ladder) ladder[qi] = score_to_ord(__builtin_inff());
         return;
     }
     const float c1 = (float)row_stats[0], c2 = __builtin_sqrtf((float)row_stats[1]);
@@ -1165,6 +1175,7 @@
     band[qi] = ok ? b : __builtin_inff();
     t_exact[qi] = ok ? key_score(k) : -__builtin_inff();
     thr[qi] = ok ? (key_score(k) - b) / t : __builtin_inff();
+    if (ladder) ladder[qi] = score_to_ord(thr[qi]);
 }
 
 constexpr int SP8_BRING = 3;
@@ -1329,7 +1340,7 @@
 
 
 constexpr uint32_t SP8R_MAX_NCH = 8;
-__host__ __device__ constexpr size_t sp8r_lds_bytes(uint32_t nch) { return (size_t)nch * SP_B_UNITS * 16 + 2 * SP_QT * 4; }
+__host__ __device__ constexpr size_t sp8r_lds_bytes(uint32_t nch) { return (size_t)nch * SP_B_UNITS * 16 + 4 * SP_QT * 4; }
 template <int OFF>
 __device__ __forceinline__ void sp_gload16(i32x4s &dst, const unsigned char *sbase, uint32_t voff) {
     asm volatile("global_load_dwordx4 %0, %1, %2 offset:%3 nt" : "=v"(dst) : "v"(voff), "s"(sbase), "n"(OFF) : "memory");
@@ -1341,6 +1352,7 @@
         sp_static_for<I + 1, N>(f);
     }
 }
+__device__ __forceinline__ float sp_lad_level(float t0, float delta, int j) { return __builtin_fmaf((float)(j + 1), delta, t0); }
 template <int AHEAD>
 __global__ __launch_bounds__(SP3_THREADS, 1) void scan_i8copy_kernel_res(const ScanArgs a, const SplitArgs s) {
     constexpr int SLOTS = AHEAD + 1, WAVES = SP3_THREADS / 64, THREADS = SP3_THREADS, MT = 2, NL = 2 * MT;
@@ -1363,11 +1375,15 @@
     const uint32_t ws = (uint32_t)w;
     auto my_tile = [&](uint64_t i) -> uint64_t { return tile_of(blockIdx.x + i * gridDim.x); };
     float *thr_lds = reinterpret_cast<float *>(smem_raw + (size_t)nch * SP_B_UNITS * 16), *qs_lds = thr_lds + SP_QT;
+    float *band_lds = qs_lds + SP_QT, *t0_lds = band_lds + SP_QT;
+    const bool lad = s.lad_thr != nullptr;
 #pragma unroll 4
     for (uint32_t u = (uint32_t)tid; u < nch * SP_B_UNITS; u += THREADS) lds[u] = s.bq[u];
     for (int u = tid; u < SP_QT; u += THREADS) {
-        thr_lds[u] = s.thr[u];
+        thr_lds[u] = lad ? ord_to_score(__hip_atomic_load(&s.lad_thr[u], __ATOMIC_RELAXED, __HIP_MEMORY_SCOPE_AGENT)) : s.thr[u];
         qs_lds[u] = s.scales[u];
+        band_lds[u] = lad ? s.lad_band[u] : 0.0f;
+        t0_lds[u] = lad ? s.lad_t0[u] : 0.0f;
     }
     __syncthreads();
     asm volatile("s_waitcnt vmcnt(0) lgkmcnt(0)" ::: "memory");
@@ -1390,6 +1406,43 @@
     uint4 *const wl = s.wlist + (uint64_t)(blockIdx.x * WAVES + (uint32_t)w) * s.wcap;
     uint32_t wcount = 0;
     const uint32_t n_rows32 = (uint32_t)a.n_cand;
+    auto witness = [&](bool w_ok, uint32_t q, uint32_t row, float x, float th, float qs, float bd) __attribute__((always_inline)) {
+        const float t0 = t0_lds[q], delta = SP_LAD_STEP * bd;
+        int j = -1;
+        if (w_ok && delta > 0.0f && bd < 3.0e38f && t0 > -__builtin_inff()) {
+            const float f = (x - t0) / delta;
+            if (f >= 1.0f) {
+                j = f >= (float)SP_LAD_LEVELS ? (int)SP_LAD_LEVELS - 1 : (int)f - 1;
+                if (!(x >= sp_lad_level(t0, delta, j))) --j;
+                if (j >= 0 && !(x >= sp_lad_level(t0, delta, j))) j = -1;
+            }
+            if (j >= 0 && !((sp_lad_level(t0, delta, j) - bd) / qs > th)) j = -1;
+            if (j >= 0 && !a.del.live(row)) j = -1;
+        }
+        if (j >= 0) __hip_atomic_fetch_add(&s.lad_cnt[q * SP_LAD_LEVELS + (uint32_t)j], 1u, __ATOMIC_RELAXED, __HIP_MEMORY_SCOPE_AGENT);
+        uint64_t wm = __ballot(j >= 0);
+        while (wm) {
+            const int src = __builtin_ctzll(wm);
+            wm &= wm - 1;
+            const uint32_t qq = (uint32_t)__builtin_amdgcn_readlane((int)q, src);
+            uint32_t sfx = __hip_atomic_load(&s.lad_cnt[qq * SP_LAD_LEVELS + (uint32_t)lane], __ATOMIC_RELAXED, __HIP_MEMORY_SCOPE_AGENT);
+#pragma unroll
+            for (int o = 1; o < 64; o <<= 1) {
+                const uint32_t up = (uint32_t)__shfl_down((int)sfx, o, 64);
+                sfx += lane + o < 64 ? up : 0u;
+            }
+            const uint64_t reached = __ballot(sfx >= a.top);
+            if (reached && lane == src) {
+                const int best = 63 - __builtin_clzll(reached);
+                const float t_new = (sp_lad_level(t0, delta, best) - bd) / qs;
+                if (t_new > th) {
+                    const uint32_t img = score_to_ord(t_new);
+                    if (__hip_atomic_fetch_max(&s.lad_thr[qq], img, __ATOMIC_RELAXED, __HIP_MEMORY_SCOPE_AGENT) < img)
+                        __hip_atomic_fetch_add(s.lad_raises, 1u, __ATOMIC_RELAXED, __HIP_MEMORY_SCOPE_AGENT);
+                }
+            }
+        }
+    };
     auto epilogue = [&](uint64_t tile) __attribute__((always_inline)) {
         const uint32_t row0 = (uint32_t)(tile * SP3_BM) + ws * (MT * 16u) + 4 * kq_r;
         uint32_t hits8 = 0;
@@ -1408,6 +1461,8 @@
             if (!__ballot((hits8 >> nt) & 1u)) continue;
             const uint32_t q = (uint32_t)nt * 16 + m_r;
             const float th = thr_lds[q], qs = qs_lds[q];
+            const float bd = band_lds[q], x_min = lad ? __builtin_fmaf(th, qs, bd) : __builtin_inff();
+            uint32_t wmask = 0;
 #pragma unroll
             for (int mt = 0; mt < MT; ++mt) {
 #pragma unroll
@@ -1423,8 +1478,20 @@
                             wl[at] = make_uint4((uint32_t)key, (uint32_t)(key >> 32), q, 0u);
                         }
                         wcount += (uint32_t)__builtin_popcountll(hits);
+                        if (c && __builtin_fmaf(v, qs, -bd) > x_min) wmask |= 1u << (mt * 4 + j);
                     }
                 }
+            }
+            while (__ballot(wmask != 0)) {
+                const uint32_t slot = wmask ? (uint32_t)__builtin_ctz(wmask) : 0u;
+                const bool w_ok = wmask != 0;
+                wmask &= wmask - 1u;
+                int vi = acc[0][nt][0];
+#pragma unroll
+                for (int mt = 0; mt < MT; ++mt)
+#pragma unroll
+                    for (int j = 0; j < 4; ++j) vi = slot == (uint32_t)(mt * 4 + j) ? acc[mt][nt][j] : vi;
+                witness(w_ok, q, row0 + (slot >> 2) * 16u + (slot & 3u), __builtin_fmaf((float)vi, qs, -bd), th, qs, bd);
             }
         }
     };
@@ -1451,10 +1518,18 @@
 #pragma unroll
                 for (int nt = 0; nt < 8; ++nt) acc[mt][nt] = (i32x4s){0, 0, 0, 0};
         }
+        const uint32_t refresh = (uint32_t)__builtin_amdgcn_readfirstlane((lad && kc + 1 == nch && ((uint32_t)it & (uint32_t)(WAVES - 1)) == ws) ? 1 : 0);
+        uint2 fresh;
+        asm volatile("s_cmp_eq_u32 %3, 0\n\ts_cbranch_scc1 .Lsp_norefresh%=\n\tglobal_load_dwordx2 %0, %1, %2 sc1\n.Lsp_norefresh%=:"
+                     : "=v"(fresh) : "v"((uint32_t)lane * 8u), "s"(s.lad_thr), "s"(refresh) : "memory", "scc");
         load_stage(tile_r, kr, rc[IL]);
         advance_r();
         asm volatile("s_waitcnt vmcnt(%0)" : : "n"(NL * AHEAD) : "memory");
         asm volatile("" : "+v"(rc[I][0]), "+v"(rc[I][1]), "+v"(rc[I][2]), "+v"(rc[I][3]) : : "memory");
+        if (refresh) {
+            asm volatile("" : "+v"(fresh) : : "memory");
+            *reinterpret_cast<float2 *>(thr_lds + 2 * lane) = make_float2(ord_to_score(fresh.x), ord_to_score(fresh.y));
+        }
 #pragma unroll
         for (int hl = 0; hl < 2; ++hl) {
             const uint4 *bb = b_rd + kc * SP_B_UNITS + hl * 64;
@@ -1773,18 +1848,22 @@
     return QMX_OK;
 }
 int32_t launch_split_i8_pack(hipStream_t st, const float *d_q, uint32_t nq, uint32_t dim, const float *d_scale, const uint64_t *d_gthr, const uint32_t *d_row_stats,
-                             float row_norm_max, void *d_bq, float *d_qscale, float *d_band, float *d_thr, float *d_t_exact, uint32_t *d_cand_cnt, uint32_t n_cnt) {
+                             float row_norm_max, void *d_bq, float *d_qscale, float *d_band, float *d_thr, float *d_t_exact, uint32_t *d_cand_cnt, uint32_t n_cnt,
+                             uint32_t *d_ladder) {
     QMX_REQUIRE(nq <= (uint32_t)SP_QT, QMX_ERR_BAD_ARG, "int8 tile of %u queries", nq);
     ::qmx::clear_stale_error();
     hipLaunchKernelGGL(sp_i8_pack_kernel, dim3(SP_QT), dim3(256), (size_t)dim * 4, st, d_q, nq, dim, d_scale, d_gthr, d_row_stats, row_norm_max, (uint4 *)d_bq,
-                       d_qscale, d_band, d_thr, d_t_exact, d_cand_cnt, n_cnt);
+                       d_qscale, d_band, d_thr, d_t_exact, d_cand_cnt, n_cnt, d_ladder);
     QMX_HIP(hipGetLastError());
     return QMX_OK;
 }
+size_t split_i8_ladder_words() { return (size_t)SP_QT * (1 + SP_LAD_LEVELS); }
+bool split_i8_ladder_ok(uint32_t dim) { return option(OPT_I8_LADDER) > 0 && option(OPT_I8_RESIDENT) > 0 && dim / 128 <= SP8R_MAX_NCH; }
 int32_t launch_scan_i8copy(hipStream_t st, const ScanArgs &a, const void *d_bq, const float *d_qscale, const float *d_thr, int num_cus, const void *d_rows_i8,
-                           void *d_wlists, uint32_t phase) {
+                           void *d_wlists, uint32_t phase, const I8Ladder *ladder) {
     const uint32_t nch_r = a.dim / 128;
     const bool resident = option(OPT_I8_RESIDENT) > 0 && nch_r <= SP8R_MAX_NCH;
+    QMX_REQUIRE(!ladder || resident, QMX_ERR_OTHER, "the threshold ladder is the resident int8 scan's");
     void (*kfn)(const ScanArgs, const SplitArgs) = resident ? scan_i8copy_kernel_res<1> : scan_i8copy_kernel;
     const size_t lds_bytes = resident ? sp8r_lds_bytes(nch_r) : (size_t)SP8_LDS;
     static thread_local DeviceOnce attr_once;
@@ -1809,6 +1888,13 @@
     s.wcnt = (uint32_t *)d_wlists;
     s.wlist = (uint4 *)((unsigned char *)d_wlists + split_wlists_counts_bytes(num_cus));
     s.phase = phase;
+    if (ladder) {
+        s.lad_thr = ladder->words;
+        s.lad_cnt = ladder->words + SP_QT;
+        s.lad_t0 = ladder->t0;
+        s.lad_band = ladder->band;
+        s.lad_raises = ladder->raises;
+    }
     const uint64_t n_tiles = split_phase_tiles((a.n_cand + SP3_BM - 1) / SP3_BM, phase);
     if (n_tiles == 0) return QMX_OK;
     const uint32_t grid = (uint32_t)std::max<uint64_t>(1, std::min<uint64_t>(n_tiles, (uint64_t)num_cus));
diff --git a/qdrant_amd/scorer.py b/qdrant_amd/scorer.py
--- a/qdrant_amd/scorer.py
+++ b/qdrant_amd/scorer.py
@@ -681,6 +681,11 @@
         F.check(F.lib().qmx_query_last_counters(self._h, C.byref(c)))
         return c
 
+    def last_prefilter_stats(self) -> "F.PrefilterStats":
+        c = F.PrefilterStats()
+        F.check(F.lib().qmx_query_last_prefilter_stats(self._h, C.byref(c)))
+        return c
+
     def close(self):
         if self._h:
             F.lib().qmx_query_destroy(self._h)
```

New measurement: 96280. 1.3% lower.
